# ssteinberg/wave_tracer

Measured on AMD Instinct MI355X. Metric: Msamples/sec (whole node), cornell-box 1440^2 wave-mode, higher is better.
Workload: dtype f32

## Files before the change

wave_tracer_amd/api.py:

```python
import ctypes as C
import json
import math
import os

_HERE = os.path.dirname(os.path.abspath(__file__))

os.environ.setdefault("HSA_KERNARG_POOL_SIZE", str(16 << 20))


def lib_path():
    return os.environ.get("WTGPU_LIB") or os.path.join(_HERE, "libwtgpu.so")


class WtgpuError(RuntimeError):
    pass


class SceneParams(C.Structure):
    _fields_ = [("res", C.c_uint32), ("max_depth", C.c_int32), ("fsd", C.c_int32), ("mis", C.c_int32), ("rr", C.c_int32),
                ("force_ray_tracing", C.c_int32), ("mesh_detail", C.c_int32), ("lut_n_theta", C.c_uint32), ("lut_m", C.c_uint32),
                ("polarimetric", C.c_int32)]


class TestHooks(C.Structure):
    _fields_ = [("only_s", C.c_uint32), ("only_t", C.c_uint32), ("crop_of", C.c_uint32)]


class SensorMaskSpec(C.Structure):
    _fields_ = [("present", C.c_int32), ("samples", C.c_uint32), ("regex", C.c_char_p), ("shape_flags", C.POINTER(C.c_uint8)),
                ("n_shapes", C.c_uint32)]


class TonemapSpec(C.Structure):
    _fields_ = [("present", C.c_int32), ("op", C.c_int32), ("mode", C.c_int32), ("gamma", C.c_float), ("db_min", C.c_float), ("db_max", C.c_float),
                ("colourmap", C.c_char_p), ("function", C.c_char_p)]


class Tonemap(C.Structure):
    _fields_ = [("op", C.c_int32), ("mode", C.c_int32), ("gamma", C.c_float), ("db_min", C.c_float), ("db_max", C.c_float),
                ("table", C.POINTER(C.c_float)), ("table_n", C.c_uint32)]


class FilmStatsSpec(C.Structure):
    _fields_ = [("stokes_component", C.c_uint32), ("scale", C.c_uint32), ("bins", C.c_uint32), ("flags", C.c_uint32), ("lo", C.c_float), ("hi", C.c_float)]


class FilmStats(C.Structure):
    _fields_ = [("n", C.c_uint64), ("n_nan", C.c_uint64), ("n_negative", C.c_uint64), ("n_zero", C.c_uint64), ("n_below", C.c_uint64), ("n_above", C.c_uint64),
                ("min", C.c_float), ("max", C.c_float), ("min_positive", C.c_float), ("pad", C.c_float), ("sum", C.c_double)]


class FilmCompareSpec(C.Structure):
    _fields_ = [("stokes_component", C.c_uint32), ("flags", C.c_uint32), ("eps", C.c_double)]


FILM_COMPARE_FIELDS = [("n", C.c_uint64), ("n_nonfinite", C.c_uint64), ("n_nonfinite_mismatch", C.c_uint64), ("n_differ", C.c_uint64), ("argmax", C.c_uint64),
                       ("max_abs", C.c_double), ("sum_abs", C.c_double), ("sum_sq", C.c_double), ("sum_a_sq", C.c_double), ("sum_b_sq", C.c_double),
                       ("sum_rel", C.c_double)]


class FilmCompare(C.Structure):
    _fields_ = FILM_COMPARE_FIELDS


class FilmPolarSpec(C.Structure):
    _fields_ = [("flags", C.c_uint32), ("maps", C.c_uint32), ("picture_plane", C.c_uint32), ("format", C.c_uint32), ("c2", C.c_double), ("s2", C.c_double),
                ("sat_gain", C.c_float), ("pad", C.c_float), ("tonemap", Tonemap)]


FILM_POLAR_FIELDS = [("n", C.c_uint64), ("n_nonfinite", C.c_uint64), ("n_dark", C.c_uint64), ("n_over", C.c_uint64), ("argmax", C.c_uint64),
                     ("max_dop", C.c_double), ("sum_i", C.c_double), ("sum_q", C.c_double), ("sum_u", C.c_double), ("sum_v", C.c_double),
                     ("sum_lin", C.c_double), ("sum_pol", C.c_double)]


class FilmPolar(C.Structure):
    _fields_ = FILM_POLAR_FIELDS


class FilmDenoiseSpec(C.Structure):
    _fields_ = [("window_radius", C.c_uint32), ("patch_radius", C.c_uint32), ("flags", C.c_uint32), ("pad", C.c_uint32), ("k", C.c_float), ("alpha", C.c_float),
                ("eps", C.c_float), ("pad2", C.c_float)]


FILM_POLAR_MAPS = ["dolp", "dop", "docp", "aolp", "chi", "analyser"]
FILM_STATS_SCALES = ["linear", "dB"]
FILM_STATS_ABS, FILM_STATS_LUMINANCE = 1, 2
FILM_STATS_MAX_BINS = 4096
TONEMAP_OPS = ["linear", "gamma", "sRGB", "dB", "function"]
TONEMAP_MODES = ["select", "normal", "colourmap"]
TONEMAP_FORMATS = {"f32": 0, "u8": 1, "u16": 2}


class SceneInfo(C.Structure):
    _fields_ = [("width", C.c_uint32), ("height", C.c_uint32), ("channels", C.c_uint32), ("n_tris", C.c_uint32), ("n_edges", C.c_uint32),
                ("n_nodes", C.c_uint32), ("n_leaves", C.c_uint32), ("n_shapes", C.c_uint32), ("n_emitters", C.c_uint32),
                ("n_materials", C.c_uint32), ("max_depth", C.c_int32), ("sensor_type", C.c_uint32), ("fsd_lut_power", C.c_double * 2),
                ("bytes_per_sample_state", C.c_uint64), ("stokes", C.c_uint32), ("integrator", C.c_uint32)]


COUNTER_FIELDS = ["samples", "segments", "ray_queries", "cone_queries", "vertices", "connections", "shadow_rays", "cone_tri_overflow",
                  "edge_overflow", "fsd_edge_overflow", "fsd_pool_overflow", "fsd_interactions", "null_interactions",
                  "surface_interactions", "light_splats", "walk_iteration_cap_hits", "traversal_stack_dropped"]


class Counters(C.Structure):
    _fields_ = [(n, C.c_uint64) for n in COUNTER_FIELDS]

    def as_dict(self):
        return {n: int(getattr(self, n)) for n in COUNTER_FIELDS}


SYMBOLS = ["wtgpu_scene_create_named", "wtgpu_scene_create_from_desc", "wtgpu_scene_get_info", "wtgpu_scene_host_desc",
           "wtgpu_scene_upload", "wtgpu_render", "wtgpu_trace_rays", "wtgpu_traverse_cones", "wtgpu_get_counters",
           "wtgpu_reset_counters", "wtgpu_last_render_timings", "wtgpu_develop", "wtgpu_scene_destroy", "wtgpu_last_error",
           "wtgpu_scene_stats_json", "wtgpu_calibrate_copy", "wtgpu_render_async", "wtgpu_join", "wtgpu_query_regions", "wtgpu_render_progressive",
           "wtgpu_cancel", "wtgpu_pause", "wtgpu_resume", "wtgpu_capture_intermediate", "wtgpu_comm_unique_id", "wtgpu_comm_create", "wtgpu_film_reduce", "wtgpu_comm_destroy", "wtgpu_scene_create_from_xml",
           "wtgpu_scene_shape_id", "wtgpu_scene_sensor_mask_spec", "wtgpu_sensor_mask", "wtgpu_sensor_mask_host",
           "wtgpu_scene_tonemap_spec", "wtgpu_develop_device", "wtgpu_tonemap_device", "wtgpu_tonemap_host",
           "wtgpu_film_stats_edges", "wtgpu_film_stats_device", "wtgpu_film_stats_host",
           "wtgpu_film_compare_device", "wtgpu_film_compare_host", "wtgpu_film_polar_device", "wtgpu_film_polar_host",
           "wtgpu_film_denoise_device", "wtgpu_film_denoise_host"]
PROGRESS_CB = C.CFUNCTYPE(C.c_int, C.c_uint64, C.c_uint64, C.c_void_p)
CAPTURE_CB = C.CFUNCTYPE(None, C.c_uint64, C.c_void_p)

_lib = None


def connect_class_order():
    import numpy as np
    lib = load_library()
    lib.wtgpu_test_connect_class_order.argtypes = [C.c_void_p, C.c_uint32, C.c_void_p, C.c_void_p]
    n, dim = C.c_uint32(0), C.c_uint32(0)
    _check(lib.wtgpu_test_connect_class_order(None, 0, C.byref(n), C.byref(dim)))
    keys = np.zeros(n.value, np.uint32)
    _check(lib.wtgpu_test_connect_class_order(keys.ctypes.data, keys.size, C.byref(n), C.byref(dim)))
    return keys, int(dim.value)


def dn_exp2_neg(t):
    import numpy as np
    t = np.ascontiguousarray(t, dtype=np.float32)
    out = np.zeros(t.shape, dtype=np.float32)
    _check(load_library().wtgpu_test_dn_exp2_neg(t.ctypes.data, t.size, out.ctypes.data))
    return out


def load_library():
    global _lib
    if _lib is not None:
        return _lib
    p = lib_path()
    if not os.path.exists(p):
        raise WtgpuError(f"{p} is missing: build it with `python -c 'import __graft_entry__ as g; g.build()'` "
                         f"(hipcc --offload-arch=gfx950); wave_tracer_amd has no CPU fallback")
    os.environ.setdefault("HSA_KERNARG_POOL_SIZE", str(16 << 20))
    try:
        import torch
    except ImportError:
        pass
    lib = C.CDLL(p)
    vp, u64, u32, i32 = C.c_void_p, C.c_uint64, C.c_uint32, C.c_int
    lib.wtgpu_scene_create_named.argtypes = [C.c_char_p, C.POINTER(SceneParams), C.POINTER(vp)]
    lib.wtgpu_scene_create_named_hooks.argtypes = [C.c_char_p, C.POINTER(SceneParams), C.POINTER(TestHooks), C.POINTER(vp)]
    lib.wtgpu_scene_create_from_desc.argtypes = [vp, C.POINTER(vp)]
    lib.wtgpu_scene_create_from_xml.argtypes = [C.c_char_p, C.POINTER(C.c_char_p), u32, C.POINTER(SceneParams), C.POINTER(vp)]
    lib.wtgpu_scene_compare.argtypes = [vp, vp, C.c_char_p, C.c_size_t]
    lib.wtgpu_scene_compare_part.argtypes = [vp, vp, C.c_char_p, C.c_char_p, C.c_size_t]
    lib.wtgpu_trace_ab_stats.argtypes = [vp, C.POINTER(C.c_double), C.POINTER(C.c_double), C.POINTER(u64), C.POINTER(u64), C.POINTER(u64)]
    lib.wtgpu_render_progressive.argtypes = [vp, vp, vp, vp, vp, u64, u64, u64, u32, PROGRESS_CB, vp, C.POINTER(u64)]
    lib.wtgpu_cancel.argtypes = [vp]
    lib.wtgpu_pause.argtypes = [vp]
    lib.wtgpu_resume.argtypes = [vp]
    lib.wtgpu_capture_intermediate.argtypes = [vp, CAPTURE_CB, vp]
    lib.wtgpu_comm_unique_id.argtypes = [vp]
    lib.wtgpu_comm_create.argtypes = [i32, i32, i32, vp, C.POINTER(vp)]
    lib.wtgpu_film_reduce.argtypes = [vp, vp, vp, vp, vp, u64, u64, i32]
    lib.wtgpu_comm_destroy.argtypes = [vp]
    lib.wtgpu_comm_destroy.restype = None
    lib.wtgpu_scene_get_info.argtypes = [vp, C.POINTER(SceneInfo)]
    lib.wtgpu_scene_host_desc.argtypes = [vp]
    lib.wtgpu_scene_host_desc.restype = vp
    lib.wtgpu_scene_upload.argtypes = [vp, i32, u64]
    lib.wtgpu_render.argtypes = [vp, vp, vp, vp, vp, u64, u64, u64]
    lib.wtgpu_render_async.argtypes = [vp, vp, vp, vp, vp, u64, u64, u64]
    lib.wtgpu_join.argtypes = [vp, vp]
    lib.wtgpu_trace_rays.argtypes = [vp, vp, vp, u32, vp, vp, vp, vp]
    lib.wtgpu_traverse_cones.argtypes = [vp, vp, vp, u32, u32, vp, vp, vp, vp]
    lib.wtgpu_query_regions.argtypes = [vp, vp, vp, u32, u32, vp, vp, vp, vp, vp, vp, vp]
    lib.wtgpu_test_fsd_apertures.argtypes = [vp, vp, vp, vp, vp, vp, u32, u32, u32, u32, vp, vp]
    lib.wtgpu_test_utd_sums.argtypes = [vp, vp, vp, vp, vp, u32, u32, u32, vp, vp, vp]
    lib.wtgpu_test_profile_counters.argtypes = [vp, vp, u32]
    lib.wtgpu_test_bsdf_queries.argtypes = [vp, vp, vp, u32, i32, vp]
    lib.wtgpu_test_source_queries.argtypes = [vp, vp, vp, u32, vp]
    lib.wtgpu_test_flux_queries.argtypes = [vp, vp, vp, u32, vp]
    lib.wtgpu_scene_shape_id.argtypes = [vp, u32, C.POINTER(C.c_char_p)]
    lib.wtgpu_scene_sensor_mask_spec.argtypes = [vp, C.POINTER(SensorMaskSpec)]
    lib.wtgpu_sensor_mask.argtypes = [vp, vp, vp, u32, u64, vp]
    lib.wtgpu_sensor_mask_host.argtypes = [vp, vp, u32, u64, u32, vp]
    lib.wtgpu_scene_tonemap_spec.argtypes = [vp, C.POINTER(TonemapSpec)]
    lib.wtgpu_develop_device.argtypes = [vp, vp, vp, vp, vp, u64, vp]
    lib.wtgpu_tonemap_device.argtypes = [vp, vp, vp, vp, vp, u64, C.POINTER(Tonemap), u32, vp, u32, vp]
    lib.wtgpu_tonemap_host.argtypes = [vp, vp, vp, vp, u64, C.POINTER(Tonemap), u32, vp, u32, u32, vp]
    lib.wtgpu_film_stats_edges.argtypes = [C.POINTER(FilmStatsSpec), vp]
    lib.wtgpu_film_stats_device.argtypes = [vp, vp, vp, vp, vp, u64, C.POINTER(FilmStatsSpec), vp, vp, vp]
    lib.wtgpu_film_stats_host.argtypes = [vp, vp, vp, vp, u64, C.POINTER(FilmStatsSpec), vp, u32, vp, vp]
    lib.wtgpu_film_compare_device.argtypes = [vp, vp, vp, vp, vp, u64, vp, vp, vp, u64, C.POINTER(FilmCompareSpec), vp, vp, vp]
    lib.wtgpu_film_compare_host.argtypes = [vp, vp, vp, vp, u64, vp, vp, vp, u64, C.POINTER(FilmCompareSpec), vp, u32, vp, vp]
    lib.wtgpu_film_polar_device.argtypes = [vp, vp, vp, vp, vp, u64, C.POINTER(FilmPolarSpec), vp, vp, vp, vp]
    lib.wtgpu_film_polar_host.argtypes = [vp, vp, vp, vp, u64, C.POINTER(FilmPolarSpec), vp, u32, vp, vp, vp]
    lib.wtgpu_film_denoise_device.argtypes = [vp, vp, vp, vp, vp, u64, vp, vp, vp, u64, C.POINTER(FilmDenoiseSpec), vp, vp, vp]
    lib.wtgpu_film_denoise_host.argtypes = [vp, vp, vp, vp, u64, vp, vp, vp, u64, C.POINTER(FilmDenoiseSpec), vp, u32, vp, vp]
    lib.wtgpu_test_dn_exp2_neg.argtypes = [vp, u64, vp]
    lib.wtgpu_calibrate_copy.argtypes = [u64, i32]
    lib.wtgpu_get_counters.argtypes = [vp, C.POINTER(Counters)]
    lib.wtgpu_reset_counters.argtypes = [vp]
    lib.wtgpu_last_render_timings.argtypes = [vp, C.POINTER(C.c_float * 12)]
    lib.wtgpu_develop.argtypes = [vp, vp, vp, vp, u64, vp]
    lib.wtgpu_scene_destroy.argtypes = [vp]
    lib.wtgpu_scene_destroy.restype = None
    lib.wtgpu_last_error.restype = C.c_char_p
    lib.wtgpu_scene_stats_json.argtypes = [vp]
    lib.wtgpu_scene_stats_json.restype = C.c_char_p
    _lib = lib
    return lib


def _check(rc):
    if rc != 0:
        raise WtgpuError(f"wtgpu error {rc}: {load_library().wtgpu_last_error().decode(errors='replace')}")


class Scene:

    def __init__(self, name, res=256, max_depth=-1, fsd=-1, mis=-1, rr=-1, force_ray_tracing=0, mesh_detail=1, lut=(0, 0), only_s=None, only_t=None, crop_of=0,
                 polarimetric=0):
        lib = load_library()
        p = SceneParams(res, max_depth, fsd, mis, rr, force_ray_tracing, mesh_detail, lut[0], lut[1], polarimetric)
        h = C.c_void_p()
        if only_s is None and only_t is None and not crop_of:
            _check(lib.wtgpu_scene_create_named(name.encode(), C.byref(p), C.byref(h)))
        else:
            hooks = TestHooks(0 if only_s is None else only_s + 1, 0 if only_t is None else only_t + 1, crop_of)
            _check(lib.wtgpu_scene_create_named_hooks(name.encode(), C.byref(p), C.byref(hooks), C.byref(h)))
        self._h = h
        self.name = name
        info = SceneInfo()
        _check(lib.wtgpu_scene_get_info(h, C.byref(info)))
        self.info = info
        self.spectral_channels, self.stokes = info.channels, info.stokes
        self.width, self.height, self.channels = info.width, info.height, info.channels * info.stokes
        self.device = None

    @classmethod
    def from_desc(cls, desc_ptr, keepalive=None, name="<desc>"):
        lib = load_library()
        self = cls.__new__(cls)
        h = C.c_void_p()
        _check(lib.wtgpu_scene_create_from_desc(C.c_void_p(desc_ptr), C.byref(h)))
        self._h = h
        self._keepalive = keepalive
        self.name = name
        info = SceneInfo()
        _check(lib.wtgpu_scene_get_info(h, C.byref(info)))
        self.info = info
        self.spectral_channels, self.stokes = info.channels, info.stokes
        self.width, self.height, self.channels = info.width, info.height, info.channels * info.stokes
        self.device = None
        return self

    @classmethod
    def from_xml(cls, path, defines=None, res=0, max_depth=-1, fsd=-1, mis=-1, rr=-1, force_ray_tracing=0, lut=(0, 0), polarimetric=0, mesh_detail=1):
        lib = load_library()
        self = cls.__new__(cls)
        p = SceneParams(res, max_depth, fsd, mis, rr, force_ray_tracing, mesh_detail, lut[0], lut[1], polarimetric)
        d = [f"{k}={v}".encode() for k, v in (defines or {}).items()]
        arr = (C.c_char_p * max(1, len(d)))(*d)
        h = C.c_void_p()
        _check(lib.wtgpu_scene_create_from_xml(str(path).encode(), arr, len(d), C.byref(p), C.byref(h)))
        self._h = h
        self.name = os.path.basename(str(path))
        info = SceneInfo()
        _check(lib.wtgpu_scene_get_info(h, C.byref(info)))
        self.info = info
        self.spectral_channels, self.stokes = info.channels, info.stokes
        self.width, self.height, self.channels = info.width, info.height, info.channels * info.stokes
        self.device = None
        return self

    def first_difference(self, other, part=None):
        buf = C.create_string_buffer(256)
        if part:
            rc = load_library().wtgpu_scene_compare_part(self._h, other._h, part.encode(), buf, 256)
        else:
            rc = load_library().wtgpu_scene_compare(self._h, other._h, buf, 256)
        if rc not in (0, 1):
            _check(rc)
        return buf.value.decode()

    @property
    def handle(self):
        return self._h

    def host_desc(self):
        return load_library().wtgpu_scene_host_desc(self._h)

    def stats(self):
        return json.loads(load_library().wtgpu_scene_stats_json(self._h).decode())

    def emitter_summary(self):
        return self.stats()["emitter_list"]

    def upload(self, device=0, max_batch_samples=0):
        _check(load_library().wtgpu_scene_upload(self._h, int(device), int(max_batch_samples)))
        self.device = int(device)
        return self

    def render_into(self, value, weight, light, sample_begin, sample_end, seed, stream=None):
        sp = C.c_void_p(stream) if stream else None
        _check(load_library().wtgpu_render(self._h, sp, value.data_ptr(), weight.data_ptr(), light.data_ptr(), int(sample_begin),
                                           int(sample_end), int(seed)))

    def render_async_into(self, value, weight, light, sample_begin, sample_end, seed, stream=None):
        sp = C.c_void_p(stream) if stream else None
        _check(load_library().wtgpu_render_async(self._h, sp, value.data_ptr(), weight.data_ptr(), light.data_ptr(), int(sample_begin),
                                                 int(sample_end), int(seed)))

    def render_progressive(self, value, weight, light, sample_begin, sample_end, seed, chunk_spp=1, progress=None, stream=None):
        sp = C.c_void_p(stream) if stream else None
        cb = PROGRESS_CB((lambda d, t, u: 1 if progress(d, t) else 0) if progress else (lambda d, t, u: 0))
        done = C.c_uint64(0)
        lib = load_library()
        rc = lib.wtgpu_render_progressive(self._h, sp, value.data_ptr(), weight.data_ptr(), light.data_ptr(), int(sample_begin), int(sample_end),
                                          int(seed), int(chunk_spp), cb, None, C.byref(done))
        if rc == 6:
            return True, int(done.value)
        _check(rc)
        return False, int(done.value)

    def cancel(self):
        _check(load_library().wtgpu_cancel(self._h))

    def pause(self):
        _check(load_library().wtgpu_pause(self._h))

    def resume(self):
        _check(load_library().wtgpu_resume(self._h))

    def capture_intermediate(self, fn):
        keep = self.__dict__.setdefault("_capture_keepalive", [])
        slot = []

        def tramp(done, user):
            try:
                fn(int(done))
            finally:
                if slot and slot[0] in keep:
                    keep.remove(slot[0])
        cb = CAPTURE_CB(tramp)
        slot.append(cb)
        keep.append(cb)
        if len(keep) > 64:
            del keep[0]
        _check(load_library().wtgpu_capture_intermediate(self._h, cb, None))

    def join(self, stream=None):
        _check(load_library().wtgpu_join(self._h, C.c_void_p(stream) if stream else None))

    def trace_rays(self, rays):
        import numpy as np
        import torch
        dev = torch.device("cuda", self.device)
        n = len(rays)
        d_rays = torch.from_numpy(np.ascontiguousarray(rays, dtype=np.float32)).to(dev)
        dist = torch.zeros(n, dtype=torch.float32, device=dev)
        tuid = torch.zeros(n, dtype=torch.int32, device=dev)
        bary = torch.zeros((n, 2), dtype=torch.float32, device=dev)
        front = torch.zeros(n, dtype=torch.int32, device=dev)
        _check(load_library().wtgpu_trace_rays(self._h, None, d_rays.data_ptr(), n, dist.data_ptr(), tuid.data_ptr(), bary.data_ptr(), front.data_ptr()))
        torch.cuda.synchronize(dev)
        return dist.cpu().numpy(), tuid.cpu().numpy().view(np.uint32), bary.cpu().numpy(), front.cpu().numpy().view(np.uint32)

    def traverse_cones(self, cones, cap=64):
        import numpy as np
        import torch
        dev = torch.device("cuda", self.device)
        n = len(cones)
        d_cones = torch.from_numpy(np.ascontiguousarray(cones, dtype=np.float32)).to(dev)
        dist = torch.zeros(n, dtype=torch.float32, device=dev)
        flags = torch.zeros(n, dtype=torch.int32, device=dev)
        ntris = torch.zeros(n, dtype=torch.int32, device=dev)
        tris = torch.zeros((n, cap), dtype=torch.int32, device=dev)
        _check(load_library().wtgpu_traverse_cones(self._h, None, d_cones.data_ptr(), n, cap, dist.data_ptr(), flags.data_ptr(), ntris.data_ptr(),
                                                   tris.data_ptr()))
        torch.cuda.synchronize(dev)
        return (dist.cpu().numpy(), flags.cpu().numpy().view(np.uint32), ntris.cpu().numpy().view(np.uint32),
                tris.cpu().numpy().view(np.uint32))

    def query_regions(self, cones, edge_cap=96):
        import numpy as np
        import torch
        dev = torch.device("cuda", self.device)
        n = len(cones)
        d_cones = torch.from_numpy(np.ascontiguousarray(cones, dtype=np.float32)).to(dev)
        dist = torch.zeros(n, dtype=torch.float32, device=dev)
        flux = torch.zeros(n, dtype=torch.float32, device=dev)
        flags, primary, ntris, nedges = (torch.zeros(n, dtype=torch.int32, device=dev) for _ in range(4))
        edges = torch.full((n, edge_cap), -1, dtype=torch.int32, device=dev)
        _check(load_library().wtgpu_query_regions(self._h, None, d_cones.data_ptr(), n, edge_cap, dist.data_ptr(), flags.data_ptr(), primary.data_ptr(),
                                                  ntris.data_ptr(), nedges.data_ptr(), edges.data_ptr(), flux.data_ptr()))
        torch.cuda.synchronize(dev)
        u = lambda t: t.cpu().numpy().view(np.uint32)
        return {"dist": dist.cpu().numpy(), "flags": u(flags), "primary": u(primary), "ntris": u(ntris), "nedges": u(nedges), "edges": u(edges),
                "flux": flux.cpu().numpy()}

    def fsd_apertures(self, cones, sk, ids, n_ids, pool_cap=4096, mode=0):
        import numpy as np
        import torch
        dev = torch.device("cuda", self.device)
        ids = np.ascontiguousarray(ids, dtype=np.uint32)
        n, id_cap = ids.shape
        n_ids = np.ascontiguousarray(n_ids, dtype=np.uint32)
        assert len(cones) == n and len(sk) == n and len(n_ids) == n and (n_ids <= id_cap).all()
        n_edges = self.info.n_edges
        assert all((ids[i, :n_ids[i]] < n_edges).all() for i in range(n)), "edge id out of range"
        t = lambda a, dt: torch.from_numpy(np.ascontiguousarray(a, dtype=dt)).to(dev)
        d_cones, d_sk = t(cones, np.float32), t(sk, np.float32)
        d_ids, d_nids = t(ids.view(np.int32), np.int32), t(n_ids.view(np.int32), np.int32)
        hdr = torch.zeros((n, 8), dtype=torch.int32, device=dev)
        segs = torch.zeros((n, pool_cap, 7), dtype=torch.float32, device=dev)
        _check(load_library().wtgpu_test_fsd_apertures(self._h, None, d_cones.data_ptr(), d_sk.data_ptr(), d_ids.data_ptr(), d_nids.data_ptr(), n, id_cap,
                                                       pool_cap, mode, hdr.data_ptr(), segs.data_ptr()))
        torch.cuda.synchronize(dev)
        return hdr.cpu().numpy().view(np.uint32), segs.cpu().numpy()

    def utd_sums(self, queries, ids, n_ids, utd_cap=48):
        import numpy as np
        import torch
        dev = torch.device("cuda", self.device)
        ids = np.ascontiguousarray(ids, dtype=np.uint32)
        n, id_cap = ids.shape
        n_ids = np.ascontiguousarray(n_ids, dtype=np.uint32)
        assert len(queries) == n and len(n_ids) == n and (n_ids <= id_cap).all()
        n_edges = self.info.n_edges
        assert all((ids[i, :n_ids[i]] < n_edges).all() for i in range(n)), "edge id out of range"
        t = lambda a, dt: torch.from_numpy(np.ascontiguousarray(a, dtype=dt)).to(dev)
        d_q, d_ids, d_nids = t(queries, np.float32), t(ids.view(np.int32), np.int32), t(n_ids.view(np.int32), np.int32)
        hdr = torch.zeros((n, 8), dtype=torch.int32, device=dev)
        edges = torch.zeros((n, utd_cap, 8), dtype=torch.int32, device=dev)
        recs = torch.zeros((n, utd_cap, 3), dtype=torch.int32, device=dev)
        _check(load_library().wtgpu_test_utd_sums(self._h, None, d_q.data_ptr(), d_ids.data_ptr(), d_nids.data_ptr(), n, id_cap, utd_cap, recs.data_ptr(),
                                                  hdr.data_ptr(), edges.data_ptr()))
        torch.cuda.synchronize(dev)
        u = lambda x: x.cpu().numpy().view(np.uint32)
        return u(hdr), u(edges), u(recs)

    def bsdf_queries(self, queries, form=-1):
        import numpy as np
        import torch
        dev = torch.device("cuda", self.device)
        q = np.ascontiguousarray(queries, dtype=np.uint32)
        n = q.shape[0]
        assert q.shape == (n, 18) and (q[:, 0] < self.info.n_materials).all(), "material id out of range"
        d_q = torch.from_numpy(q.view(np.int32)).to(dev)
        out = torch.zeros((n, 48), dtype=torch.int32, device=dev)
        _check(load_library().wtgpu_test_bsdf_queries(self._h, None, d_q.data_ptr(), n, int(form), out.data_ptr()))
        torch.cuda.synchronize(dev)
        return out.cpu().numpy().view(np.uint32)

    def source_queries(self, queries):
        import numpy as np
        import torch
        dev = torch.device("cuda", self.device)
        q = np.ascontiguousarray(queries, dtype=np.uint32)
        n = q.shape[0]
        assert q.shape == (n, 24)
        d_q = torch.from_numpy(q.view(np.int32)).to(dev)
        out = torch.zeros((n, 80), dtype=torch.int32, device=dev)
        _check(load_library().wtgpu_test_source_queries(self._h, None, d_q.data_ptr(), n, out.data_ptr()))
        torch.cuda.synchronize(dev)
        return out.cpu().numpy().view(np.uint32)

    def flux_queries(self, queries):
        import numpy as np
        import torch
        dev = torch.device("cuda", self.device)
        q = np.ascontiguousarray(queries, dtype=np.uint32)
        n = q.shape[0]
        assert q.shape == (n, 20)
        d_q = torch.from_numpy(q.view(np.int32)).to(dev)
        out = torch.zeros((n, 36), dtype=torch.int32, device=dev)
        _check(load_library().wtgpu_test_flux_queries(self._h, None, d_q.data_ptr(), n, out.data_ptr()))
        torch.cuda.synchronize(dev)
        return out.cpu().numpy().view(np.uint32)

    @property
    def shape_ids(self):
        lib, out = load_library(), []
        for i in range(self.info.n_shapes):
            p = C.c_char_p()
            _check(lib.wtgpu_scene_shape_id(self._h, i, C.byref(p)))
            out.append(p.value.decode())
        return out

    @property
    def sensor_mask_spec(self):
        import numpy as np
        s = SensorMaskSpec()
        _check(load_library().wtgpu_scene_sensor_mask_spec(self._h, C.byref(s)))
        if not s.present:
            return None
        flags = np.ctypeslib.as_array(s.shape_flags, (s.n_shapes,)).copy() if s.n_shapes else np.zeros(0, np.uint8)
        return {"regex": s.regex.decode(), "samples": int(s.samples), "shapes": flags}

    def _mask_args(self, samples, shapes):
        import numpy as np
        if samples is None:
            spec = self.sensor_mask_spec
            samples = spec["samples"] if spec else 32
        if shapes is None:
            return int(samples), None
        flags = np.ascontiguousarray(np.asarray(shapes) != 0, dtype=np.uint8)
        if flags.shape != (self.info.n_shapes,):
            raise ValueError(f"shapes: one flag per shape expected ({self.info.n_shapes}), got shape {flags.shape}")
        return int(samples), flags

    def sensor_mask(self, samples=None, seed=1, shapes=None, stream=None):
        import torch
        if self.device is None:
            raise WtgpuError("sensor_mask: upload(device) first")
        dev = torch.device("cuda", self.device)
        n, flags = self._mask_args(samples, shapes)
        out = torch.empty((self.height, self.width), dtype=torch.float32, device=dev)
        _check(load_library().wtgpu_sensor_mask(self._h, self._stream_arg(stream, dev), None if flags is None else flags.ctypes.data, n, int(seed),
                                                out.data_ptr()))
        return out

    def sensor_mask_host(self, samples=None, seed=1, shapes=None, threads=0):
        import numpy as np
        n, flags = self._mask_args(samples, shapes)
        out = np.zeros((self.height, self.width), np.float32)
        _check(load_library().wtgpu_sensor_mask_host(self._h, None if flags is None else flags.ctypes.data, n, int(seed), int(threads), out.ctypes.data))
        return out

    @property
    def tonemap_spec(self):
        s = TonemapSpec()
        _check(load_library().wtgpu_scene_tonemap_spec(self._h, C.byref(s)))
        return {"present": bool(s.present), "op": TONEMAP_OPS[s.op], "mode": TONEMAP_MODES[s.mode], "gamma": float(s.gamma),
                "db_range": (float(s.db_min), float(s.db_max)), "colourmap": s.colourmap.decode(), "function": s.function.decode()}

    @staticmethod
    def _tonemap_struct(tm):
        import numpy as np
        if tm is None:
            return None, None
        table = tm.get("table")
        tab = None if table is None else np.ascontiguousarray(table, dtype=np.float32)
        if tab is not None and (tab.ndim != 2 or tab.shape[1] != 3):
            raise ValueError(f"table: [n, 3] expected, got shape {tab.shape}")
        db = tm.get("db_range", (0.0, 0.0))
        st = Tonemap(TONEMAP_OPS.index(tm.get("op", "linear")), TONEMAP_MODES.index(tm.get("mode", "select")), float(tm.get("gamma", 2.2)),
                     float(db[0]), float(db[1]), None if tab is None else tab.ctypes.data_as(C.POINTER(C.c_float)), 0 if tab is None else len(tab))
        return st, tab

    @staticmethod
    def _stream_arg(stream, dev):
        import torch
        st = stream if stream is not None else torch.cuda.current_stream(dev).cuda_stream
        return C.c_void_p(st) if st else None

    def _host_films(self, what, value, weight, light, mask=None):
        import numpy as np
        v, w, l = (np.ascontiguousarray(t, dtype=np.float64) for t in (value, weight, light))
        m = None if mask is None else np.ascontiguousarray(mask, dtype=np.float32)
        n = self.width * self.height
        if v.size != n * self.channels or l.size != v.size or w.size != n or (m is not None and m.size != n):
            raise ValueError(f"{what}: films of the scene's size expected")
        return v, w, l, m

    def _device_films(self, what, value, weight, light, mask=None):
        import torch
        if self.device is None:
            raise WtgpuError(f"{what}: upload(device) first")
        n = self.width * self.height
        for t, name, numel, dtype in ((value, "value", n * self.channels, torch.float64), (weight, "weight", n, torch.float64),
                                      (light, "light", n * self.channels, torch.float64), (mask, "mask", n, torch.float32)):
            if t is None and name == "mask":
                continue
            if not (t.is_cuda and t.device.index == self.device and t.dtype == dtype and t.numel() == numel and t.is_contiguous()):
                raise ValueError(f"{what}: {name}: a contiguous {dtype} tensor of {numel} elements on cuda:{self.device} expected")
        return torch.device("cuda", self.device)

    def develop_device(self, value, weight, light, spe, stream=None):
        import torch
        dev = self._device_films("develop_device", value, weight, light)
        out = torch.empty(tuple(value.shape), dtype=torch.float32, device=dev)
        _check(load_library().wtgpu_develop_device(self._h, self._stream_arg(stream, dev), value.data_ptr(), weight.data_ptr(), light.data_ptr(), int(spe),
                                                   out.data_ptr()))
        return out

    def tonemap_device(self, value, weight, light, spe, tm=None, stokes_component=0, mask=None, fmt="f32", stream=None):
        import torch
        dev = self._device_films("tonemap_device", value, weight, light, mask)
        st_tm, keep = self._tonemap_struct(tm)
        dtype = {"f32": torch.float32, "u8": torch.uint8, "u16": torch.int16}[fmt]
        out = torch.empty((self.height, self.width, 4 if mask is not None else 3), dtype=dtype, device=dev)
        _check(load_library().wtgpu_tonemap_device(self._h, self._stream_arg(stream, dev), value.data_ptr(), weight.data_ptr(), light.data_ptr(), int(spe),
                                                   None if st_tm is None else C.byref(st_tm), int(stokes_component),
                                                   None if mask is None else mask.data_ptr(), TONEMAP_FORMATS[fmt], out.data_ptr()))
        del keep
        return out

    def tonemap_host(self, value, weight, light, spe, tm=None, stokes_component=0, mask=None, fmt="f32", threads=0):
        import numpy as np
        v, w, l, m = self._host_films("tonemap_host", value, weight, light, mask)
        st_tm, keep = self._tonemap_struct(tm)
        out = np.zeros((self.height, self.width, 4 if m is not None else 3), {"f32": np.float32, "u8": np.uint8, "u16": np.uint16}[fmt])
        _check(load_library().wtgpu_tonemap_host(self._h, v.ctypes.data, w.ctypes.data, l.ctypes.data, int(spe), None if st_tm is None else C.byref(st_tm),
                                                 int(stokes_component), None if m is None else m.ctypes.data, TONEMAP_FORMATS[fmt], int(threads), out.ctypes.data))
        del keep
        return out

    def _film_stats(self, what, call, stokes_component, scale, range, bins, abs, luminance):
        import numpy as np
        if scale not in FILM_STATS_SCALES:
            raise ValueError(f"{what}: scale 'dB' or 'linear' expected, got {scale!r}")
        planes = self.spectral_channels + (1 if luminance else 0)
        flags = (FILM_STATS_ABS if abs else 0) | (FILM_STATS_LUMINANCE if luminance else 0)

        def one_pass(lo, hi, nbins):
            spec = FilmStatsSpec(int(stokes_component), FILM_STATS_SCALES.index(scale), int(nbins), flags, float(lo), float(hi))
            rec = (FilmStats * max(planes, 1))()
            hist = np.zeros((planes, min(int(nbins), FILM_STATS_MAX_BINS)), dtype=np.uint64)
            call(spec, rec, hist.ctypes.data if hist.size else None)
            return spec, rec, hist

        if range is None:
            _, rec, _ = one_pass(0.0, 0.0, 0)
            lows = np.array([r.min_positive if scale == "dB" else r.min for r in rec], dtype=np.float64)
            highs = np.array([r.max for r in rec], dtype=np.float64)
            if np.isnan(lows).all() or not np.isfinite(np.nanmax(highs)):
                raise ValueError(f"{what}: range=None needs a finite {'positive ' if scale == 'dB' else ''}element to take the range from; pass a range")
            lo, hi = float(np.nanmin(lows)), float(np.nanmax(highs))
            if scale == "dB":
                lo, hi = 10.0 * math.log10(lo) - 1e-3, 10.0 * math.log10(hi) + 1e-3
            else:
                pad = max(math.fabs(lo), math.fabs(hi), 1e-30) * 1e-6
                lo, hi = lo - pad, hi + pad
            range = (lo, hi)
        spec, rec, hist = one_pass(range[0], range[1], bins)
        edges = np.zeros(spec.bins + 1, dtype=np.float32)
        _check(load_library().wtgpu_film_stats_edges(C.byref(spec), edges.ctypes.data))
        out = {name: np.array([getattr(r, name) for r in rec], dtype=dt) for name, dt in
               (("n", np.uint64), ("n_nan", np.uint64), ("n_negative", np.uint64), ("n_zero", np.uint64), ("n_below", np.uint64), ("n_above", np.uint64),
                ("min", np.float32), ("max", np.float32), ("min_positive", np.float32), ("sum", np.float64))}
        out.update(hist=hist, edges=edges, scale=scale, range=(float(spec.lo), float(spec.hi)), bins=int(spec.bins))
        return out

    def film_stats_device(self, value, weight, light, spe, *, stokes_component=0, scale="dB", range=None, bins=256, abs=False, luminance=False, mask=None,
                          stream=None):
        dev = self._device_films("film_stats_device", value, weight, light, mask)
        st = self._stream_arg(stream, dev)
        lib = load_library()

        def call(spec, rec, hist):
            _check(lib.wtgpu_film_stats_device(self._h, st, value.data_ptr(), weight.data_ptr(), light.data_ptr(), int(spe),
                                               C.byref(spec), None if mask is None else mask.data_ptr(), C.cast(rec, C.c_void_p), hist))
        return self._film_stats("film_stats_device", call, stokes_component, scale, range, bins, abs, luminance)

    def film_stats_host(self, value, weight, light, spe, *, stokes_component=0, scale="dB", range=None, bins=256, abs=False, luminance=False, mask=None,
                        threads=0):
        v, w, l, m = self._host_films("film_stats_host", value, weight, light, mask)
        lib = load_library()

        def call(spec, rec, hist):
            _check(lib.wtgpu_film_stats_host(self._h, v.ctypes.data, w.ctypes.data, l.ctypes.data, int(spe), C.byref(spec), None if m is None else m.ctypes.data,
                                             int(threads), C.cast(rec, C.c_void_p), hist))
        return self._film_stats("film_stats_host", call, stokes_component, scale, range, bins, abs, luminance)

    def _film_compare(self, call, stokes_component, abs, luminance, eps):
        import numpy as np
        planes = self.spectral_channels + (1 if luminance else 0)
        spec = FilmCompareSpec(int(stokes_component), (FILM_STATS_ABS if abs else 0) | (FILM_STATS_LUMINANCE if luminance else 0), float(eps))
        rec = (FilmCompare * max(planes, 1))()
        call(spec, rec, planes)
        out = {name: np.array([getattr(r, name) for r in rec], dtype=np.uint64 if t is C.c_uint64 else np.float64) for name, t in FILM_COMPARE_FIELDS}
        finite = (out["n"] - out["n_nonfinite"]).astype(np.float64)
        with np.errstate(divide="ignore", invalid="ignore"):
            out["rmse"] = np.sqrt(out["sum_sq"] / finite)
            out["mean_abs"] = out["sum_abs"] / finite
            out["rel_l2"] = np.sqrt(out["sum_sq"] / out["sum_b_sq"])
            out["rel_mse"] = out["sum_rel"] / finite
        return out

    def film_compare_device(self, films_a, spe_a, films_b, spe_b, *, stokes_component=0, abs=False, luminance=False, mask=None, eps=1e-4, diff=False, stream=None):
        import torch
        dev = self._device_films("film_compare_device", *films_a, mask)
        self._device_films("film_compare_device", *films_b)
        st = self._stream_arg(stream, dev)
        d = {}

        def call(spec, rec, planes):
            if diff:
                d["diff"] = torch.empty((self.height, self.width, planes), dtype=torch.float32, device=dev)
            _check(load_library().wtgpu_film_compare_device(self._h, st, *(t.data_ptr() for t in films_a), int(spe_a),
                                                            *(t.data_ptr() for t in films_b), int(spe_b), C.byref(spec), None if mask is None else mask.data_ptr(),
                                                            C.cast(rec, C.c_void_p), d["diff"].data_ptr() if diff else None))
        out = self._film_compare(call, stokes_component, abs, luminance, eps)
        out.update(d)
        return out

    def film_compare_host(self, films_a, spe_a, films_b, spe_b, *, stokes_component=0, abs=False, luminance=False, mask=None, eps=1e-4, diff=False, threads=0):
        import numpy as np
        sets = [self._host_films("film_compare_host", *films)[:3] for films in (films_a, films_b)]
        m = None if mask is None else np.ascontiguousarray(mask, dtype=np.float32)
        if m is not None and m.size != self.width * self.height:
            raise ValueError("film_compare_host: a mask of the scene's size expected")
        d = {}

        def call(spec, rec, planes):
            if diff:
                d["diff"] = np.zeros((self.height, self.width, planes), dtype=np.float32)
            _check(load_library().wtgpu_film_compare_host(self._h, *(t.ctypes.data for t in sets[0]), int(spe_a), *(t.ctypes.data for t in sets[1]), int(spe_b),
                                                          C.byref(spec), None if m is None else m.ctypes.data, int(threads), C.cast(rec, C.c_void_p),
                                                          d["diff"].ctypes.data if diff else None))
        out = self._film_compare(call, stokes_component, abs, luminance, eps)
        out.update(d)
        return out

    def _film_polar(self, what, call, luminance, maps, analyser, c2s2, picture, picture_plane, tm, fmt, sat_gain, masked):
        import numpy as np
        names = [maps] if isinstance(maps, str) else list(maps)
        for m in names:
            if m not in FILM_POLAR_MAPS:
                raise ValueError(f"{what}: maps of {FILM_POLAR_MAPS} expected, got {m!r}")
        if fmt not in TONEMAP_FORMATS:
            raise ValueError(f"{what}: fmt f32, u8 or u16 expected, got {fmt!r}")
        names = [m for m in FILM_POLAR_MAPS if m in names]
        planes = self.spectral_channels + (1 if luminance else 0)
        c2, s2 = (math.cos(2.0 * analyser), math.sin(2.0 * analyser)) if c2s2 is None else c2s2
        st_tm, _ = self._tonemap_struct(dict(tm or {"op": "linear"}, table=None))
        spec = FilmPolarSpec(FILM_STATS_LUMINANCE if luminance else 0, sum(1 << FILM_POLAR_MAPS.index(m) for m in names), int(picture_plane), TONEMAP_FORMATS[fmt],
                             float(c2), float(s2), float(sat_gain), 0.0, st_tm)
        rec = (FilmPolar * max(planes, 1))()
        got_maps, got_picture = call(spec, rec, (self.height, self.width, planes, len(names)) if names else None,
                                     (self.height, self.width, 4 if masked else 3) if picture else None)
        out = {name: np.array([getattr(r, name) for r in rec][:planes], dtype=np.uint64 if t is C.c_uint64 else np.float64) for name, t in FILM_POLAR_FIELDS}
        with np.errstate(divide="ignore", invalid="ignore"):
            out["dop_total"] = np.sqrt(out["sum_q"] ** 2 + out["sum_u"] ** 2 + out["sum_v"] ** 2) / out["sum_i"]
            out["aolp_total"] = 0.5 * np.arctan2(out["sum_u"], out["sum_q"])
            out["mean_dolp"] = out["sum_lin"] / out["sum_i"]
            out["mean_dop"] = out["sum_pol"] / out["sum_i"]
        out["maps"] = {m: got_maps[..., k] for k, m in enumerate(names)}
        out["picture"] = got_picture
        return out

    def film_polar_device(self, value, weight, light, spe, *, luminance=False, maps=(), analyser=0.0, c2s2=None, mask=None, picture=False, picture_plane=0, tm=None,
                          fmt="f32", sat_gain=1.0, stream=None):
        import torch
        dev = self._device_films("film_polar_device", value, weight, light, mask)
        st = self._stream_arg(stream, dev)

        def call(spec, rec, maps_shape, picture_shape):
            m = None if maps_shape is None else torch.empty(maps_shape, dtype=torch.float32, device=dev)
            p = None if picture_shape is None else torch.empty(picture_shape, dtype={"f32": torch.float32, "u8": torch.uint8, "u16": torch.int16}[fmt], device=dev)
            _check(load_library().wtgpu_film_polar_device(self._h, st, value.data_ptr(), weight.data_ptr(), light.data_ptr(), int(spe), C.byref(spec),
                                                          None if mask is None else mask.data_ptr(), C.cast(rec, C.c_void_p),
                                                          None if m is None else m.data_ptr(), None if p is None else p.data_ptr()))
            return m, p
        return self._film_polar("film_polar_device", call, luminance, maps, analyser, c2s2, picture, picture_plane, tm, fmt, sat_gain, mask is not None)

    def film_polar_host(self, value, weight, light, spe, *, luminance=False, maps=(), analyser=0.0, c2s2=None, mask=None, picture=False, picture_plane=0, tm=None,
                        fmt="f32", sat_gain=1.0, threads=0):
        import numpy as np
        v, w, l, m = self._host_films("film_polar_host", value, weight, light, mask)

        def call(spec, rec, maps_shape, picture_shape):
            mp = None if maps_shape is None else np.zeros(maps_shape, dtype=np.float32)
            p = None if picture_shape is None else np.zeros(picture_shape, dtype={"f32": np.float32, "u8": np.uint8, "u16": np.uint16}[fmt])
            _check(load_library().wtgpu_film_polar_host(self._h, v.ctypes.data, w.ctypes.data, l.ctypes.data, int(spe), C.byref(spec),
                                                        None if m is None else m.ctypes.data, int(threads), C.cast(rec, C.c_void_p),
                                                        None if mp is None else mp.ctypes.data, None if p is None else p.ctypes.data))
            return mp, p
        return self._film_polar("film_polar_host", call, luminance, maps, analyser, c2s2, picture, picture_plane, tm, fmt, sat_gain, m is not None)

    @staticmethod
    def _film_denoise_spec(window, patch, k, alpha, eps):
        return FilmDenoiseSpec(int(window), int(patch), 0, 0, float(k), float(alpha), float(eps), 0.0)

    def film_denoise_device(self, films_a, spe_a, films_b, spe_b, *, window=7, patch=2, k=0.45, alpha=1.0, eps=1e-10, mask=None, residual=False, stream=None):
        import torch
        dev = self._device_films("film_denoise_device", *films_a, mask)
        self._device_films("film_denoise_device", *films_b)
        shape = (self.height, self.width, self.spectral_channels, self.stokes)
        out = torch.empty(shape, dtype=torch.float32, device=dev)
        res = torch.empty(shape, dtype=torch.float32, device=dev) if residual else None
        spec = self._film_denoise_spec(window, patch, k, alpha, eps)
        _check(load_library().wtgpu_film_denoise_device(self._h, self._stream_arg(stream, dev), *(t.data_ptr() for t in films_a), int(spe_a),
                                                        *(t.data_ptr() for t in films_b), int(spe_b), C.byref(spec), None if mask is None else mask.data_ptr(),
                                                        out.data_ptr(), None if res is None else res.data_ptr()))
        return {"film": out, "residual": res}

    def film_denoise_host(self, films_a, spe_a, films_b, spe_b, *, window=7, patch=2, k=0.45, alpha=1.0, eps=1e-10, mask=None, residual=False, threads=0):
        import numpy as np
        sets = [self._host_films("film_denoise_host", *films)[:3] for films in (films_a, films_b)]
        m = None if mask is None else np.ascontiguousarray(mask, dtype=np.float32)
        if m is not None and m.size != self.width * self.height:
            raise ValueError("film_denoise_host: a mask of the scene's size expected")
        shape = (self.height, self.width, self.spectral_channels, self.stokes)
        out = np.zeros(shape, dtype=np.float32)
        res = np.zeros(shape, dtype=np.float32) if residual else None
        spec = self._film_denoise_spec(window, patch, k, alpha, eps)
        _check(load_library().wtgpu_film_denoise_host(self._h, *(t.ctypes.data for t in sets[0]), int(spe_a), *(t.ctypes.data for t in sets[1]), int(spe_b),
                                                      C.byref(spec), None if m is None else m.ctypes.data, int(threads), out.ctypes.data,
                                                      None if res is None else res.ctypes.data))
        return {"film": out, "residual": res}

    def profile_counters(self, n=8):
        out = (C.c_uint64 * n)()
        _check(load_library().wtgpu_test_profile_counters(self._h, out, n))
        return [int(v) for v in out]

    def connect_class_items(self, slice=0, max_items=1 << 22):
        import numpy as np
        lib = load_library()
        lib.wtgpu_test_connect_class_items.argtypes = [C.c_void_p, C.c_uint32, C.c_void_p, C.c_void_p, C.c_uint32, C.c_void_p]
        n_keys = connect_class_order()[0].size
        table = np.zeros(3 * n_keys + 1, np.uint32)
        items = np.zeros(max_items, np.uint32)
        n = C.c_uint32(0)
        _check(lib.wtgpu_test_connect_class_items(self._h, slice, table.ctypes.data, items.ctypes.data, items.size, C.byref(n)))
        return table[:n_keys + 1].copy(), table[n_keys + 1:2 * n_keys + 1].copy(), table[2 * n_keys + 1:].copy(), items[:n.value].copy()

    def counters(self):
        c = Counters()
        _check(load_library().wtgpu_get_counters(self._h, C.byref(c)))
        return c.as_dict()

    def reset_counters(self):
        _check(load_library().wtgpu_reset_counters(self._h))

    def trace_ab_stats(self):
        a, b, d, w, r = C.c_double(0), C.c_double(0), C.c_uint64(0), C.c_uint64(0), C.c_uint64(0)
        _check(load_library().wtgpu_trace_ab_stats(self._h, C.byref(a), C.byref(b), C.byref(d), C.byref(w), C.byref(r)))
        return {"ms_refill": a.value, "ms_sm": b.value, "differing_words": int(d.value), "walks": int(w.value), "rounds": int(r.value)}

    def timings(self):
        t = (C.c_float * 12)()
        _check(load_library().wtgpu_last_render_timings(self._h, C.byref(t)))
        return {"generate_ms": t[0], "trace_ms": t[1], "interact_ms": t[2], "connect_ms": t[3], "rounds": int(t[4]),
                "trace_launches": int(t[5]), "batches": int(t[6]), "trace_heavy_ms": t[7], "interact_b_ms": t[8], "flux_ms": t[9],
                "interact_c_ms": t[10], "rounds_per_batch": float(t[11])}

    def close(self):
        if self._h:
            load_library().wtgpu_scene_destroy(self._h)
            self._h = None

    def __del__(self):
        try:
            self.close()
        except Exception:
            pass


class Comm:

    def __init__(self, world, rank, device, unique_id):
        h = C.c_void_p()
        self._id = C.create_string_buffer(bytes(unique_id), 128)
        _check(load_library().wtgpu_comm_create(int(world), int(rank), int(device), self._id, C.byref(h)))
        self._h = h

    @staticmethod
    def unique_id():
        buf = C.create_string_buffer(128)
        _check(load_library().wtgpu_comm_unique_id(buf))
        return buf.raw

    def film_reduce(self, value, weight, light, root=0, stream=None):
        sp = C.c_void_p(stream) if stream else None
        _check(load_library().wtgpu_film_reduce(self._h, sp, value.data_ptr(), weight.data_ptr(), light.data_ptr(), value.numel(), weight.numel(), int(root)))

    def close(self):
        if self._h:
            load_library().wtgpu_comm_destroy(self._h)
            self._h = None

    def __del__(self):
        try:
            self.close()
        except Exception:
            pass
```

wave_tracer_amd/csrc/kernels_fsd.hip:

```cpp
#include "wtgpu_kernels.h"

namespace wtk {

__global__ void __launch_bounds__(64, 3) k_flux_split(launch_args_t a) {
    __shared__ coop_gather_shared_t sh;
    coop_set_dropped_counter(sh, a.st.counters + kDroppedSlot);
    uint32_t* ctl = a.st.ctl;
    const uint32_t n = ctl[CTL_INTC_COUNT];
    const int lane = threadIdx.x & 63;
    for (;;) {
        const uint32_t base = wave_grab(ctl + CTL_FSPLIT_HEAD);
        if (base >= n) break;
        uint32_t w_mine = 0;
        bool need = false;
        if (base + (uint32_t)lane < n) {
            w_mine = a.st.intc_queue[base + lane];
            need = is_region_marker(WT_TRAV_U(a, w_mine, tuid));
        }
        unsigned long long m = __ballot(need);
        while (m) {
            const int src = __ffsll((long long)m) - 1;
            m &= m - 1;
            const uint32_t w = (uint32_t)__shfl((int)w_mine, src, 64);
            const walk_trace_in_t wk = walk_load_trace_in(a.st.walks, a.st.walk_words, w);
            const cone_t tcone = walk_trace_envelope(a.sc, wk);
            const float beam_dist = WT_TRAV_F(a, w, dist), region_depth = WT_TRAV_F(a, w, region_depth);
            if (threadIdx.x == 0) a.st.facc[w] = 0.0;
            coop_split(a.sc, tcone, range_t{beam_dist, beam_dist + region_depth}, sh, a.flux_task_tris, [&](int32_t ptr) {
                const uint32_t idx = atomicAdd(ctl + CTL_FTASK_COUNT, 1u);
                if (idx < a.st.ftask_cap)
                    a.st.ftasks[idx] = make_uint2(w, (uint32_t)ptr);
                else
                    atomicAdd(a.st.counters + WT_COUNTER_SLOT(fsd_pool_overflow), 1ull);
            });
            __syncthreads();
        }
    }
}
__global__ void __launch_bounds__(64, WTGPU_LB_FLUX) k_flux_tasks(launch_args_t a) {
    __shared__ coop_gather_shared_t sh;
    coop_set_dropped_counter(sh, a.st.counters + kDroppedSlot);
    uint32_t* ctl = a.st.ctl;
    const uint32_t n = min(ctl[CTL_FTASK_COUNT], a.st.ftask_cap);
    for (;;) {
        const uint32_t item = wave_grab_item(ctl + CTL_FTASK_HEAD);
        if (item >= n) break;
        const uint2 task = a.st.ftasks[item];
        const uint32_t w = task.x;
        walk_t wk;
        soa_load(a.st.walks, a.st.walk_words, w, wk);
        const float beam_dist = WT_TRAV_F(a, w, dist), region_depth = WT_TRAV_F(a, w, region_depth);
        const bool want_front = WT_TRAV_U(a, w, front_face) != 0;
        const range_t izr{beam_dist, beam_dist + region_depth};
        const vec3 sd3 = beam_footprint(wk.beam, beam_dist) / kBeamEnvelope;
        const cone_t tcone = walk_trace_envelope(a.sc, wk);
        unsigned long long gst[2] = {0, 0};
        const double flux = coop_gather(a.sc, tcone, izr, wk.beam.env, cone_frame(wk.beam.env), izr, vec2{sd3.x, sd3.y}, want_front, sh, true, false,
                                        a.profile ? gst : nullptr, (int32_t)task.y).flux;
        if (threadIdx.x == 0) {
            if (flux != 0.0) unsafeAtomicAdd(&a.st.facc[w], flux);
            if (a.profile) {
                atomicAdd(a.st.counters + kNumCounters + 0, 1ull);
                atomicAdd(a.st.counters + kNumCounters + 1, gst[0]);
                atomicAdd(a.st.counters + kNumCounters + 2, gst[1]);
                atomicMax(a.st.counters + kNumCounters + 4, gst[0]);
            }
        }
        __syncthreads();
    }
}

constexpr uint32_t kEasyTries = 512;
constexpr uint32_t kStageSegs = 256;
template <int BLOCK>
WT_D void interact_c_body(const launch_args_t& a, int in) {
    constexpr bool HARD = BLOCK > 64;
    __shared__ uint32_t s_item;
    __shared__ uint32_t s_tmin;
    __shared__ float s_res[3];
    __shared__ stack_entry_t lds[8];
    __shared__ fsd_edge_t s_seg[kStageSegs];
    uint32_t* ctl = a.st.ctl;
    const uint32_t n = ctl[HARD ? CTL_INTD_COUNT : CTL_INTC_COUNT];
    const uint32_t* queue_in = HARD ? a.st.intd_queue : a.st.intc_queue;
    const int tid = threadIdx.x, lane = threadIdx.x & 63;
    bdpt_counters_t ctr;
    memset(&ctr, 0, sizeof(ctr));
    const fsd_pool_t pool = fsd_pool_of(a);
    for (;;) {
        const long long pl0 = a.profile == 3 ? clock64() : 0;
        uint32_t item = 0;
        if (HARD) {
            __syncthreads();
            if (tid == 0) s_item = atomicAdd(ctl + CTL_INTD_HEAD, 1u);
            __syncthreads();
            item = s_item;
        } else
            item = wave_grab_item(ctl + CTL_INTC_HEAD);
        if (item >= n) break;
        const uint32_t w = queue_in[item];
        uint32_t i, stream;
        walk_ident(a, w, i, stream);
        const uint64_t sample_id = sample_id_of(a, i);
        const uint32_t rng_draws = a.st.walks[(size_t)w * a.st.walk_words + WT_WALK_WORD(rng_draws)];
        const uint32_t slot = WT_TRAV_U(a, w, by);
        fsd_aperture_t ap = pool.hdr[slot];
        const fsd_edges_ref_t ed = fsd_pool_edges(pool, slot);
        const long long pc0 = a.profile == 3 ? clock64() : 0;
        if (!HARD) {
            const walk_trace_in_t wk = walk_load_trace_in(a.st.walks, a.st.walk_words, w);
            cone_t benv = wk.env;
            const float tr_dist = WT_TRAV_F(a, w, dist), tr_depth = WT_TRAV_F(a, w, region_depth);
            const uint32_t tr_tuid = WT_TRAV_U(a, w, tuid), tr_ntris = WT_TRAV_U(a, w, ntris);
            const bool tr_front = WT_TRAV_U(a, w, front_face) != 0;
            const range_t izr{tr_dist, tr_dist + tr_depth};
            const vec2 axes = cone_axes(benv, tr_dist);
            const vec2 sigma{axes.x / kBeamEnvelope, axes.y / kBeamEnvelope};
            double flux;
            if (is_region_marker(tr_tuid)) {
                flux = a.st.facc[w];
            } else {
                const uint32_t* tl = a.st.tris + (size_t)w * kTriListWords;
                flux = (uint32_t)lane < tr_ntris ? (double)region_triangle_flux(a.sc, cone_frame(benv), benv, izr, sigma, tl[lane], tr_front) : 0.0;
#pragma unroll
                for (int off = 32; off > 0; off >>= 1) flux += __shfl_xor(flux, off, 64);
            }
            const float I = (float)(1.0 - flux);
            ap.recp_I = I > 0.f ? 1.f / I : 0.f;
            if (lane == 0) pool.hdr[slot] = ap;
        }
        const sampler_t ss = make_sampler(a.seed, sample_id, stream, 0);
        const uint32_t base = fsd_tries_base(make_sampler(a.seed, sample_id, stream, rng_draws));
        const uint32_t max_tries = fsd_max_tries(ap);
        const uint32_t t_begin = HARD ? kEasyTries : 0u, t_end = HARD ? max_tries : (max_tries < kEasyTries ? max_tries : kEasyTries);
        bool acc = false;
        uint32_t t_acc = 0;
        float rx = 0.f, ry = 0.f, rf = 0.f;
        auto run_tries = [&](const fsd_edges_ref_t& edr) {
            for (uint32_t t0 = t_begin; t0 < t_end && !acc; t0 += BLOCK) {
                const uint32_t t = t0 + (uint32_t)tid;
                fsd_try_t r{{0.f, 0.f}, 0.f, 0u};
                if (t < t_end) r = fsd_try(a.sc, ap, edr, sampler_at(ss, base + t * kFsdDrawsPerTry));
                if (!HARD) {
                    const unsigned long long am = __ballot(r.accept != 0);
                    if (am) {
                        const int wl = __ffsll((long long)am) - 1;
                        rx = __shfl(r.x.x, wl, 64);
                        ry = __shfl(r.x.y, wl, 64);
                        rf = __shfl(r.f, wl, 64);
                        t_acc = t0 + (uint32_t)wl;
                        acc = true;
                    }
                } else {
                    if (tid == 0) s_tmin = 0xFFFFFFFFu;
                    __syncthreads();
                    if (r.accept) atomicMin(&s_tmin, t);
                    __syncthreads();
                    const uint32_t tm = s_tmin;
                    if (tm != 0xFFFFFFFFu) {
                        if (t == tm) {
                            s_res[0] = r.x.x;
                            s_res[1] = r.x.y;
                            s_res[2] = r.f;
                        }
                        __syncthreads();
                        rx = s_res[0];
                        ry = s_res[1];
                        rf = s_res[2];
                        t_acc = tm;
                        acc = true;
                    }
                    __syncthreads();
                }
            }
        };
        if (ap.n_edges <= kStageSegs) {
            __syncthreads();
            for (uint32_t k = (uint32_t)tid; k < ap.n_edges; k += BLOCK) s_seg[k] = ed.p[k];
            __syncthreads();
            run_tries(fsd_edges_ref_t{s_seg, 1});
        } else
            run_tries(ed);
        if (a.profile == 3 && tid == 0) {
            const int bin = 31 - __clz((int)max(ap.n_edges, 1u));
            atomicAdd(a.st.counters + kNumCounters + 8 + bin, 1ull);
            atomicAdd(a.st.counters + kNumCounters + 24 + bin, (unsigned long long)(acc ? t_acc + 1u - t_begin : t_end - t_begin));
            atomicAdd(a.st.counters + kNumCounters + 40 + bin, (unsigned long long)(clock64() - pc0));
            atomicAdd(a.st.counters + kNumCounters + 112 + bin, (unsigned long long)(pc0 - pl0));
        }
        const long long pm0 = a.profile == 3 ? clock64() : 0;
        if (!HARD && !acc && t_end < max_tries) {
            if (lane == 0) a.st.intd_queue[atomicAdd(ctl + CTL_INTD_COUNT, 1u)] = w;
            continue;
        }
        bool cont = false;
        if (tid == 0) {
            walk_t wk;
            soa_load(a.st.walks, a.st.walk_words, w, wk);
            trav_result_t tr;
            soa_load(a.st.trav, kTravWords, w, tr);
            fsd_defer_t defer;
            defer.defer_sampling = defer.to_sampling_pass = 0;
            defer.have_aperture = 1;
            defer.split_no_primary = 0;
            defer.known_no_primary = 1;
            defer.no_primary = 0;
            defer.has_gather = defer.gather_n_edges = defer.gather_edge_overflow = 0;
            defer.gather_flux = 0.f;
            defer.gather_edges = nullptr;
            defer.pending = 0;
            defer.resolved = 1;
            defer.slot = slot;
            defer.base = base;
            defer.next_try = 0;
            defer.fs = fsd_finalize(ap, acc, vec2{rx, ry}, rf);
            defer.end_draws = fsd_draws_after(base, acc ? t_acc : max_tries - 1u);
            const uint_list_t tris{a.st.tris + (size_t)w * kTriListWords, 1u, kMaxConeTris};
            const vertex_store_t vs = walk_vertices(a, w);
            stack_ref_t stack = make_stack_ref(lds, 1, 8, 8, nullptr);
            cont = bdpt_walk_step<2>(a.sc, wk, tr, tris, vs, pool, a.seed, sample_id, stream, &ctr, &stack, &defer);
            wk.active = cont ? 1u : 0u;
            soa_store(a.st.walks, a.st.walk_words, w, wk);
            if (a.profile == 3) atomicAdd(a.st.counters + kNumCounters + 96 + (31 - __clz((int)max(ap.n_edges, 1u))), (unsigned long long)(clock64() - pm0));
        }
        if (tid < 64) queue_append(a, ctl, 1 - in, cont, w);
    }
    if (a.count_stats && tid < 64) flush_counters(a.st.counters, ctr);
}
__global__ void __launch_bounds__(64, WTGPU_LB_INTERACT_C) k_interact_c(launch_args_t a, int in) { interact_c_body<64>(a, in); }
__global__ void __launch_bounds__(WTGPU_HARD_BLOCK) k_interact_c_hard(launch_args_t a, int in) { interact_c_body<WTGPU_HARD_BLOCK>(a, in); }

}
```

wave_tracer_amd/csrc/kernels_trace_refill.h:

```cpp
#pragma once
#include "wtgpu_kernels.h"

namespace wtk {

#ifndef WTGPU_LEAF_NUM
#define WTGPU_LEAF_NUM 1
#define WTGPU_LEAF_DEN 2
#endif
#ifndef WTGPU_REFILL_MIN
#define WTGPU_REFILL_MIN 16
#endif
WT_D bool policy_next_query(const scene_t& sc, const cone_t& env, bool rt, const stack_ref_t& stack, axis_walk_t& aw, cone_query_t& q, trav_result_t& r) {
    for (;;) {
        const int need = aw_next(sc, env, rt, stack, aw, q, r);
        if (need != AW_TEST) return need == AW_QUERY;
        aw_test_done(aw, cone_attempt_too_short_by(sc, env, aw.cand, aw.sr, aw.min_df_prog));
    }
}
WT_D void trace_round_begin(uint32_t* ctl, int in, uint32_t round, uint32_t n) {
    ctl[CTL_COUNT0 + (1 - in)] = 0;
    ctl[CTL_BACK0 + (1 - in)] = 0;
    ctl[CTL_HEAD_INTERACT] = 0;
    ctl[CTL_INTB_COUNT] = 0;
    ctl[CTL_INTB_HEAD] = 0;
    ctl[CTL_GATHER_COUNT] = 0;
    ctl[CTL_GATHER_HEAD] = 0;
    ctl[CTL_INTC_COUNT] = 0;
    ctl[CTL_INTC_HEAD] = 0;
    ctl[CTL_FTASK_COUNT] = 0;
    ctl[CTL_FTASK_HEAD] = 0;
    ctl[CTL_FSPLIT_HEAD] = 0;
    ctl[CTL_EPOOL_COUNT] = 0;
    ctl[CTL_INTD_COUNT] = 0;
    ctl[CTL_INTD_HEAD] = 0;
#pragma unroll
    for (uint32_t c = 0; c < kNumWalkClasses; ++c) ctl[CTL_CLS_COUNT0 + c] = ctl[CTL_CLS_HEAD0 + c] = 0;
    ctl[CTL_UTD_COUNT0 + (round & 1u)] = 0;
    ctl[CTL_FSDQ_COUNT0 + ((round + 1u) & 1u)] = 0;
    ctl[CTL_FSDQ_HEAD] = 0;
    ctl[CTL_NEEQ_COUNT] = 0;
    ctl[CTL_NEEQ_HEAD] = 0;
    if (n > 0) ctl[CTL_ROUNDS] = round + 1;
}
WT_D void trace_refill_body(const launch_args_t& a, int in, int first_round, uint32_t round) {
    __shared__ stack_entry_t lds[kLdsStack * kBlock];
    uint32_t* ctl = a.st.ctl;
    const uint32_t n = queue_count(ctl, in);
    if (blockIdx.x == 0 && threadIdx.x == 0) trace_round_begin(ctl, in, round, n);
    bdpt_counters_t ctr;
    memset(&ctr, 0, sizeof(ctr));
    stack_entry_t spill[kSpillStack];
    stack_ref_t stack;
    lds_stack(lds, spill, stack);
    const size_t W2 = 2 * (size_t)a.st.cap;
    const bool rt = a.sc.sensor.ray_trace_only || a.sc.opts.force_ray_tracing;
    const int lane = threadIdx.x & 63;
    const unsigned long long below = (1ull << lane) - 1ull;
    int st = 0;
    uint32_t w = 0;
    cone_t env;
    axis_walk_t aw;
    cone_query_t q;
    uint_list_t tris{nullptr, 1u, 0u, nullptr};
    memset(&env, 0, sizeof(env));
    memset(&aw, 0, sizeof(aw));
    memset(&q, 0, sizeof(q));
    bool exhausted = false;
#ifdef WTGPU_REFILL_PROF
    unsigned long long pc[6] = {0, 0, 0, 0, 0, 0}, pl[6] = {0, 0, 0, 0, 0, 0};
    long long pt;
#define RP_BEGIN() pt = clock64()
#define RP_END(i, mask) do { const long long d_ = clock64() - pt; pc[i] += (unsigned long long)d_; pl[i] += (unsigned long long)d_ * (unsigned long long)__popcll(mask); } while (0)
#else
#define RP_BEGIN()
#define RP_END(i, mask)
#endif
    for (;;) {
        bool fin = false;
        trav_result_t r;
        RP_BEGIN();
        const unsigned long long m_srv = __ballot(st == 2);
        if (st == 2) {
            cq_end(env, tris, q);
            fin = aw_query_done(a.sc, env, aw, q.rec, r);
            if (!fin) fin = !policy_next_query(a.sc, env, rt, stack, aw, q, r);
            st = fin ? 0 : 1;
        }
        RP_END(0, m_srv);
        uint32_t w_fin = w;
        const int n_idle = __popcll(__ballot(st == 0 && !fin)), n_run = __popcll(__ballot(st == 1));
        bool fetched = false;
        const bool any_fin = __ballot(fin) != 0;
        if (!exhausted && !any_fin && (n_idle >= WTGPU_REFILL_MIN || n_run == 0)) {
            const unsigned long long im = __ballot(st == 0);
            const bool take = st == 0;
            uint32_t base = 0;
            if (lane == 0) base = atomicAdd(ctl + CTL_HEAD_TRACE, (uint32_t)__popcll(im));
            base = (uint32_t)__shfl((int)base, 0, 64);
            if (base + (uint32_t)__popcll(im) >= n) exhausted = true;
            const uint32_t qi = base + (uint32_t)__popcll(im & below);
            RP_BEGIN();
            const unsigned long long m_f = __ballot(take && qi < n);
            if (take && qi < n) {
                w = queue_walk(a, ctl, in, qi, first_round);
                w_fin = w;
                const walk_trace_in_t wk = walk_load_trace_in(a.st.walks, a.st.walk_words, w);
                uint32_t* slot = a.st.tris + (size_t)w * kTriListWords;
                tris = uint_list_t{slot, 1u, (a.collect_list & 1u) ? kMaxConeTris : 0u, reinterpret_cast<float*>(slot + kMaxConeTris)};
                env = walk_trace_envelope(a.sc, wk);
                ray_hit_t ah;
                const bool axis_hit = ads_intersect_ray(a.sc, env.o, env.d, range_t{0.f, WT_INF}, stack, ah);
                aw_begin(aw, wavenum_to_wavelen_m(wk.k), WT_INF, axis_hit, ah, a.cone_budget, true, !(a.collect_list & 1u) || (a.collect_list & 2u), a.lane_cache ? wk.prev_offset_tuid : kInvalid);
                aw.use_cache = a.lane_cache;
                fin = !policy_next_query(a.sc, env, rt, stack, aw, q, r);
                st = fin ? 0 : 1;
            }
            RP_END(1, m_f);
            fetched = true;
        }
        RP_BEGIN();
        const unsigned long long m_st = __ballot(fin);
        {
            const bool heavy = fin && r.aborted == 1;
            if (fin) {
                if (heavy) {
                    a.st.trav[(size_t)w_fin * kTravWords + WT_TRAV_WORD(dist)] = __float_as_uint(r.dist);
                    a.st.trav[(size_t)w_fin * kTravWords + WT_TRAV_WORD(ntris)] = r.ntris;
                    a.st.trav[(size_t)w_fin * kTravWords + WT_TRAV_WORD(n_ray_queries)] = r.n_ray_queries;
                    a.st.trav[(size_t)w_fin * kTravWords + WT_TRAV_WORD(n_cone_queries)] = r.n_cone_queries;
                    a.st.trav[(size_t)w_fin * kTravWords + WT_TRAV_WORD(tuid)] = r.tuid;
                    a.st.trav[(size_t)w_fin * kTravWords + WT_TRAV_WORD(bx)] = __float_as_uint(r.bx);
                    a.st.trav[(size_t)w_fin * kTravWords + WT_TRAV_WORD(by)] = __float_as_uint(r.by);
                    a.st.trav[(size_t)w_fin * kTravWords + WT_TRAV_WORD(pdist)] = __float_as_uint(r.pdist);
                    a.st.trav[(size_t)w_fin * kTravWords + WT_TRAV_WORD(front_face)] = r.front_face;
                    a.st.trav[(size_t)w_fin * kTravWords + WT_TRAV_WORD(overflow)] = r.overflow;
                } else {
                    soa_store(a.st.trav, kTravWords, w_fin, r);
                    ctr.segments += 1;
                    ctr.ray_queries += r.n_ray_queries;
                    ctr.cone_queries += r.n_cone_queries;
                    if (a.collect_list & 1u) ctr.cone_tri_overflow += r.overflow;
                }
            }
            wave_append(a.st.heavy_queue, ctl + CTL_HEAVY_COUNT, heavy, w_fin);
        }
        RP_END(2, m_st);
        if (fetched || any_fin) continue;
        const int running = __popcll(__ballot(st == 1));
        if (running == 0) {
            if (exhausted) break;
            continue;
        }
        const int leave_at = running < 4 * WTGPU_REFILL_MIN ? (running + 3) / 4 : WTGPU_REFILL_MIN;
        for (;;) {
            for (;;) {
                const bool at_node = st == 1 && q.leaf == 0 && q.s > 0;
                const unsigned long long nm = __ballot(at_node);
                if (!nm) break;
                RP_BEGIN();
                if (at_node) cq_node_step(a.sc, env, stack, q);
                RP_END(3, nm);
                if (WTGPU_LEAF_DEN * __popcll(__ballot(st == 1 && q.leaf != 0)) >= WTGPU_LEAF_NUM * running) break;
            }
            RP_BEGIN();
            const unsigned long long m_leaf = __ballot(st == 1 && q.leaf != 0);
            if (st == 1 && q.leaf != 0) cq_leaf_step(a.sc, env, stack, tris, q);
            RP_END(4, m_leaf);
            if (st == 1 && !cq_running(q)) st = 2;
            const int waiting = __popcll(__ballot(st == 2)) + (exhausted ? 0 : __popcll(__ballot(st == 0)));
            if (waiting >= leave_at || !__ballot(st == 1)) break;
        }
    }
    if (a.count_stats) flush_counters(a.st.counters, ctr);
#ifdef WTGPU_REFILL_PROF
    if (lane == 0)
        for (int i = 0; i < 6; ++i) {
            atomicAdd(a.st.counters + kNumCounters + i, pc[i]);
            atomicAdd(a.st.counters + kNumCounters + 8 + i, pl[i]);
        }
    if (lane != 0 && pc[5]) { atomicAdd(a.st.counters + kNumCounters + 5, pc[5]); atomicAdd(a.st.counters + kNumCounters + 8 + 5, pl[5]); }
#endif
}


}
```

wave_tracer_amd/csrc/wtgpu.hip:

```cpp
#include "wtgpu_host.h"

thread_local std::string g_err;

static void note_rounds(wtgpu_scene* s, uint32_t n) { s->rounds_hist[s->rounds_hist_n++ % 8u] = n; }
static int drain_rec(wtgpu_scene* s, chunk_rec_t& r) {
    if (!r.busy) return WTGPU_OK;
    HIP_CHECK(hipEventSynchronize(r.ev[r.ev_final]));
    const uint32_t rounds = r.h_ctl[CTL_ROUNDS];
    s->cap_hits += r.h_ctl[CTL_COUNT0 + (r.rounds_launched & 1u)] + r.h_ctl[CTL_BACK0 + (r.rounds_launched & 1u)];
    s->acc[4] += rounds;
    s->acc[5] += rounds;
    s->acc[6] += 1;
    s->rounds_launched_total += r.rounds_launched;
    if (s->knobs.timing) {
        auto elapsed = [](hipEvent_t a, hipEvent_t b) {
            float ms = 0.f;
            return hipEventElapsedTime(&ms, a, b) == hipSuccess ? ms : 0.f;
        };
        s->acc[0] += elapsed(r.ev[0], r.ev[1]);
        size_t e = 1;
        for (uint32_t k = 0; k < r.rounds_timed; ++k, e += 6) {
            static const int slot[6] = {1, 7, 2, 8, 9, 10};
            for (int q = 0; q < 6; ++q) s->acc[slot[q]] += elapsed(r.ev[e + q], r.ev[e + q + 1]);
        }
        s->acc[3] += elapsed(r.ev[e], r.ev[r.ev_final]);
    }
    r.busy = false;
    return WTGPU_OK;
}

struct batch_launcher_t {
    wtgpu_scene* s;
    const wtgpu_scene::knobs_t& K;
    uint32_t grid_round = 0, grid_heavy = 0;
    bool path_mode = false;
    bool ev_fail = false;
    static constexpr int kHpSlots = 64;
    bool hp_on = false, trace_on = false;
    double hp_t[kHpSlots] = {0};
    unsigned long hp_n[kHpSlots] = {0};
    static const char** hp_labels() {
        static const char* labels[kHpSlots] = {nullptr};
        return labels;
    }
    static int hp_slot(const char* label) {
        static std::mutex m;
        std::lock_guard<std::mutex> l(m);
        const char** labels = hp_labels();
        int i = 0;
        while (i < kHpSlots - 1 && labels[i] && std::strcmp(labels[i], label) != 0) ++i;
        if (!labels[i]) labels[i] = label;
        return i;
    }
    explicit batch_launcher_t(wtgpu_scene* s_) : s(s_), K(s_->knobs) {
        grid_round = s->n_cus * K.round_blocks_per_cu;
        grid_heavy = s->n_cus * K.heavy_waves_per_cu;
        path_mode = s->host.opts.integrator != INTEGRATOR_BDPT;
        hp_on = K.host_prof != 0;
        trace_on = K.trace_launch != 0;
    }
#define HP_LAUNCH(kernel, ...)                                                                                            \
    do {                                                                                                                  \
        if (trace_on) {    \
            fprintf(stderr, "[wtgpu launch] %s ...", #kernel);                                                            \
            hipLaunchKernelGGL(kernel, __VA_ARGS__);                                                                      \
            const hipError_t e_ = hipDeviceSynchronize();                                                                 \
            fprintf(stderr, " done (%s)\n", hipGetErrorString(e_));                                                       \
        } else if (hp_on) {                                                                                                      \
            static const int slot_ = hp_slot(#kernel);                                                                    \
            const auto t0_ = std::chrono::steady_clock::now();                                                            \
            hipLaunchKernelGGL(kernel, __VA_ARGS__);                                                                      \
            hp_t[slot_] += std::chrono::duration<double, std::micro>(std::chrono::steady_clock::now() - t0_).count();     \
            hp_n[slot_]++;                                                                                                \
        } else                                                                                                            \
            hipLaunchKernelGGL(kernel, __VA_ARGS__);                                                                      \
    } while (0)
    void rec(chunk_rec_t& r, hipStream_t st_) {
        const auto hp0_ = std::chrono::steady_clock::now();
        if (s->knobs.timing && r.ev_used + 1 >= r.ev.size()) return;
        if (s->knobs.timing && hipEventRecord(r.ev[r.ev_used++], st_) != hipSuccess) ev_fail = true;
        if (hp_on) { static const int slot_ = hp_slot("hipEventRecord"); hp_t[slot_] += std::chrono::duration<double, std::micro>(std::chrono::steady_clock::now() - hp0_).count(); hp_n[slot_]++; }
    }
    uint32_t g_full(uint32_t nb) const { return std::min<uint32_t>(grid_round, ((path_mode ? 1u : 2u) * nb + kBlock - 1) / kBlock); }
    void generate(const launch_args_t& a, chunk_rec_t& r, hipStream_t st_) {
        r.ev_used = 0;
        r.rounds_launched = 0;
        r.rounds_timed = 0;
        rec(r, st_);
        if (path_mode)
            HP_LAUNCH(k_path_generate, dim3((a.nb + kBlock - 1) / kBlock), dim3(kBlock), 0, st_, a);
        else
            HP_LAUNCH(k_generate, dim3((a.nb + kBlock - 1) / kBlock), dim3(kBlock), 0, st_, a);
        rec(r, st_);
    }
    int rounds(const launch_args_t& a, const path_state_t* ps, chunk_rec_t& r, hipStream_t st_, uint32_t r_begin, uint32_t r_end, int stage_from = 0) {
        const uint32_t nb = a.nb, walks_per_sample = path_mode ? 1u : 2u, gf = g_full(nb);
        const uint32_t grid_div_b = K.grid_div_b, grid_div_c = K.grid_div_c, grid_mul_flux = K.grid_mul_flux;
        const int dbg_stage = (int)K.dbg_stage;
        for (uint32_t round = r_begin; round < r_end; ++round) {
            const int in = (int)(round & 1u), first = round == 0 ? 1 : 0;
            if (s->knobs.timing && r.ev_used + 7 < r.ev.size()) r.rounds_timed++;
            if (round == K.stagger_round && K.stagger_round > 0) {
                HIP_CHECK(hipEventRecord(r.ev_stagger, st_));
                s->ev_stagger_last = r.ev_stagger;
            }
            uint32_t g0, gh;
            if (K.decay_q > 0) {
                const double f = std::min(1.0, (double)K.decay_c * std::pow(K.decay_q * .01, (double)round));
                g0 = std::max<uint32_t>(2u, (uint32_t)(gf * f));
                gh = std::max<uint32_t>(2u, (uint32_t)(std::min<uint32_t>(grid_heavy, walks_per_sample * nb) * f));
            } else {
                const uint32_t shrink = round < K.shrink_r1 ? 1u : (round < K.shrink_r2 ? K.shrink_f1 : K.shrink_f2);
                g0 = std::max<uint32_t>(1u, gf / shrink);
                gh = std::max<uint32_t>(1u, std::min<uint32_t>(grid_heavy, walks_per_sample * nb) / (round < K.shrink_r1 ? 1u : (round < K.shrink_r2 ? K.shrink_h1 : 32u)));
            }
            const int sf = round == r_begin ? stage_from : 0;
            if (sf <= 0 && dbg_stage >= 2 + 3 * (int)round) {
                if (round < K.trace_ab) {
                    const int rc = trace_ab_round(s, a, st_, in, first, round, g0);
                    if (rc) return rc;
                } else if (K.trace_sm || (K.trace_staged && round < K.trace_staged_rounds))
                    launch_trace_alt(s, a, st_, in, first, round, g0);
                else
                    HP_LAUNCH(k_trace_refill, dim3(g0), dim3(kBlock), 0, st_, a, in, first, round);
            }
            rec(r, st_);
            if (sf <= 1 && dbg_stage >= 3 + 3 * (int)round) {
                if (a.profile == 2)
                    HP_LAUNCH(k_trace_heavy_prof, dim3(gh), dim3(64), 0, st_, a);
                else
                    HP_LAUNCH(k_trace_heavy, dim3(gh), dim3(64), 0, st_, a);
            }
            rec(r, st_);
            if (path_mode) {
                if (round > 0) HP_LAUNCH(k_path_fsd, dim3(gh), dim3(64), 0, st_, a, ps, round);
                if (dbg_stage >= 4 + 3 * (int)round) HP_LAUNCH(k_path_interact, dim3(g0), dim3(kBlock), 0, st_, a, ps, in, first, round);
                HP_LAUNCH(k_path_edges, dim3(gh), dim3(64), 0, st_, a, ps);
                HP_LAUNCH(k_path_interact_b, dim3(std::max<uint32_t>(1u, g0 / 2u)), dim3(kBlock), 0, st_, a, ps, in, round);
                HP_LAUNCH(k_path_nee, dim3(gh), dim3(64), 0, st_, a, ps, round);
                rec(r, st_);
                rec(r, st_);
                rec(r, st_);
                rec(r, st_);
                continue;
            }
            if (sf > 2) {
            } else if (K.sorted_interact) {
                HP_LAUNCH(k_classify, dim3(g0), dim3(kBlock), 0, st_, a, in, first);
                if (K.sorted_interact >= 2)
                    HP_LAUNCH(k_interact_sorted, dim3(g0), dim3(kBlock), 0, st_, a, in);
                else {
                HP_LAUNCH(k_interact_diffuse, dim3(std::max<uint32_t>(1u, g0 / K.grid_div_cls[0])), dim3(kBlock), 0, st_, a, in);
                HP_LAUNCH(k_interact_dielectric, dim3(std::max<uint32_t>(1u, g0 / K.grid_div_cls[1])), dim3(kBlock), 0, st_, a, in);
                HP_LAUNCH(k_interact_spm, dim3(std::max<uint32_t>(1u, g0 / K.grid_div_cls[2])), dim3(kBlock), 0, st_, a, in);
                HP_LAUNCH(k_interact_any, dim3(std::max<uint32_t>(1u, g0 / K.grid_div_cls[3])), dim3(kBlock), 0, st_, a, in);
                }
            } else if (K.coop_io)
                HP_LAUNCH(k_interact_coop, dim3(g0), dim3(kBlock), 0, st_, a, in, first);
            else
                HP_LAUNCH(k_interact, dim3(g0), dim3(kBlock), 0, st_, a, in, first);
            rec(r, st_);
            if (sf <= 3) HP_LAUNCH(k_edges, dim3(gh), dim3(64), 0, st_, a);
            if (sf <= 4) HP_LAUNCH(k_interact_b, dim3(std::max<uint32_t>(1u, g0 / grid_div_b)), dim3(kBlock), 0, st_, a, in);
            rec(r, st_);
            HP_LAUNCH(k_flux_split, dim3(std::max<uint32_t>(1u, gh / 4u)), dim3(64), 0, st_, a);
            HP_LAUNCH(k_flux_tasks, dim3(std::max<uint32_t>(1u, gh * grid_mul_flux)), dim3(64), 0, st_, a);
            rec(r, st_);
            HP_LAUNCH(k_interact_c, dim3(std::max<uint32_t>(1u, gh / grid_div_c)), dim3(64), 0, st_, a, in);
            HP_LAUNCH(k_interact_c_hard, dim3(std::max<uint32_t>(1u, gh / K.grid_div_hard)), dim3(WTGPU_HARD_BLOCK), 0, st_, a, in);
            rec(r, st_);
        }
        r.rounds_launched = r_end;
        return WTGPU_OK;
    }
    void light(const launch_args_t& a, hipStream_t st_, uint32_t launched) {
        if (path_mode || !K.light_rounds || launched >= K.max_rounds) return;
        HP_LAUNCH(k_light_rounds, dim3(1), dim3(kBlock), 0, st_, a, (int)(launched & 1u), launched, K.max_rounds - launched);
    }
    int tail(const launch_args_t& a, chunk_rec_t& r, hipStream_t st_) {
        const uint32_t nb = a.nb, gf = g_full(nb);
        if (path_mode) {
            HP_LAUNCH(k_path_flush, dim3(kFlushGrid), dim3(kBlock), 0, st_, a, (int)(r.rounds_launched & 1u));
        } else {
            const bool open = (uint32_t)s->host.opts.max_depth + 2 >= kKeyDim - 1;
            const bool staged = K.staged_connect && !open;
            const uint32_t by_class = !staged && K.connect_class ? 1u : 0u;
            HP_LAUNCH(k_connect_enum, dim3((nb + kEnumBlock - 1) / kEnumBlock), dim3(kEnumBlock), 0, st_, a, by_class);
            HP_LAUNCH(k_connect_scan, dim3(1), dim3(64), 0, st_, a, by_class);
            if (staged) {
                for (uint32_t c = 0; c < s->n_chunks; ++c) {
                    const uint32_t g = c == 0 ? gf : std::max<uint32_t>(1u, gf / 8u);
                    HP_LAUNCH(k_connect_eval, dim3(g), dim3(kBlock), 0, st_, a, c);
                    HP_LAUNCH(k_connect_shadow, dim3(g), dim3(kBlock), 0, st_, a, c);
                    HP_LAUNCH(k_connect_mis, dim3(g), dim3(kBlock), 0, st_, a, c);
                }
            } else if (by_class) {
                HP_LAUNCH(k_connect_class, dim3(gf), dim3(kBlock), 0, st_, a);
                if (open) HP_LAUNCH(k_connect_class_open, dim3(std::max<uint32_t>(1u, gf / 8u)), dim3(kBlock), 0, st_, a);
            } else {
                HP_LAUNCH(k_connect_strat, dim3(gf), dim3(kBlock), 0, st_, a);
                if (open) HP_LAUNCH(k_connect_strat_open, dim3(std::max<uint32_t>(1u, gf / 8u)), dim3(kBlock), 0, st_, a);
            }
            const uint32_t fw = a.film.width, fh = a.film.height, planes = film_planes(s->host.sensor);
            if (K.tiled_splat && s->host.sensor.rf_radius <= 1 && planes <= 16 && (uint64_t)nb * 2u >= (uint64_t)a.npix) {
                for (uint32_t phase = 0; phase < kSplatPhases; ++phase) {
                    const uint32_t rows = splat_phase_rows(phase, fh), segs = splat_phase_segments(phase, splat_segments(fw));
                    if (rows * segs) HP_LAUNCH(k_connect_splat_tiled, dim3(rows * segs), dim3(kSplatBlock), 3 * kSplatCols * (planes + 1) * sizeof(double), st_, a, phase);
                }
            } else
                HP_LAUNCH(k_connect_splat, dim3((nb + kBlock - 1) / kBlock), dim3(kBlock), 0, st_, a);
        }
        HIP_CHECK(hipGetLastError());
        HIP_CHECK(hipMemcpyAsync(r.h_ctl, a.st.ctl, CTL_WORDS * sizeof(uint32_t), hipMemcpyDeviceToHost, st_));
        r.ev_final = s->knobs.timing ? r.ev_used : 0;
        HIP_CHECK(hipEventRecord(r.ev[r.ev_final], st_));
        if (ev_fail) return fail(WTGPU_ERR_HIP, "hipEventRecord failed");
        r.busy = true;
        return WTGPU_OK;
    }
#undef HP_LAUNCH
    void report() const {
        if (!hp_on) return;
        const char* const* labels = hp_labels();
        for (int i = 0; i < kHpSlots; ++i)
            if (hp_n[i]) fprintf(stderr, "[host prof] %-22s %6lu calls %9.1f us total %7.2f us each\n", labels[i], hp_n[i], hp_t[i], hp_t[i] / hp_n[i]);
    }
};
static_assert(sizeof(launch_args_t) <= sizeof(wtgpu_scene::pending_t::args), "pending_t::args holds a launch block");

static uint32_t expected_rounds(const wtgpu_scene* s) {
    if (s->knobs.first_rounds) return s->knobs.first_rounds;
    if (s->rounds_hist_n == 0) return std::min<uint32_t>(kMaxWalkIters, 32u);
    const uint32_t n = std::min<uint32_t>(s->rounds_hist_n, 8u);
    uint32_t sum = 0;
    for (uint32_t i = 0; i < n; ++i) sum += s->rounds_hist[i];
    const uint32_t mean = (sum + n - 1) / n;
    return std::min<uint32_t>(kMaxWalkIters, mean + s->knobs.rounds_margin);
}
static int finish_look(wtgpu_scene* s, size_t k, batch_launcher_t& L) {
    wtgpu_scene::pending_t& p = s->pending[k];
    chunk_rec_t& r = *p.rec;
    launch_args_t a;
    std::memcpy(&a, p.args, sizeof(a));
    hipStream_t st_ = s->streams[k];
    uint32_t& launched = p.launched;
    const bool light = !L.path_mode && s->knobs.light_rounds != 0;
    uint32_t stop = 0;
    if (light && launched < s->knobs.max_rounds) {
        launched += r.h_mid[CTL_LIGHT_DONE];
        stop = r.h_mid[CTL_LIGHT_STOP];
        s->light_rounds_run += r.h_mid[CTL_LIGHT_DONE];
    }
    bool done = false;
    if (s->knobs.tail_diag) {
        static unsigned long long looks = 0, by_stop[8] = {0}, light_done = 0, left_sum = 0;
        static bool reg = false;
        if (!reg) { reg = true; atexit([] { fprintf(stderr, "[tail diag] looks %llu (stop 0/1/2/3/4: %llu %llu %llu %llu %llu), light rounds %llu, walks left at looks (sum) %llu\n", looks, by_stop[0], by_stop[1], by_stop[2], by_stop[3], by_stop[4], light_done, left_sum); }); }
        looks++; by_stop[stop < 8 ? stop : 7]++; light_done += light ? r.h_mid[CTL_LIGHT_DONE] : 0;
        left_sum += r.h_mid[CTL_COUNT0 + (launched & 1u)] + r.h_mid[CTL_BACK0 + (launched & 1u)];
    }
    if (stop >= 1 && stop <= 3) {
        static const int from[4] = {0, 1, 3, 5};
        const int rc = L.rounds(a, s->d_path_slices[k], r, st_, launched, launched + 1, from[stop]);
        if (rc) return rc;
        launched += 1;
    } else {
        const uint32_t q = launched & 1u;
        const uint32_t left = r.h_mid[CTL_COUNT0 + q] + r.h_mid[CTL_BACK0 + q];
        if (left == 0) {
            note_rounds(s, std::min<uint32_t>(r.h_mid[CTL_ROUNDS], kMaxWalkIters));
            done = true;
        } else if (launched >= s->knobs.max_rounds)
            done = true;
        else {
            s->round_fallbacks++;
            const uint32_t next = std::min<uint32_t>(s->knobs.max_rounds, launched + p.rounds_step);
            const int rc = L.rounds(a, s->d_path_slices[k], r, st_, launched, next);
            if (rc) return rc;
            launched = next;
            p.rounds_step = std::min<uint32_t>(64u, p.rounds_step * 2u);
        }
    }
    if (done) {
        p.active = false;
        r.rounds_launched = launched;
        return L.tail(a, r, st_);
    }
    L.light(a, st_, launched);
    HIP_CHECK(hipMemcpyAsync(r.h_mid, a.st.ctl, CTL_WORDS * sizeof(uint32_t), hipMemcpyDeviceToHost, st_));
    HIP_CHECK(hipEventRecord(r.ev_mid, st_));
    return WTGPU_OK;
}
static int serve_pending(wtgpu_scene* s, size_t k, batch_launcher_t& L) {
    const size_t n = s->pending.size();
    for (;;) {
        bool any = false, progressed = false;
        for (size_t j = 0; j < n; ++j) {
            wtgpu_scene::pending_t& p = s->pending[j];
            if (!p.active) continue;
            if (k != (size_t)-1 && !s->pending[k].active) break;
            any = true;
            const hipError_t q = hipEventQuery(p.rec->ev_mid);
            if (q == hipSuccess) {
                const int rc = finish_look(s, j, L);
                if (rc) return rc;
                progressed = true;
            } else if (q != hipErrorNotReady)
                HIP_CHECK(q);
            else
                (void)hipGetLastError();
        }
        if (k != (size_t)-1 ? !s->pending[k].active : !any) return WTGPU_OK;
        if (!progressed) {
            std::this_thread::sleep_for(std::chrono::microseconds(20));
        }
    }
}
static int finish_all_pending(wtgpu_scene* s) {
    bool any = false;
    for (const auto& p : s->pending) any = any || p.active;
    if (!any) return WTGPU_OK;
    batch_launcher_t L(s);
    return serve_pending(s, (size_t)-1, L);
}
int drain_all(wtgpu_scene* s) {
    {
        const int rc = finish_all_pending(s);
        if (rc) return rc;
    }
    for (auto& r : s->recs) {
        const int rc = drain_rec(s, r);
        if (rc) return rc;
    }
    return WTGPU_OK;
}

extern "C" {

const char* wtgpu_last_error(void) { return g_err.c_str(); }

int wtgpu_join(wtgpu_scene* s, void* stream_) {
    if (!s || !s->uploaded) return fail(WTGPU_ERR_INVALID, "scene not uploaded");
    hipStream_t caller = static_cast<hipStream_t>(stream_);
    device_guard_t guard(s->device);
    {
        const int rc = finish_all_pending(s);
        if (rc) return rc;
    }
    for (size_t k = 0; k < s->slices.size(); ++k) {
        HIP_CHECK(hipEventRecord(s->ev_done[k], s->streams[k]));
        HIP_CHECK(hipStreamWaitEvent(caller, s->ev_done[k], 0));
    }
    return WTGPU_OK;
}

int wtgpu_render(wtgpu_scene* s, void* stream_, double* d_value, double* d_weight, double* d_light, uint64_t sb, uint64_t se, uint64_t seed) {
    const int rc = wtgpu_render_async(s, stream_, d_value, d_weight, d_light, sb, se, seed);
    return rc ? rc : wtgpu_join(s, stream_);
}

int wtgpu_render_async(wtgpu_scene* s, void* stream_, double* d_value, double* d_weight, double* d_light, uint64_t sb, uint64_t se, uint64_t seed) {
    if (!s || !s->uploaded) return fail(WTGPU_ERR_INVALID, "scene not uploaded");
    if (!d_value || !d_weight || !d_light || se < sb) return fail(WTGPU_ERR_INVALID, "bad film pointers / sample range");
    hipStream_t caller = static_cast<hipStream_t>(stream_);
    device_guard_t guard(s->device);
    const scene_t& h = s->host;
    const uint64_t npix = (uint64_t)h.sensor.width * h.sensor.height;
    const uint64_t total = npix * (se - sb);
    if (total == 0) return WTGPU_OK;
    launch_args_t a;
    static_assert(sizeof(launch_args_t) <= 984, "by-value kernel arguments beyond 1 KB serialise the streams (see path_state_t)");
    a.sc = s->dev;
    a.film = film_t{d_value, d_weight, d_light, h.sensor.width, h.sensor.height, h.sensor.channels};
    a.seed = seed;
    a.npix = (uint32_t)npix;
    a.sample_begin = sb;
    const wtgpu_scene::knobs_t& K = s->knobs;
    a.count_stats = K.count_stats;
    a.cone_budget = K.cone_budget;
    a.profile = K.profile;
    a.coop_aperture_min = K.coop_aperture_min;
    a.heavy_probe = K.heavy_probe;
    a.split_queues = K.split_queues;
    a.lane_cache = K.lane_cache;
    a.heavy_cache = K.heavy_cache;
    a.flux_task_tris = K.flux_task_tris;
    a.collect_list = ((h.opts.integrator != INTEGRATOR_BDPT || !K.no_lists) ? 1u : 0u) | ((h.opts.integrator == INTEGRATOR_BDPT && K.primary_axis) ? 2u : 0u);
    batch_launcher_t L(s);

    HIP_CHECK(hipEventRecord(s->ev_begin, caller));
    const size_t n_slices = s->slices.size();
    std::vector<char> used(n_slices, 0);
    const uint64_t cap = s->slices[0].cap;
    for (uint64_t j0 = 0; j0 < total; j0 += cap) {
        const size_t k = s->slice_next++ % n_slices;
        hipStream_t st_ = s->streams[k];
        {
            const int rc = s->pending[k].active ? serve_pending(s, k, L) : WTGPU_OK;
            if (rc) return rc;
        }
        if (!used[k]) {
            HIP_CHECK(hipStreamWaitEvent(st_, s->ev_begin, 0));
            used[k] = 1;
        }
        chunk_rec_t& r = s->recs[s->rec_next];
        s->rec_next = (s->rec_next + 1) % s->recs.size();
        int rc = drain_rec(s, r);
        if (rc) return rc;
        const uint32_t nb = (uint32_t)std::min<uint64_t>(cap, total - j0);
        if (K.stagger_round > 0 && s->ev_stagger_last && n_slices > 1) HIP_CHECK(hipStreamWaitEvent(st_, s->ev_stagger_last, 0));
        a.st = s->slices[k];
        a.j0 = j0;
        a.nb = nb;
        const uint32_t r1 = expected_rounds(s);
        L.generate(a, r, st_);
        rc = L.rounds(a, s->d_path_slices[k], r, st_, 0, r1);
        if (rc) return rc;
        HIP_CHECK(hipGetLastError());
        L.light(a, st_, r1);
        HIP_CHECK(hipMemcpyAsync(r.h_mid, a.st.ctl, CTL_WORDS * sizeof(uint32_t), hipMemcpyDeviceToHost, st_));
        HIP_CHECK(hipEventRecord(r.ev_mid, st_));
        wtgpu_scene::pending_t& p = s->pending[k];
        std::memcpy(p.args, &a, sizeof(a));
        p.rec = &r;
        p.launched = r1;
        p.rounds_step = 8;
        p.active = true;

    }
    L.report();
    s->samples_rendered += total;
    return WTGPU_OK;
}

int wtgpu_last_render_timings(wtgpu_scene* s, float out[12]) {
    if (!s || !out || !s->uploaded) return fail(WTGPU_ERR_INVALID, "scene not uploaded");
    const int rc = drain_all(s);
    if (rc) return rc;
    for (int i = 0; i < 12; ++i) out[i] = (float)s->acc[i];
    out[11] = s->acc[6] > 0 ? (float)((double)s->rounds_launched_total / s->acc[6]) : (float)kMaxWalkIters;
    return WTGPU_OK;
}

}
```

wave_tracer_amd/csrc/wtgpu_counters.hip:

```cpp
#include "wtgpu_host.h"

extern "C" {

int wtgpu_get_counters(wtgpu_scene* s, wtgpu_counters* out) {
    if (!s || !out || !s->uploaded) return fail(WTGPU_ERR_INVALID, "scene not uploaded");
    bdpt_counters_t c;
    {
        const int rc = drain_all(s);
        if (rc) return rc;
    }
    HIP_CHECK(hipDeviceSynchronize());
    HIP_CHECK(hipMemcpy(&c, s->slices[0].counters, sizeof(c), hipMemcpyDeviceToHost));
    out->samples = s->samples_rendered;
    out->segments = c.segments;
    out->ray_queries = c.ray_queries;
    out->cone_queries = c.cone_queries;
    out->vertices = c.vertices;
    out->connections = c.connections;
    out->shadow_rays = c.shadow_rays;
    out->cone_tri_overflow = c.cone_tri_overflow;
    out->edge_overflow = c.edge_overflow;
    out->fsd_edge_overflow = c.fsd_edge_overflow;
    out->fsd_pool_overflow = c.fsd_pool_overflow;
    out->fsd_interactions = c.fsd_interactions;
    out->null_interactions = c.null_interactions;
    out->surface_interactions = c.surface_interactions;
    out->light_splats = c.light_splats;
    out->walk_iteration_cap_hits = s->cap_hits;
    {
        unsigned long long dropped = 0;
        HIP_CHECK(hipMemcpy(&dropped, s->slices[0].counters + kDroppedSlot, sizeof(dropped), hipMemcpyDeviceToHost));
        out->traversal_stack_dropped = dropped;
    }
#ifdef WTGPU_STEP_PROF
    {
        unsigned long long p[8];
        HIP_CHECK(hipMemcpy(p, s->slices[0].counters + kNumCounters, sizeof(p), hipMemcpyDeviceToHost));
        fprintf(stderr, "[wtgpu step prof] pass-B walks %llu (with aperture %llu); total Mticks: scan %.1f pre %.1f edges %.1f integrals+aperture %.1f sample+append %.1f continue %.1f\n", p[7], p[6],
                double(p[0]) * 1e-6, double(p[1]) * 1e-6, double(p[2]) * 1e-6, double(p[3]) * 1e-6, double(p[4]) * 1e-6, double(p[5]) * 1e-6);
    }
#endif
#ifdef WTGPU_COOP_PROF
    if (getenv("WTGPU_PROFILE")) {
        unsigned long long p[12];
        HIP_CHECK(hipMemcpy(p, s->slices[0].counters + kNumCounters, sizeof(p), hipMemcpyDeviceToHost));
        const double n = p[4] ? double(p[4]) : 1.;
        fprintf(stderr, "[coop prof] items %llu; per item ticks: A.pop %.0f A.node+test %.0f A.push %.0f B1.filter %.0f flush+phaseB %.0f; per item: phase-B entries %.1f, candidates %.0f, filter batches %.1f, exact batches %.1f\n", p[4], p[0] / n, p[1] / n,
                p[2] / n, p[7] / n, p[6] / n, p[10] / n, p[11] / n, p[8] / n, p[9] / n);
    }
#endif
    if (s->knobs.profile == 1) {
        unsigned long long p[8];
        HIP_CHECK(hipMemcpy(p, s->slices[0].counters + kNumCounters, sizeof(p), hipMemcpyDeviceToHost));
        fprintf(stderr, "[wtgpu profile] flux tasks: %llu, candidates %llu (max %llu per task), exact-tested %llu; k_edges: %llu walks, %llu edges, %llu apertures built\n", p[0], p[1], p[4], p[2], p[5], p[6], p[3]);
    }
    if (s->knobs.profile == 3) {
        unsigned long long p[kProfSlots];
        HIP_CHECK(hipMemcpy(p, s->slices[0].counters + kNumCounters, sizeof(p), hipMemcpyDeviceToHost));
        fprintf(stderr, "[wtgpu profile] pass C by aperture size (slice 0): bin=log2(segments) items tries/item kticks/item total-Mticks\n");
        for (int b = 0; b < 16; ++b)
            if (p[8 + b]) fprintf(stderr, "[wtgpu profile]   C %2d %8llu %10.1f %10.1f %10.1f   fetch+load %.1f commit %.1f kticks/item\n", b, p[8 + b], double(p[24 + b]) / p[8 + b], double(p[40 + b]) / p[8 + b] * 1e-3, double(p[40 + b]) * 1e-6, double(p[112 + b]) / p[8 + b] * 1e-3, double(p[96 + b]) / p[8 + b] * 1e-3);
        fprintf(stderr, "[wtgpu profile] pass B by gathered scene edges: bin items kticks/item total-Mticks\n");
        for (int b = 0; b < 16; ++b)
            if (p[56 + b]) fprintf(stderr, "[wtgpu profile]   B %2d %8llu %10.1f %10.1f\n", b, p[56 + b], double(p[72 + b]) / p[56 + b] * 1e-3, double(p[72 + b]) * 1e-6);
    }
#ifdef WTGPU_REFILL_PROF
    {
        unsigned long long p[16];
        HIP_CHECK(hipMemcpy(p, s->slices[0].counters + kNumCounters, sizeof(p), hipMemcpyDeviceToHost));
        const char* nm[6] = {"serve", "fetch", "store", "nodes", "leaf", "(ray in fetch)"};
        for (int i = 0; i < 6; ++i) fprintf(stderr, "[refill prof] %-16s %10.1f Mticks  lanes %.1f\n", nm[i], p[i] * 1e-6, p[i] ? double(p[8 + i]) / p[i] : 0.);
    }
#endif
#ifdef WTGPU_SM_PROF
    {
        unsigned long long p[64];
        HIP_CHECK(hipMemcpy(p, s->slices[0].counters + kNumCounters, sizeof(p), hipMemcpyDeviceToHost));
        const char* nm[7] = {"serve", "fetch", "aw_next", "store", "NODE", "TRI", "EXACT"};
        for (int i = 0; i < 7; ++i)
            fprintf(stderr, "[sm prof] %-8s %10.1f Mticks  %10.2f Msteps  %7.0f ticks/step  lanes %.1f\n", nm[i], p[32 + i] * 1e-6, p[48 + i] * 1e-6, p[48 + i] ? double(p[32 + i]) / p[48 + i] : 0.,
                    p[32 + i] ? double(p[40 + i]) / p[32 + i] : 0.);
    }
#endif
    if (s->knobs.profile == 2) {
        unsigned long long p[8];
        HIP_CHECK(hipMemcpy(p, s->slices[0].counters + kNumCounters, sizeof(p), hipMemcpyDeviceToHost));
        fprintf(stderr, "[wtgpu profile] heavy items %llu: clock ticks ray %llu probe %llu cone %llu total %llu (per item: ray %.0f probe %.0f cone %.0f total %.0f; cone+probe phase A %.0f phase B %.0f; phase-A steps %.1f entries %.1f)\n", p[4], p[0],
                p[1], p[2], p[3], p[4] ? double(p[0]) / p[4] : 0., p[4] ? double(p[1]) / p[4] : 0., p[4] ? double(p[2]) / p[4] : 0., p[4] ? double(p[3]) / p[4] : 0., p[4] ? double(p[5]) / p[4] : 0., p[4] ? double(p[6]) / p[4] : 0., p[4] ? double(p[7] & 0xffffffffull) / p[4] : 0., p[4] ? double(p[7] >> 32) / p[4] : 0.);
    }
    return WTGPU_OK;
}
int wtgpu_reset_counters(wtgpu_scene* s) {
    if (!s || !s->uploaded) return fail(WTGPU_ERR_INVALID, "scene not uploaded");
    {
        const int rc = drain_all(s);
        if (rc) return rc;
    }
    HIP_CHECK(hipDeviceSynchronize());
    HIP_CHECK(hipMemset(s->slices[0].counters, 0, (kNumCounters + kProfSlots + 1) * sizeof(unsigned long long)));
    s->samples_rendered = 0;
    s->cap_hits = 0;
    for (double& v : s->acc) v = 0;
    s->rounds_launched_total = 0;
    return WTGPU_OK;
}

int wtgpu_test_profile_counters(wtgpu_scene* s, unsigned long long* out, uint32_t n) {
    if (!s || !out || !s->uploaded || n > kProfSlots) return fail(WTGPU_ERR_INVALID, "wtgpu_test_profile_counters: uploaded scene, n <= kProfSlots");
    {
        const int rc = drain_all(s);
        if (rc) return rc;
    }
    HIP_CHECK(hipDeviceSynchronize());
    HIP_CHECK(hipMemcpy(out, s->slices[0].counters + kNumCounters, n * sizeof(unsigned long long), hipMemcpyDeviceToHost));
    return WTGPU_OK;
}

}
```

wave_tracer_amd/csrc/wtgpu_kernels.h:

```cpp
#pragma once
#include <hip/hip_runtime.h>

#include <cstddef>
#include <cstdint>
#include <cstring>

#include "../../include/wtgpu.h"
#include "wt/bdpt.h"
#include "wt/coop.h"
#include "wt/coop_fsd.h"
#include "wt/coop_utd.h"
#include "wt/path.h"

using namespace wt;
namespace wt {
struct tonemap_args_t;
struct film_polar_args_t;
struct film_denoise_args_t;
}

namespace wtk {


#ifndef WTGPU_LB_TRACE
#define WTGPU_LB_TRACE 3
#endif
#ifndef WTGPU_LB_HEAVY
#define WTGPU_LB_HEAVY 3
#endif
#ifndef WTGPU_LB_INTERACT
#define WTGPU_LB_INTERACT 3
#endif
#ifndef WTGPU_LB_INTERACT_B
#define WTGPU_LB_INTERACT_B 3
#endif
#ifndef WTGPU_LB_INTERACT_C
#define WTGPU_LB_INTERACT_C 3
#endif
#ifndef WTGPU_LB_FLUX
#define WTGPU_LB_FLUX 3
#endif
#ifndef WTGPU_LB_CONNECT
#define WTGPU_LB_CONNECT 2
#endif
constexpr uint32_t kFluxTaskTris = 2048;
constexpr int kBlock = 128;
#ifndef WTGPU_LDS_STACK
#define WTGPU_LDS_STACK 20
#endif
constexpr int kLdsStack = WTGPU_LDS_STACK;
constexpr uint32_t kConeBudget = 96;
constexpr int kSpillStack = 64 - kLdsStack;

enum : uint32_t { CTL_STRAT_HEAD_OPEN = 25, CTL_UTD_COUNT0 = 26, CTL_UTD_COUNT1 = 27, CTL_FSDQ_COUNT0 = 28, CTL_FSDQ_COUNT1 = 29, CTL_FSDQ_HEAD = 30, CTL_NEEQ_COUNT = 31, CTL_NEEQ_HEAD = 32, CTL_COUNT0 = 0, CTL_COUNT1 = 1, CTL_HEAD_TRACE = 2, CTL_HEAD_INTERACT = 3, CTL_HEAVY_COUNT = 4, CTL_HEAVY_HEAD = 5, CTL_FSD_COUNTER = 6,
                  CTL_ROUNDS = 7, CTL_STRAT_HEAD = 8, CTL_INTB_COUNT = 9, CTL_INTB_HEAD = 10, CTL_GATHER_COUNT = 11, CTL_GATHER_HEAD = 12, CTL_INTC_COUNT = 13, CTL_INTC_HEAD = 14, CTL_FTASK_COUNT = 15, CTL_FTASK_HEAD = 16, CTL_FSPLIT_HEAD = 17, CTL_EPOOL_COUNT = 18, CTL_FSD_ECOUNTER = 19, CTL_INTD_COUNT = 20, CTL_INTD_HEAD = 21, CTL_BACK0 = 22, CTL_BACK1 = 23,
                  CTL_TPOL_COUNT0 = 41, CTL_TPOL_COUNT1 = 42, CTL_TPOL_HEAD = 43, CTL_TCONE_COUNT0 = 44, CTL_TCONE_COUNT1 = 45, CTL_TCONE_HEAD = 46,
                  CTL_CLS_COUNT0 = 33, CTL_CLS_HEAD0 = 37,
                  CTL_LIGHT_DONE = 47, CTL_LIGHT_STOP = 48,
                  CTL_WORDS = 56 };
constexpr uint32_t kTriListWords = 128;
constexpr uint32_t kGatherMarker = 0xFFFFFFFEu;
constexpr uint32_t kApertureMarker = 0xFFFFFFFDu, kNullApertureMarker = 0xFFFFFFFCu;
__host__ __device__ inline bool is_region_marker(uint32_t t) { return t == kGatherMarker || t == kApertureMarker; }
constexpr uint32_t kKeyDim = kMaxVerts + 2, kNumKeys = kKeyDim * kKeyDim;
__host__ __device__ constexpr uint32_t class_key_work(uint32_t key) { return (key / kKeyDim) * (key % kKeyDim); }
__host__ __device__ constexpr uint32_t class_key_rank(uint32_t key) {
    uint32_t r = 0;
    for (uint32_t k = 0; k < kNumKeys; ++k)
        if (class_key_work(k) > class_key_work(key) || (class_key_work(k) == class_key_work(key) && k < key)) ++r;
    return r;
}
__host__ __device__ constexpr bool class_key_open(uint32_t key) { return key / kKeyDim == kKeyDim - 1 || key % kKeyDim == kKeyDim - 1; }
constexpr uint32_t kClassCount = kNumKeys + 1, kClassKey = kClassCount + kNumKeys, kClassTableWords = kClassKey + kNumKeys;

struct device_state_t {
    uint64_t cap = 0;
    uint32_t max_verts = 0;
    uint32_t walk_words = 0;
    size_t vert_words = 0;
    uint32_t* walks = nullptr;
    uint32_t* verts = nullptr;
    uint32_t* ctx = nullptr;
    uint32_t* trav = nullptr;
    uint32_t* tris = nullptr;
    uint32_t* queue[2] = {nullptr, nullptr};
    uint32_t* heavy_queue = nullptr;
    uint32_t* intb_queue = nullptr;
    uint32_t* gather_queue = nullptr;
    uint32_t* intc_queue = nullptr;
    uint32_t* intd_queue = nullptr;
    uint2* ftasks = nullptr;
    uint32_t ftask_cap = 0;
    double* facc = nullptr;
    uint32_t* epool = nullptr;
    uint32_t epool_cap = 0;
    uint32_t* ctl = nullptr;
    fsd_aperture_t* fsd_hdr = nullptr;
    fsd_edge_t* fsd_edges = nullptr;
    uint32_t fsd_cap = 0;
    uint32_t fsd_ecap = 0;
    uint32_t* strat_items = nullptr;
    uint32_t* strat_count = nullptr;
    uint32_t* strat_prefix = nullptr;
    double* lacc = nullptr;
    unsigned long long* counters = nullptr;
    const struct bdpt_ext_t* ext = nullptr;
};
struct bdpt_ext_t {
    const unsigned char* tri_class = nullptr;
    uint32_t* cls_queue = nullptr;
    struct conn_pending_t* pend = nullptr;
    uint32_t* surv = nullptr;
    uint32_t* chunk_ctl = nullptr;
    uint32_t pend_cap = 0, n_chunks = 0;
};
enum : uint32_t { CHUNK_EVAL_HEAD = 0, CHUNK_PEND_COUNT = 1, CHUNK_PEND_HEAD = 2, CHUNK_SURV_COUNT = 3, CHUNK_MIS_HEAD = 4, kChunkCtlWords = 8 };
struct conn_pending_t {
    uint32_t i;
    uint32_t st;
    float L[4];
    float o[3], d[3], dist;
};
struct path_state_t {
    utd_edge_rec_t* utd[2] = {nullptr, nullptr};
    uint32_t utd_cap = 0;
    uint32_t* fsdq[2] = {nullptr, nullptr};
    uint32_t* neeq = nullptr;
    float* fsd_f = nullptr;
    path_nee_rec_t* nee_recs = nullptr;
    uint2* gather_info = nullptr;
};
constexpr size_t kWalkWords = sizeof(walk_t) / 4;
constexpr size_t kCtxWords = sizeof(sample_ctx_t) / 4;
constexpr size_t kTravWords = sizeof(trav_result_t) / 4;
#define WT_TRAV_WORD(field) (offsetof(trav_result_t, field) / 4)
struct trace_stage_t {
    cone_t env;
    axis_walk_t aw;
};
constexpr size_t kStageWords = sizeof(trace_stage_t) / 4;
constexpr size_t kNumCounters = sizeof(bdpt_counters_t) / sizeof(unsigned long long);
constexpr size_t kProfSlots = 128;
constexpr size_t kDroppedSlot = kNumCounters + kProfSlots;


struct launch_args_t {
    scene_t sc;
    device_state_t st;
    film_t film;
    uint64_t seed;
    uint64_t j0;
    uint32_t nb;
    uint32_t npix;
    uint64_t sample_begin;
    uint32_t count_stats;
    uint32_t cone_budget;
    uint32_t flux_task_tris;
    uint32_t heavy_probe;
    uint32_t coop_aperture_min;
    uint32_t profile;
    uint32_t split_queues;
    uint32_t lane_cache, heavy_cache;
    uint32_t collect_list;
};

WT_D uint32_t* trace_stage_words(const launch_args_t& a) { return a.st.trav + kTravWords * 2 * (size_t)a.st.cap; }
WT_D uint32_t* trace_pol_queue(const launch_args_t& a) { return a.st.heavy_queue + 2 * (size_t)a.st.cap; }
WT_D uint32_t* trace_cone_queue(const launch_args_t& a) { return a.st.heavy_queue + 4 * (size_t)a.st.cap; }
WT_D void lds_stack(stack_entry_t* lds, stack_entry_t* spill, stack_ref_t& s, uint32_t block = kBlock) {
    s = make_stack_ref(lds + threadIdx.x, block, kLdsStack + kSpillStack, kLdsStack, spill);
}

WT_D void flush_counters(unsigned long long* g, const bdpt_counters_t& c) {
    const unsigned long long* p = reinterpret_cast<const unsigned long long*>(&c);
#pragma unroll
    for (size_t i = 0; i < kNumCounters; ++i) {
        unsigned long long v = p[i];
        for (int off = 32; off > 0; off >>= 1) v += __shfl_down(v, off, 64);
        if ((threadIdx.x & 63) == 0 && v) atomicAdd(&g[i], v);
    }
}

WT_D void walk_ident(const launch_args_t& a, uint32_t w, uint32_t& i, uint32_t& stream) {
    if (w < a.st.cap) {
        i = w;
        stream = STREAM_SENSOR_WALK;
    } else {
        i = w - (uint32_t)a.st.cap;
        stream = STREAM_EMITTER_WALK;
    }
}
WT_D uint32_t queue_count(const uint32_t* ctl, int in) { return ctl[CTL_COUNT0 + in] + ctl[CTL_BACK0 + in]; }
WT_D uint32_t queue_walk(const launch_args_t& a, const uint32_t* ctl, int in, uint32_t qi, int first_round) {
    if (first_round) return qi < a.nb ? qi : (uint32_t)a.st.cap + (qi - a.nb);
    const uint32_t front = ctl[CTL_COUNT0 + in];
    return qi < front ? a.st.queue[in][qi] : a.st.queue[in][2 * (size_t)a.st.cap - 1 - (qi - front)];
}
WT_D bool wave_first_lane() { return __builtin_amdgcn_mbcnt_hi(~0u, __builtin_amdgcn_mbcnt_lo(~0u, 0u)) == 0u; }
WT_D uint32_t wave_grab0(uint32_t* head, uint32_t inc) {
    __builtin_amdgcn_wave_barrier();
    uint32_t old = 0;
    if (wave_first_lane()) old = atomicAdd(head, inc);
    __builtin_amdgcn_wave_barrier();
    return (uint32_t)__builtin_amdgcn_readfirstlane((int)old);
}
WT_D uint32_t wave_grab(uint32_t* head) { return wave_grab0(head, 64u); }
WT_D uint32_t wave_grab_item(uint32_t* head) { return wave_grab0(head, 1u); }
WT_D uint32_t wave_bcast0(uint32_t v) {
    __builtin_amdgcn_wave_barrier();
    return (uint32_t)__builtin_amdgcn_readfirstlane((int)v);
}
WT_D void wave_append(uint32_t* queue, uint32_t* count, bool pred, uint32_t w) {
    const unsigned long long m = __ballot(pred);
    if (!m) return;
    const int lane = threadIdx.x & 63;
    const int leader = __ffsll((long long)m) - 1;
    uint32_t base = 0;
    if (lane == leader) base = atomicAdd(count, (uint32_t)__popcll(m));
    base = (uint32_t)__shfl((int)base, leader, 64);
    if (pred) queue[base + (uint32_t)__popcll(m & ((1ull << lane) - 1ull))] = w;
}

WT_D void queue_append(const launch_args_t& a, uint32_t* ctl, int out, bool pred, uint32_t w) {
    const bool back = pred && w >= a.st.cap && a.split_queues;
    wave_append(a.st.queue[out], ctl + CTL_COUNT0 + out, pred && !back, w);
    const unsigned long long m = __ballot(back);
    if (!m) return;
    const int lane = threadIdx.x & 63;
    const int leader = __ffsll((long long)m) - 1;
    uint32_t base = 0;
    if (lane == leader) base = atomicAdd(ctl + CTL_BACK0 + out, (uint32_t)__popcll(m));
    base = (uint32_t)__shfl((int)base, leader, 64);
    if (back) a.st.queue[out][2 * (size_t)a.st.cap - 1 - (base + (uint32_t)__popcll(m & ((1ull << lane) - 1ull)))] = w;
}

WT_D uint64_t sample_id_of(const launch_args_t& a, uint32_t i, uint32_t& pix) {
    const uint64_t j = a.j0 + i;
    pix = (uint32_t)(j % a.npix);
    const uint64_t smp = a.sample_begin + j / a.npix;
    return ((uint64_t)pix << 32) | (smp & 0xFFFFFFFFull);
}
WT_D uint64_t sample_id_of(const launch_args_t& a, uint32_t i) {
    uint32_t pix;
    return sample_id_of(a, i, pix);
}
WT_D fsd_pool_t fsd_pool_of(const launch_args_t& a) {
    return fsd_pool_t{a.st.fsd_hdr, a.st.fsd_edges, a.st.ctl + CTL_FSD_COUNTER, a.st.fsd_cap, a.st.ctl + CTL_FSD_ECOUNTER, a.st.fsd_ecap};
}
WT_D vertex_store_t walk_vertices(const launch_args_t& a, size_t w) { return vertex_store_t{a.st.verts, a.st.vert_words, w}; }
WT_D vertex_store_t sensor_vertices(const launch_args_t& a, uint32_t i) { return walk_vertices(a, i); }
WT_D vertex_store_t emitter_vertices(const launch_args_t& a, uint32_t i) { return walk_vertices(a, (size_t)a.st.cap + i); }
__host__ __device__ constexpr __attribute__((always_inline)) uint32_t bucket_of(const uint32_t* prefix, uint32_t idx, uint32_t n = kNumKeys) {
    uint32_t lo = 0, hi = n;
    while (hi - lo > 1) {
        const uint32_t mid = (lo + hi) >> 1;
        if (prefix[mid] <= idx)
            lo = mid;
        else
            hi = mid;
    }
    return lo;
}
namespace bucket_of_check {
constexpr uint32_t front[] = {0, 0, 0, 3, 5};
constexpr uint32_t middle[] = {0, 2, 2, 2, 5};
constexpr uint32_t back[] = {0, 3, 5, 5, 5};
constexpr uint32_t ranks[] = {0, 64, 64, 192, 256};
static_assert(bucket_of(front, 0, 4) == 2 && bucket_of(front, 2, 4) == 2 && bucket_of(front, 3, 4) == 3 && bucket_of(front, 4, 4) == 3, "empty buckets at the front");
static_assert(bucket_of(middle, 0, 4) == 0 && bucket_of(middle, 1, 4) == 0 && bucket_of(middle, 2, 4) == 3 && bucket_of(middle, 4, 4) == 3, "empty buckets in the middle");
static_assert(bucket_of(back, 0, 4) == 0 && bucket_of(back, 2, 4) == 0 && bucket_of(back, 3, 4) == 1 && bucket_of(back, 4, 4) == 1, "empty buckets at the end");
static_assert(bucket_of(ranks, 0, 4) == 0 && bucket_of(ranks, 64, 4) == 2 && bucket_of(ranks, 128, 4) == 2 && bucket_of(ranks, 192, 4) == 3, "classes start at multiples of 64");
static_assert(bucket_of(front, 0, 1) == 0, "one key");
}
#define WT_COUNTER_SLOT(field) (offsetof(bdpt_counters_t, field) / sizeof(unsigned long long))
WT_D void flush_counter(const launch_args_t& a, size_t slot, unsigned long long v) {
    for (int off = 32; off > 0; off >>= 1) v += __shfl_down(v, off, 64);
    if ((threadIdx.x & 63) == 0 && v) atomicAdd(a.st.counters + slot, v);
}
WT_D uint32_t& trav_word(const launch_args_t& a, uint32_t w, size_t word) { return a.st.trav[(size_t)w * kTravWords + word]; }
#define WT_TRAV_U(a, w, field) trav_word(a, w, WT_TRAV_WORD(field))
#define WT_TRAV_F(a, w, field) __uint_as_float(WT_TRAV_U(a, w, field))
WT_D vec3 trav_origin(const launch_args_t& a, uint32_t w) { return vec3{WT_TRAV_F(a, w, origin.x), WT_TRAV_F(a, w, origin.y), WT_TRAV_F(a, w, origin.z)}; }
WT_D uint32_t edges_to_pool(const launch_args_t& a, const gather_out_t& g, coop_edges_t& eg, uint32_t& n_edges, uint32_t& dropped) {
    const bool bitmap = a.sc.n_edges <= kCoopEdgeBits;
    n_edges = bitmap ? coop_edge_count(a.sc, eg) : g.n_edges;
    dropped = bitmap ? 0u : g.edge_overflow;
    const uint32_t off = wave_grab0(a.st.ctl + CTL_EPOOL_COUNT, n_edges);
    if (off + n_edges > a.st.epool_cap) {
        dropped += n_edges;
        n_edges = 0;
    } else if (bitmap)
        coop_edge_write(a.sc, eg, a.st.epool + off, n_edges);
    else
        for (uint32_t j = threadIdx.x; j < n_edges; j += 64) a.st.epool[off + j] = eg.edge_ids[j];
    return off;
}
WT_D void ctl_reset_batch(uint32_t* ctl) {
    ctl[CTL_COUNT1] = 0;
    ctl[CTL_BACK0] = ctl[CTL_BACK1] = 0;
    ctl[CTL_UTD_COUNT0] = ctl[CTL_UTD_COUNT1] = ctl[CTL_FSDQ_COUNT0] = ctl[CTL_FSDQ_COUNT1] = ctl[CTL_FSDQ_HEAD] = ctl[CTL_NEEQ_COUNT] = ctl[CTL_NEEQ_HEAD] = 0;
    ctl[CTL_HEAD_TRACE] = ctl[CTL_HEAD_INTERACT] = ctl[CTL_HEAVY_COUNT] = ctl[CTL_HEAVY_HEAD] = ctl[CTL_FSD_COUNTER] = ctl[CTL_ROUNDS] = 0;
    ctl[CTL_TPOL_COUNT0] = ctl[CTL_TPOL_COUNT1] = ctl[CTL_TPOL_HEAD] = ctl[CTL_TCONE_COUNT0] = ctl[CTL_TCONE_COUNT1] = ctl[CTL_TCONE_HEAD] = 0;
    ctl[CTL_INTB_COUNT] = ctl[CTL_INTB_HEAD] = ctl[CTL_GATHER_COUNT] = ctl[CTL_GATHER_HEAD] = ctl[CTL_INTC_COUNT] = ctl[CTL_INTC_HEAD] = 0;
    ctl[CTL_FTASK_COUNT] = ctl[CTL_FTASK_HEAD] = ctl[CTL_FSPLIT_HEAD] = ctl[CTL_EPOOL_COUNT] = ctl[CTL_FSD_ECOUNTER] = 0;
    ctl[CTL_INTD_COUNT] = ctl[CTL_INTD_HEAD] = 0;
}
WT_D void interact_round_begin(uint32_t* ctl) {
    ctl[CTL_HEAVY_COUNT] = 0;
    ctl[CTL_HEAVY_HEAD] = 0;
    ctl[CTL_HEAD_TRACE] = 0;
}

constexpr int kIoRows = 32;
template <int W>
constexpr int io_pitch() { return (W & 1) ? W : W + 1; }
template <int W, class T>
WT_D void wave_load_records(const uint32_t* base, size_t stride, uint32_t idx, bool valid, uint32_t* lds, T& out) {
    static_assert(sizeof(T) == 4 * W, "record size");
    constexpr int P = io_pitch<W>();
    const int lane = threadIdx.x & 63;
    uint32_t* o = reinterpret_cast<uint32_t*>(&out);
    const unsigned long long all = __ballot(valid);
#pragma unroll 1
    for (int h = 0; h < 2; ++h) {
        unsigned long long m = all & (h ? 0xFFFFFFFF00000000ull : 0x00000000FFFFFFFFull);
        while (m) {
            const int r = __ffsll((long long)m) - 1;
            m &= m - 1;
            const uint32_t* src = base + (size_t)__builtin_amdgcn_readlane(idx, r) * stride;
#pragma unroll
            for (int w0 = 0; w0 < W; w0 += 64)
                if (w0 + lane < W) lds[(r & 31) * P + w0 + lane] = src[w0 + lane];
        }
        __builtin_amdgcn_wave_barrier();
        if (valid && (lane >> 5) == h) {
#pragma unroll
            for (int i = 0; i < W; ++i) o[i] = lds[(lane & 31) * P + i];
        }
        __builtin_amdgcn_wave_barrier();
    }
}
template <int W, class T>
WT_D void wave_store_records(uint32_t* base, size_t stride, uint32_t idx, uint32_t off, bool valid, uint32_t* lds, const T& in) {
    static_assert(sizeof(T) == 4 * W, "record size");
    constexpr int P = io_pitch<W>();
    const int lane = threadIdx.x & 63;
    const uint32_t* o = reinterpret_cast<const uint32_t*>(&in);
    const unsigned long long all = __ballot(valid);
    if (!all) return;
#pragma unroll 1
    for (int h = 0; h < 2; ++h) {
        if (valid && (lane >> 5) == h) {
#pragma unroll
            for (int i = 0; i < W; ++i) lds[(lane & 31) * P + i] = o[i];
        }
        __builtin_amdgcn_wave_barrier();
        unsigned long long m = all & (h ? 0xFFFFFFFF00000000ull : 0x00000000FFFFFFFFull);
        while (m) {
            const int r = __ffsll((long long)m) - 1;
            m &= m - 1;
            uint32_t* dst = base + (size_t)__builtin_amdgcn_readlane(idx, r) * stride + __builtin_amdgcn_readlane(off, r);
#pragma unroll
            for (int w0 = 0; w0 < W; w0 += 64)
                if (w0 + lane < W) dst[w0 + lane] = lds[(r & 31) * P + w0 + lane];
        }
        __builtin_amdgcn_wave_barrier();
    }
}

constexpr uint32_t kFlushGrid = 64;
constexpr int kEnumBlock = 1024;
constexpr uint32_t kSplatBlock = 64, kSplatCols = kSplatBlock + 2;
constexpr uint32_t kSplatPhases = 6;
__host__ __device__ constexpr uint32_t splat_segments(uint32_t width) { return (width + kSplatBlock - 1) / kSplatBlock; }
__host__ __device__ constexpr uint32_t splat_phase_rows(uint32_t phase, uint32_t height) { return (height + 2u - phase / 2u) / 3u; }
__host__ __device__ constexpr uint32_t splat_phase_segments(uint32_t phase, uint32_t segs) { return (segs + 1u - (phase & 1u)) / 2u; }
__host__ __device__ constexpr uint32_t splat_block_row(uint32_t phase, uint32_t block, uint32_t phase_segs) { return phase / 2u + 3u * (block / phase_segs); }
__host__ __device__ constexpr uint32_t splat_block_segment(uint32_t phase, uint32_t block, uint32_t phase_segs) { return (phase & 1u) + 2u * (block % phase_segs); }
__host__ __device__ constexpr bool splat_phases_cover(uint32_t height, uint32_t segs) {
    uint32_t seen[8 * 8] = {};
    for (uint32_t phase = 0; phase < kSplatPhases; ++phase) {
        const uint32_t ps = splat_phase_segments(phase, segs), n = splat_phase_rows(phase, height) * ps;
        for (uint32_t b = 0; b < n; ++b) {
            const uint32_t r = splat_block_row(phase, b, ps), s = splat_block_segment(phase, b, ps);
            if (r >= height || s >= segs || r % 3u != phase / 2u || s % 2u != (phase & 1u)) return false;
            ++seen[r * 8 + s];
        }
    }
    for (uint32_t r = 0; r < height; ++r)
        for (uint32_t s = 0; s < segs; ++s)
            if (seen[r * 8 + s] != 1) return false;
    return true;
}
static_assert(splat_phases_cover(1, 1) && splat_phases_cover(2, 1) && splat_phases_cover(3, 2) && splat_phases_cover(4, 2) && splat_phases_cover(5, 3) && splat_phases_cover(6, 4) &&
              splat_phases_cover(7, 5) && splat_phases_cover(8, 8) && splat_phases_cover(7, 1) && splat_phases_cover(1, 6),
              "heights 0, 1, 2 mod 3; even and odd segment counts");
static_assert(splat_segments(1) == 1 && splat_segments(64) == 1 && splat_segments(65) == 2 && splat_segments(1440) == 23 && splat_segments(1920) == 30, "segments of a row");
#ifndef WTGPU_HARD_BLOCK
#define WTGPU_HARD_BLOCK 256
#endif
__global__ void k_generate(launch_args_t a);
__global__ void k_trace_refill(launch_args_t a, int in, int first_round, uint32_t round);
__global__ void k_trace_sm(launch_args_t a, int in, int first_round, uint32_t round);
__global__ void k_tr_axis(launch_args_t a, int in, int first_round, uint32_t round);
__global__ void k_tr_cone(launch_args_t a, uint32_t it);
__global__ void k_tr_policy(launch_args_t a, uint32_t it);
__global__ void k_tr_tail(launch_args_t a, uint32_t it);
__global__ void k_trace_heavy(launch_args_t a);
__global__ void k_trace_heavy_prof(launch_args_t a);
__global__ void k_interact(launch_args_t a, int in, int first_round);
__global__ void k_classify(launch_args_t a, int in, int first_round);
__global__ void k_interact_diffuse(launch_args_t a, int in);
__global__ void k_interact_dielectric(launch_args_t a, int in);
__global__ void k_interact_spm(launch_args_t a, int in);
__global__ void k_interact_any(launch_args_t a, int in);
__global__ void k_interact_sorted(launch_args_t a, int in);
__global__ void k_interact_coop(launch_args_t a, int in, int first_round);
__global__ void k_edges(launch_args_t a);
__global__ void k_interact_b(launch_args_t a, int in);
__global__ void k_light_rounds(launch_args_t a, int in, uint32_t round, uint32_t max_rounds);
__global__ void k_flux_split(launch_args_t a);
__global__ void k_flux_tasks(launch_args_t a);
__global__ void k_interact_c(launch_args_t a, int in);
__global__ void k_interact_c_hard(launch_args_t a, int in);
__global__ void k_path_generate(launch_args_t a);
__global__ void k_path_fsd(launch_args_t a, const path_state_t* __restrict__ ps, uint32_t round);
__global__ void k_path_edges(launch_args_t a, const path_state_t* __restrict__ ps);
__global__ void k_path_interact(launch_args_t a, const path_state_t* __restrict__ ps, int in, int first_round, uint32_t round);
__global__ void k_path_interact_b(launch_args_t a, const path_state_t* __restrict__ ps, int in, uint32_t round);
__global__ void k_path_nee(launch_args_t a, const path_state_t* __restrict__ ps, uint32_t round);
__global__ void k_path_flush(launch_args_t a, int in);
__global__ void k_connect_enum(launch_args_t a, uint32_t by_class);
__global__ void k_connect_scan(launch_args_t a, uint32_t by_class);
__global__ void k_connect_strat(launch_args_t a);
__global__ void k_connect_strat_open(launch_args_t a);
__global__ void k_connect_class(launch_args_t a);
__global__ void k_connect_class_open(launch_args_t a);
__global__ void k_connect_eval(launch_args_t a, uint32_t chunk);
__global__ void k_connect_shadow(launch_args_t a, uint32_t chunk);
__global__ void k_connect_mis(launch_args_t a, uint32_t chunk);
__global__ void k_connect_splat(launch_args_t a);
__global__ void k_connect_splat_tiled(launch_args_t a, uint32_t phase);
__global__ void k_calib_copy(const uint32_t* in, uint32_t* out, size_t n);
__global__ void k_trace_rays(scene_t sc, const float* rays, uint32_t n, float* dist, uint32_t* tuid, float* bary, uint32_t* front);
__global__ void k_traverse_cones(scene_t sc, const float* cones, uint32_t n, uint32_t cap, float* dist, uint32_t* flags, uint32_t* ntris, uint32_t* out_tris,
                                 uint32_t* scratch_tris);
__global__ void k_query_regions(scene_t sc, const float* cones, uint32_t n, uint32_t edge_cap, float* dist, uint32_t* flags, uint32_t* primary, uint32_t* ntris,
                                uint32_t* nedges, uint32_t* edges, float* flux, unsigned long long* dropped);
int test_fsd_apertures(const scene_t& sc, hipStream_t stream, const float* d_cones, const float* d_sk, const uint32_t* d_ids, const uint32_t* d_n_ids,
                       uint32_t n, uint32_t id_cap, uint32_t pool_cap, uint32_t mode, uint32_t* d_hdr, float* d_segs);
int test_utd_sums(const scene_t& sc, hipStream_t stream, const float* d_queries, const uint32_t* d_ids, const uint32_t* d_n_ids, uint32_t n, uint32_t id_cap,
                  uint32_t utd_cap, uint32_t* d_recs, uint32_t* d_hdr, uint32_t* d_edges);
int test_bsdf_queries(const scene_t& sc, hipStream_t stream, const uint32_t* d_queries, uint32_t n, int form, uint32_t* d_out);
int test_source_queries(const scene_t& sc, hipStream_t stream, const uint32_t* d_queries, uint32_t n, uint32_t* d_out);
int test_flux_queries(const scene_t& sc, hipStream_t stream, const uint32_t* d_queries, uint32_t n, uint32_t* d_out);
int sensor_mask_launch(const scene_t& sc, hipStream_t stream, const uint8_t* d_shape_matches, uint32_t samples, uint64_t seed, float* d_out);
void sensor_mask_host(const scene_t& sc, const uint8_t* shape_matches, uint32_t samples, uint64_t seed, uint32_t n_threads, float* out);
constexpr uint32_t kMaxTonemapTable = 1024;
int develop_launch(const sensor_t& sn, hipStream_t stream, const double* d_value, const double* d_weight, const double* d_light, uint64_t spe,
                   uint32_t per_pixel, float* d_out);
int develop_tonemap_launch(const sensor_t& sn, hipStream_t stream, const double* d_value, const double* d_weight, const double* d_light, uint64_t spe,
                           const tonemap_args_t& t, uint32_t s, const float* d_mask, uint32_t format, uint32_t lds_table, void* d_out);
void develop_tonemap_host(const sensor_t& sn, const double* value, const double* weight, const double* light, uint64_t spe, const tonemap_args_t& t, uint32_t s,
                          const float* mask, uint32_t format, uint32_t n_threads, void* out);
int film_stats_launch(const sensor_t& sn, hipStream_t stream, uint32_t n_cus, const double* d_value, const double* d_weight, const double* d_light, uint64_t spe, uint32_t s,
                      uint32_t flags, const float* d_mask, const float* d_edges, uint32_t bins, void* d_rec, unsigned long long* d_hist, double* d_sums);
void film_stats_host(const sensor_t& sn, const double* value, const double* weight, const double* light, uint64_t spe, uint32_t s, uint32_t flags, const float* mask,
                     const float* edges, uint32_t bins, uint32_t n_threads, void* out_rec, unsigned long long* out_hist);
size_t film_compare_wave_bytes(uint64_t npix, uint32_t n_cus);
int film_compare_launch(const sensor_t& sn, hipStream_t stream, uint32_t n_cus, const double* a_value, const double* a_weight, const double* a_light, uint64_t spe_a,
                        const double* b_value, const double* b_weight, const double* b_light, uint64_t spe_b, uint32_t s, uint32_t flags, double eps, const float* d_mask,
                        void* d_rec, double* d_sums, void* d_wave, float* d_diff);
void film_compare_host(const sensor_t& sn, const double* a_value, const double* a_weight, const double* a_light, uint64_t spe_a, const double* b_value,
                       const double* b_weight, const double* b_light, uint64_t spe_b, uint32_t s, uint32_t flags, double eps, const float* mask, uint32_t n_threads,
                       void* out_rec, float* diff);
size_t film_polar_wave_bytes(uint64_t npix, uint32_t n_cus);
int film_polar_launch(const sensor_t& sn, hipStream_t stream, uint32_t n_cus, const double* d_value, const double* d_weight, const double* d_light, uint64_t spe,
                      uint32_t flags, const film_polar_args_t& a, uint32_t staged, const float* d_mask, void* d_rec, double* d_sums, void* d_wave, float* d_maps,
                      void* d_picture);
void film_polar_host(const sensor_t& sn, const double* value, const double* weight, const double* light, uint64_t spe, uint32_t flags, const film_polar_args_t& a,
                     const float* mask, uint32_t n_threads, void* out_rec, float* maps, void* picture);
size_t film_denoise_scratch_floats(const sensor_t& sn);
int film_denoise_launch(const sensor_t& sn, hipStream_t stream, const double* a_value, const double* a_weight, const double* a_light, uint64_t spe_a,
                        const double* b_value, const double* b_weight, const double* b_light, uint64_t spe_b, const film_denoise_args_t& a, uint32_t fused,
                        const float* d_mask, float* d_scratch, float* d_out, float* d_residual);
void film_denoise_host(const sensor_t& sn, const double* a_value, const double* a_weight, const double* a_light, uint64_t spe_a, const double* b_value,
                       const double* b_weight, const double* b_light, uint64_t spe_b, const film_denoise_args_t& a, const float* mask, uint32_t n_threads,
                       float* out, float* residual);
void film_denoise_exp2_neg(const float* t, uint64_t n, float* out);

}
using namespace wtk;
```

wave_tracer_amd/csrc/wtgpu_knobs.h:

```cpp
#pragma once
#include <cstddef>
#include <cstdint>

struct knobs_t {
    uint32_t cone_budget, count_stats, split_queues, lane_cache, heavy_cache, heavy_probe, coop_aperture_min, flux_task_tris, profile, no_lists, primary_axis;
    uint32_t streams, state_gb, timing, conn_pool;
    uint32_t first_rounds, rounds_margin, light_rounds, max_rounds, stagger_round;
    uint32_t shrink_r1, shrink_f1, shrink_r2, shrink_f2, shrink_h1, decay_q, decay_c;
    uint32_t heavy_waves_per_cu, round_blocks_per_cu, grid_div_b, grid_div_c, grid_div_hard, grid_mul_flux;
    uint32_t sorted_interact, coop_io, staged_connect, connect_class, tiled_splat;
    uint32_t trace_staged, trace_stages, trace_staged_rounds, trace_sm, trace_ab;
    uint32_t develop_per_pixel, tonemap_lds_table, film_polar_staged, film_denoise_fused;
    uint32_t dbg_stage;
    uint32_t host_prof, trace_launch, tail_diag, trace_ab_verbose;
    uint32_t grid_div_cls[4];
};

enum knob_kind_t {
    KNOB_U32,
    KNOB_INT,
    KNOB_NONZERO,
    KNOB_PRESENT
};
struct knob_t {
    const char* name;
    uint32_t knobs_t::*field;
    knob_kind_t kind;
    long long dflt, lo, hi;
    const char* help;
};
#pragma GCC visibility push(hidden)
extern const knob_t kKnobs[];
extern const size_t kNumKnobs;
constexpr uint32_t kKnobConeBudget = 96, kKnobFluxTaskTris = 2048;

void read_knobs(knobs_t& k);
#pragma GCC visibility pop
```

wave_tracer_amd/csrc/wtgpu_knobs.hip:

```cpp
#include "wtgpu_knobs.h"

#include <algorithm>
#include <climits>
#include <cstdio>
#include <cstdlib>

#include "wt/bdpt.h"

using wt::kMaxWalkIters;
using wt::kWalkIterLimit;

#define K(field) &knobs_t::field
static constexpr long long kU32 = 0xFFFFFFFFll;
const knob_t kKnobs[] = {
    {"WTGPU_CONE_BUDGET", K(cone_budget), KNOB_U32, kKnobConeBudget, 0, kU32, "work units one lane may spend on a cone query before it is handed to a wavefront (wtgpu_kernels.h: kConeBudget)"},
    {"WTGPU_COUNT_STATS", K(count_stats), KNOB_U32, 1, 0, kU32, "0: the kernels keep no statistics (wtgpu_kernels.h: launch_args_t::count_stats)"},
    {"WTGPU_SPLIT_QUEUES", K(split_queues), KNOB_U32, 1, 0, kU32, "round queues keep sensor and emitter walks apart; 0: one mixed queue (A/B)"},
    {"WTGPU_LANE_CACHE", K(lane_cache), KNOB_U32, 1, 0, kU32, "0 (diagnostic): the per-lane traversal without its remembered rejecting triangles"},
    {"WTGPU_HEAVY_CACHE", K(heavy_cache), KNOB_U32, 1, 0, kU32, "0 (diagnostic): the wave-cooperative traversal without its remembered rejecting triangles"},
    {"WTGPU_HEAVY_PROBE", K(heavy_probe), KNOB_U32, 1, 0, kU32, "k_trace_heavy: any-hit probe of the near slab before the handed-over cone query too; 0: off"},
    {"WTGPU_COOP_APERTURE_MIN", K(coop_aperture_min), KNOB_U32, 8, 0, kU32, "segments from which an aperture is built by a wavefront; 0xFFFFFFFF: every aperture by a single lane of pass B"},
    {"WTGPU_FLUX_TASK_TRIS", K(flux_task_tris), KNOB_U32, kKnobFluxTaskTris, 64, kU32, "triangles per region-sum task (k_flux_split / k_flux_tasks; wtgpu_kernels.h: kFluxTaskTris)"},
    {"WTGPU_PROFILE", K(profile), KNOB_U32, 0, 0, kU32, "1 / 2 / 3: in-kernel clock breakdowns, printed by wtgpu_get_counters (wtgpu_counters.hip)"},
    {"WTGPU_NO_LISTS", K(no_lists), KNOB_PRESENT, 0, 0, 1, "set (any value; plt_bdpt, diagnostic): no bounded triangle lists, every interaction region is gathered"},
    {"WTGPU_PRIMARY_AXIS", K(primary_axis), KNOB_U32, 0, 0, kU32, "1 (plt_bdpt): the triangle under the beam axis of every diffusive hit comes from the trace kernels' axis query"},
    {"WTGPU_STREAMS", K(streams), KNOB_INT, 3, 1, INT_MAX, "state slices = internal streams; ms per pass at 1 / 2 / 3 / 4 / 6 / 8: 158 / 142 / 130 / 142 / 157 / 206 (headline)"},
    {"WTGPU_STATE_GB", K(state_gb), KNOB_INT, 224, 1, INT_MAX, "budget of the per-batch state of all slices, GB (of the MI355X's 288; never more than 85 % of what is free): deep scenes get smaller batches"},
    {"WTGPU_TIMING", K(timing), KNOB_NONZERO, 1, 0, 1, "0: no per-kernel HIP events (wtgpu_last_render_timings reads zeros)"},
    {"WTGPU_CONN_POOL", K(conn_pool), KNOB_U32, 16, 1, kU32, "staged connections: pending connections per sample of a chunk"},
    {"WTGPU_FIRST_ROUNDS", K(first_rounds), KNOB_U32, 0, 0, kMaxWalkIters, "rounds launched up front; 0: adaptive (the recent batches' mean + WTGPU_ROUNDS_MARGIN); tests use 2, 96 = as before round 4"},
    {"WTGPU_ROUNDS_MARGIN", K(rounds_margin), KNOB_U32, 2, 0, kU32, "rounds added to the recent batches' mean"},
    {"WTGPU_LIGHT_ROUNDS", K(light_rounds), KNOB_U32, 1, 0, kU32, "0: the rounds beyond the expected ones as ordinary rounds only (k_light_rounds off)"},
    {"WTGPU_MAX_ROUNDS", K(max_rounds), KNOB_U32, kWalkIterLimit, 8, kWalkIterLimit, "rounds a batch may get before its surviving walks are dropped and counted (CHANGES RESULTS below the default, wt/bdpt.h kWalkIterLimit: nothing is dropped in any workload seen; 96 = rounds 1-5)"},
    {"WTGPU_STAGGER_ROUND", K(stagger_round), KNOB_U32, 0, 0, kMaxWalkIters - 1, "r > 0 (diagnostic): a batch starts when the previous one has finished its round r; 0: all streams start at once.  4 streams, r = 0 / 3 / 6 / 10 / 16: 151 / 150 / 161 / 200 / 263 ms per pass"},
    {"WTGPU_SHRINK_R1", K(shrink_r1), KNOB_U32, 8, 0, kU32, "from this round on the round kernels' grids are divided by WTGPU_SHRINK_F1 (heavy: WTGPU_SHRINK_H1)"},
    {"WTGPU_SHRINK_F1", K(shrink_f1), KNOB_U32, 4, 1, kU32, "see WTGPU_SHRINK_R1"},
    {"WTGPU_SHRINK_R2", K(shrink_r2), KNOB_U32, 16, 0, kU32, "from this round on the grids are divided by WTGPU_SHRINK_F2 (heavy: 32)"},
    {"WTGPU_SHRINK_F2", K(shrink_f2), KNOB_U32, 32, 1, kU32, "see WTGPU_SHRINK_R2"},
    {"WTGPU_SHRINK_H1", K(shrink_h1), KNOB_U32, 4, 1, kU32, "see WTGPU_SHRINK_R1"},
    {"WTGPU_DECAY_Q", K(decay_q), KNOB_U32, 0, 0, kU32, "per cent; > 0: grids follow WTGPU_DECAY_C x q^round instead of the step schedule above"},
    {"WTGPU_DECAY_C", K(decay_c), KNOB_U32, 4, 1, kU32, "safety factor of the geometric schedule"},
    {"WTGPU_HEAVY_WAVES", K(heavy_waves_per_cu), KNOB_U32, 8, 1, kU32, "wavefronts per CU of the wave-per-item kernels; swept 6 / 8 / 10 / 12 / 16 / 24 / 32: 169.6 / 168.0 / 171.6 / 174.3 / 176 / 181 / 183 ms per pass"},
    {"WTGPU_ROUND_BLOCKS", K(round_blocks_per_cu), KNOB_U32, 8, 1, kU32, "blocks per CU of the round kernels' persistent grids"},
    {"WTGPU_GRID_B", K(grid_div_b), KNOB_U32, 4, 1, kU32, "pass B's grid relative to the round's (divisor)"},
    {"WTGPU_GRID_C", K(grid_div_c), KNOB_U32, 1, 1, kU32, "pass C's grid (divisor); 2 until round 4; 1: bidir_room 33.6 -> 33.9, cornell 25.15 -> 25.35 Msamples/s, pass C's bracket 69 -> 56 / 93 -> 65 ms"},
    {"WTGPU_GRID_HARD", K(grid_div_hard), KNOB_U32, 4, 1, kU32, "k_interact_c_hard's grid (divisor)"},
    {"WTGPU_GRID_FLUX", K(grid_mul_flux), KNOB_U32, 2, 1, kU32, "k_flux_tasks' grid (multiplier)"},
    {"WTGPU_SORTED_INTERACT", K(sorted_interact), KNOB_U32, 0, 0, kU32, "pass A: 0 k_interact (one kernel, every walk); 1 k_classify + one kernel per material class; 2 k_classify + k_interact_sorted"},
    {"WTGPU_COOP_IO", K(coop_io), KNOB_U32, 0, 0, kU32, "1: pass A with wave-cooperative record transfers (k_interact_coop)"},
    {"WTGPU_STAGED_CONNECT", K(staged_connect), KNOB_U32, 0, 0, kU32, "connections: 0 k_connect_strat (one kernel per strategy item); 1 k_connect_eval -> k_connect_shadow -> k_connect_mis, in chunks"},
    {"WTGPU_CONNECT_CLASS", K(connect_class), KNOB_U32, 1, 0, kU32, "connections (the one-kernel form): 0 k_connect_strat (an item is one strategy of a sample); 1 k_connect_class (an item is a sample, bucketed by the lengths of its subpaths, all of its strategies in a row; DESIGN.md §4)"},
    {"WTGPU_TILED_SPLAT", K(tiled_splat), KNOB_U32, 1, 0, kU32, "0: the plain per-sample splat kernel"},
    {"WTGPU_TRACE_STAGED", K(trace_staged), KNOB_U32, 1, 0, kU32, "1: the traversal in stages (k_tr_axis / k_tr_cone / k_tr_policy / k_tr_tail) ..."},
    {"WTGPU_TRACE_STAGES", K(trace_stages), KNOB_U32, 3, 1, 16, "... with this many cone stages before the tail ..."},
    {"WTGPU_TRACE_STAGED_ROUNDS", K(trace_staged_rounds), KNOB_U32, 4, 0, kU32, "... for the first so many rounds of a batch (the long ones: a stage is a launch, and a short round is bound by its launches)"},
    {"WTGPU_TRACE_SM", K(trace_sm), KNOB_U32, 0, 0, kU32, "1: the phase-machine trace kernel (k_trace_sm)"},
    {"WTGPU_TRACE_AB", K(trace_ab), KNOB_U32, 0, 0, kU32, "n: the first n rounds replay their trace queue through both trace kernels, timed, outputs compared (wtgpu_trace_ab.hip)"},
    {"WTGPU_DEVELOP_PER_PIXEL", K(develop_per_pixel), KNOB_U32, 0, 0, 1, "k_develop: 0 one lane per plane element; 1 one lane per pixel (A/B: tools/bench_develop.py)"},
    {"WTGPU_TONEMAP_LDS_TABLE", K(tonemap_lds_table), KNOB_U32, 0, 0, 1, "k_develop_tonemap: 1 every block stages the colour table in LDS; 0 the lanes read it through the caches (A/B: tools/bench_develop.py)"},
    {"WTGPU_FILM_POLAR_STAGED", K(film_polar_staged), KNOB_U32, 1, 0, 1, "k_film_polar: 1 a wavefront loads its chunk's planes contiguously, develops them and hands them to the pixels' lanes through LDS; 0 every lane loads its own pixels' planes (A/B: tools/bench_film_polar.py)"},
    {"WTGPU_FILM_DENOISE_FUSED", K(film_denoise_fused), KNOB_U32, 2, 0, 2, "k_denoise_filter: 1 a block filters both directions (A by B's weights, B by A's) in one launch and keeps the first in registers; 0 one launch per direction, the first leaving its result in scratch memory; 2 whichever was measured faster for the film's planes: 1 up to 4 planes, 0 for 12 (A/B: tools/bench_film_denoise.py)"},
    {"WTGPU_DEBUG_STAGE", K(dbg_stage), KNOB_INT, 1 << 30, INT_MIN, INT_MAX, "bring-up aid: stops launching the round kernels after stage n (INVALID RESULTS)"},
    {"WTGPU_HOST_PROF", K(host_prof), KNOB_PRESENT, 0, 0, 1, "set: host time spent inside each kind of launch call, printed per render call"},
    {"WTGPU_TRACE_LAUNCH", K(trace_launch), KNOB_PRESENT, 0, 0, 1, "set (bring-up aid): every launch is named and waited for — the last line names a kernel that hangs"},
    {"WTGPU_TAIL_DIAG", K(tail_diag), KNOB_PRESENT, 0, 0, 1, "set: why the host was called back for a pending batch, printed at exit (DESIGN.md §9)"},
    {"WTGPU_TRACE_AB_VERBOSE", K(trace_ab_verbose), KNOB_PRESENT, 0, 0, 1, "set: one line per round replayed by WTGPU_TRACE_AB"},
};
#undef K
const size_t kNumKnobs = sizeof(kKnobs) / sizeof(kKnobs[0]);

void read_knobs(knobs_t& k) {
    for (size_t i = 0; i < kNumKnobs; ++i) {
        const knob_t& d = kKnobs[i];
        const char* e = getenv(d.name);
        long long v = d.dflt;
        if (d.kind == KNOB_PRESENT) v = e ? 1 : 0;
        else if (e && d.kind == KNOB_U32) v = std::min<long long>(std::max<long long>(0, strtoll(e, nullptr, 10)), kU32);
        else if (e && d.kind == KNOB_INT) v = atoi(e);
        else if (e) v = atoi(e) != 0;
        k.*d.field = (uint32_t)std::min(d.hi, std::max(d.lo, v));
    }
    unsigned v[4] = {1, 4, 2, 4};
    if (const char* e = getenv("WTGPU_GRID_CLS")) sscanf(e, "%u,%u,%u,%u", &v[0], &v[1], &v[2], &v[3]);
    for (int c = 0; c < 4; ++c) k.grid_div_cls[c] = std::max(1u, v[c]);
}
```

wave_tracer_amd/csrc/wtgpu_upload.hip:

```cpp
#include "wtgpu_host.h"

static int g_env_by_host = 0;
__attribute__((constructor)) static void wtgpu_runtime_settings() {
    if (getenv("HSA_KERNARG_POOL_SIZE")) g_env_by_host |= 1;
    setenv("HSA_KERNARG_POOL_SIZE", "16777216", 0);
}
static int runtime_settings_ok(std::string& why) {
    const char* k = getenv("HSA_KERNARG_POOL_SIZE");
    const long ring = k ? atol(k) : (1l << 20);
    if (getenv("WTGPU_ALLOW_SLOW_RUNTIME")) return 1;
    if (ring < (4l << 20)) {
        why = "HSA_KERNARG_POOL_SIZE=" + std::string(k ? k : "(unset)") + ": a batch enqueues ~900 launches of ~1 KB of kernel arguments; with a ring below 4 MiB the enqueueing "
              "thread blocks and the streams serialise; export HSA_KERNARG_POOL_SIZE=16777216 before the HIP runtime initialises, or WTGPU_ALLOW_SLOW_RUNTIME=1";
        return 0;
    }
    if (!(g_env_by_host & 1) && !getenv("WTGPU_QUIET")) {
        static bool told = false;
        if (!told) fprintf(stderr, "[wtgpu] note: HSA_KERNARG_POOL_SIZE=16777216 defaulted by libwtgpu.so; effective only if the HIP runtime had not initialised before the library was loaded "
                           "(a host that uses HIP earlier exports it itself, INTEGRATION.md)\n");
        told = true;
    }
    return 1;
}

static int upload_scene_arrays(wtgpu_scene* s) {
    const scene_t& h = s->host;
    scene_t d = h;
    int rc;
#define UP(field, n) \
    if ((rc = upload(s, h.field, (size_t)(n), &d.field)) != WTGPU_OK) return rc;
    {
        d.tri_geo = nullptr;
        if (h.n_tris > 0 && h.tri_geo) {
            const size_t nt = h.n_tris;
            std::vector<float> sph(4 * nt);
            for (size_t i = 0; i < nt; ++i) tri_bounding_sphere(h.tri_geo[i].a, h.tri_geo[i].b, h.tri_geo[i].c, &sph[4 * i]);
            void* p = nullptr;
            HIP_CHECK(hipMalloc(&p, nt * (sizeof(tri_geo_t) + 16)));
            s->dev_allocs.push_back(p);
            HIP_CHECK(hipMemcpy(p, h.tri_geo, nt * sizeof(tri_geo_t), hipMemcpyHostToDevice));
            HIP_CHECK(hipMemcpy(static_cast<char*>(p) + nt * sizeof(tri_geo_t), sph.data(), nt * 16, hipMemcpyHostToDevice));
            d.tri_geo = static_cast<const tri_geo_t*>(p);
        }
    }
    UP(tri_meta, h.n_tris)
    UP(tri_shade, h.n_tris)
    UP(edges, h.n_edges)
    {
        d.nodes = nullptr;
        if (h.n_nodes > 0 && h.nodes) {
            const size_t nn = h.n_nodes;
            vec3 mn{WT_INF, WT_INF, WT_INF}, mx{-WT_INF, -WT_INF, -WT_INF};
            for (size_t i = 0; i < nn; ++i)
                for (int c = 0; c < 8; ++c)
                    if (h.nodes[i].child[c] != 0) {
                        mn = vmin(mn, vec3{h.nodes[i].minx[c], h.nodes[i].miny[c], h.nodes[i].minz[c]});
                        mx = vmax(mx, vec3{h.nodes[i].maxx[c], h.nodes[i].maxy[c], h.nodes[i].maxz[c]});
                    }
            const qgrid_t g = qgrid_make(mn, mx);
            std::vector<bvh8_qnode_t> qn(nn);
            bool ok = finitef(mn.x) && finitef(mn.y) && finitef(mn.z) && finitef(mx.x) && finitef(mx.y) && finitef(mx.z);
            for (size_t i = 0; i < nn && ok; ++i) ok = qnode_make(h.nodes[i], g, qn[i]);
            if (!ok) return fail(WTGPU_ERR_INVALID, "the scene's BVH boxes cannot be enclosed by the 16-bit node grid (non-finite or out-of-range box)");
            const float gw[8] = {g.origin.x, g.origin.y, g.origin.z, g.cell.x, g.cell.y, g.cell.z, 0.f, 0.f};
            void* p = nullptr;
            HIP_CHECK(hipMalloc(&p, nn * (sizeof(bvh8_node_t) + sizeof(bvh8_qnode_t)) + sizeof(gw)));
            s->dev_allocs.push_back(p);
            HIP_CHECK(hipMemcpy(p, h.nodes, nn * sizeof(bvh8_node_t), hipMemcpyHostToDevice));
            HIP_CHECK(hipMemcpy(static_cast<char*>(p) + nn * sizeof(bvh8_node_t), qn.data(), nn * sizeof(bvh8_qnode_t), hipMemcpyHostToDevice));
            HIP_CHECK(hipMemcpy(static_cast<char*>(p) + nn * (sizeof(bvh8_node_t) + sizeof(bvh8_qnode_t)), gw, sizeof(gw), hipMemcpyHostToDevice));
            d.nodes = static_cast<const bvh8_node_t*>(p);
        }
    }
    UP(leaves, h.n_leaves)
    UP(shapes, h.n_shapes)
    const scene_extents_t ex = scene_extents(h);
    UP(shape_tri_tuid, ex.shape_tris)
    UP(shape_tri_cdf, ex.shape_tris + h.n_shapes)
    UP(materials, h.n_materials)
    UP(spectra, h.n_spectra)
    UP(spectra_data, ex.spec_words)
    UP(textures, h.n_textures)
    for (uint32_t i = 0; i < h.n_emitters; ++i)
        if (h.emitters[i].type == EMIT_AREA && h.emitters[i].radiance_tex > 0) {
            const emitter_t& e = h.emitters[i];
            if ((uint32_t)e.radiance_tex > h.n_textures || h.textures[e.radiance_tex - 1].type != TEX_BITMAP || e.shape < 0 || (uint32_t)e.shape >= h.n_shapes ||
                e.tab_words < h.shapes[e.shape].tri_count * 5ull + 1)
                return fail(WTGPU_ERR_INVALID, "area emitter " + std::to_string(i) + ": radiance_tex must name a bitmap texture and tab / tab_words the emitter's sampling tables (wt/sources.h area_table_*)");
        }
    UP(texture_data, ex.tex_words)
    UP(emitters, h.n_emitters)
    UP(emitter_cdf, h.n_emitters + 1)
    UP(kdists, h.n_emitters)
    UP(kdist_data, ex.kd_words)
    if ((rc = upload(s, h.lut.icdf_theta1, h.lut.m ? h.lut.n_theta : 0, &d.lut.icdf_theta1)) != WTGPU_OK) return rc;
    if ((rc = upload(s, h.lut.icdf_theta2, h.lut.m ? h.lut.n_theta : 0, &d.lut.icdf_theta2)) != WTGPU_OK) return rc;
    if ((rc = upload(s, h.lut.icdf1, (size_t)h.lut.m * h.lut.m, &d.lut.icdf1)) != WTGPU_OK) return rc;
    if ((rc = upload(s, h.lut.icdf2, (size_t)h.lut.m * h.lut.m, &d.lut.icdf2)) != WTGPU_OK) return rc;
#undef UP
    s->dev = d;
    s->d_tri_class = nullptr;
    if (h.n_tris > 0 && h.opts.integrator == INTEGRATOR_BDPT) {
        std::vector<unsigned char> cls(h.n_tris);
        for (uint32_t t = 0; t < h.n_tris; ++t) cls[t] = (unsigned char)walk_class_of_triangle(h, t);
        if ((rc = upload(s, cls.data(), cls.size(), &s->d_tri_class)) != WTGPU_OK) return rc;
    }
    return WTGPU_OK;
}

static int alloc_slice(wtgpu_scene* s, uint32_t k, uint64_t batch_cap, unsigned long long* counters) {
    const scene_t& h = s->host;
    int rc;
    device_state_t& st = s->slices[k];
    st.cap = batch_cap;
    st.max_verts = (uint32_t)h.opts.max_depth + 2;
    st.walk_words = (uint32_t)(h.opts.integrator != INTEGRATOR_BDPT ? kPathWalkWords : kWalkWords);
    st.vert_words = (size_t)st.max_verts * kVertexWords;
    st.counters = counters;
    const size_t W2 = 2 * (size_t)st.cap;
    const bool path_mode = h.opts.integrator != INTEGRATOR_BDPT;
    if ((rc = dmalloc(s, &st.walks, (path_mode ? kPathWalkWords : kWalkWords) * W2))) return rc;
    {
        path_state_t P;
        P.utd_cap = path_mode ? (uint32_t)std::min<uint64_t>(48ull * st.cap + 65536, 1ull << 28) : 1u;
        for (int q = 0; q < 2; ++q) {
            if ((rc = dmalloc(s, &P.utd[q], (size_t)P.utd_cap))) return rc;
            if ((rc = dmalloc(s, &P.fsdq[q], path_mode ? (size_t)st.cap : 1))) return rc;
        }
        if ((rc = dmalloc(s, &P.neeq, path_mode ? (size_t)st.cap : 1))) return rc;
        if ((rc = dmalloc(s, &P.fsd_f, path_mode ? (size_t)st.cap : 1))) return rc;
        if ((rc = dmalloc(s, &P.nee_recs, path_mode ? (size_t)st.cap : 1))) return rc;
        if ((rc = dmalloc(s, &P.gather_info, path_mode ? (size_t)st.cap : 1))) return rc;
        path_state_t* dP = nullptr;
        if ((rc = dmalloc(s, &dP, 1))) return rc;
        HIP_CHECK(hipMemcpy(dP, &P, sizeof(P), hipMemcpyHostToDevice));
        s->d_path_slices.push_back(dP);
    }
    if (!path_mode) {
        bdpt_ext_t X;
        X.tri_class = s->d_tri_class;
        if (s->knobs.sorted_interact && (rc = dmalloc(s, &X.cls_queue, (size_t)kNumWalkClasses * W2))) return rc;
        X.pend_cap = (uint32_t)std::min<uint64_t>((uint64_t)s->knobs.conn_pool * st.cap + 4096, 0xFFFFFF00ull);
        if (s->knobs.staged_connect) {
            uint64_t pairs = 0;
            const int md = h.opts.max_depth;
            for (int t = 0; t <= md + 2; ++t)
                for (int q = 0; q <= md + 2; ++q)
                    if (t + q - 2 >= 0 && t + q - 2 <= md && !(t == 1 && q == 1)) ++pairs;
            X.n_chunks = (uint32_t)((pairs * st.cap + X.pend_cap - 1) / X.pend_cap);
            if ((rc = dmalloc(s, &X.pend, (size_t)X.pend_cap))) return rc;
            if ((rc = dmalloc(s, &X.surv, (size_t)X.pend_cap))) return rc;
            if ((rc = dmalloc(s, &X.chunk_ctl, (size_t)X.n_chunks * kChunkCtlWords))) return rc;
        } else
            X.pend_cap = 0;
        s->pend_cap = X.pend_cap;
        s->n_chunks = X.n_chunks;
        bdpt_ext_t* dX = nullptr;
        if ((rc = dmalloc(s, &dX, 1))) return rc;
        HIP_CHECK(hipMemcpy(dX, &X, sizeof(X), hipMemcpyHostToDevice));
        st.ext = dX;
    }
    if ((rc = dmalloc(s, &st.verts, path_mode ? 1 : (size_t)st.max_verts * kVertexWords * W2))) return rc;
    if ((rc = dmalloc(s, &st.ctx, kCtxWords * (size_t)st.cap))) return rc;
    if ((rc = dmalloc(s, &st.trav, (kTravWords + kStageWords) * W2))) return rc;
    if ((rc = dmalloc(s, &st.tris, (size_t)kTriListWords * W2))) return rc;
    if ((rc = dmalloc(s, &st.queue[0], W2))) return rc;
    if ((rc = dmalloc(s, &st.queue[1], W2))) return rc;
    if ((rc = dmalloc(s, &st.heavy_queue, 3 * W2))) return rc;
    if ((rc = dmalloc(s, &st.intb_queue, W2))) return rc;
    if ((rc = dmalloc(s, &st.gather_queue, W2))) return rc;
    if ((rc = dmalloc(s, &st.intc_queue, W2))) return rc;
    if ((rc = dmalloc(s, &st.intd_queue, W2))) return rc;
    st.ftask_cap = path_mode ? 1u : (1u << 22);
    if ((rc = dmalloc(s, &st.ftasks, (size_t)st.ftask_cap))) return rc;
    if ((rc = dmalloc(s, &st.facc, path_mode ? 1 : W2))) return rc;
    st.epool_cap = 1u << 23;
    if ((rc = dmalloc(s, &st.epool, (size_t)st.epool_cap))) return rc;
    if ((rc = dmalloc(s, &st.ctl, (size_t)CTL_WORDS))) return rc;
    HIP_CHECK(hipMemset(st.ctl, 0, CTL_WORDS * sizeof(uint32_t)));
    st.fsd_cap = (h.opts.FSD && !h.opts.force_ray_tracing && !path_mode) ? (uint32_t)std::min<uint64_t>(W2, 1u << 22) : 1u;
    if ((rc = dmalloc(s, &st.fsd_hdr, st.fsd_cap))) return rc;
    st.fsd_ecap = st.fsd_cap > 1 ? (uint32_t)std::min<uint64_t>(64ull * st.cap + kFsdMaxEdges, 1ull << 28) : 1u;
    if ((rc = dmalloc(s, &st.fsd_edges, (size_t)st.fsd_ecap))) return rc;
    if ((rc = dmalloc(s, &st.strat_items, path_mode ? 1 : (size_t)kNumKeys * st.cap))) return rc;
    if ((rc = dmalloc(s, &st.strat_count, (size_t)kNumKeys))) return rc;
    if ((rc = dmalloc(s, &st.strat_prefix, (size_t)kClassTableWords))) return rc;
    if ((rc = dmalloc(s, &st.lacc, 4 * (size_t)st.cap))) return rc;
    HIP_CHECK(hipMemset(st.strat_count, 0, kNumKeys * sizeof(uint32_t)));
    HIP_CHECK(hipStreamCreateWithFlags(&s->streams[k], hipStreamNonBlocking));
    HIP_CHECK(hipEventCreateWithFlags(&s->ev_done[k], hipEventDisableTiming));
    return WTGPU_OK;
}

static uint64_t size_batches(const wtgpu_scene* s, uint64_t max_batch, uint32_t& n_slices) {
    const scene_t& h = s->host;
    const uint64_t npix = (uint64_t)h.sensor.width * h.sensor.height;
    n_slices = s->knobs.streams;
    uint64_t batch_cap = max_batch ? std::min<uint64_t>(max_batch, 1u << 24) : std::min<uint64_t>(npix, 1u << 22);
    n_slices = (uint32_t)std::min<uint64_t>(n_slices, std::max<uint64_t>(1, batch_cap / 64));
    {
        const bool pm = h.opts.integrator != INTEGRATOR_BDPT;
        const uint64_t mv = (uint64_t)h.opts.max_depth + 2;
        uint64_t per_sample = 4ull * (2 * ((pm ? kPathWalkWords : kWalkWords) + (pm ? 0 : mv * kVertexWords) + kTravWords + kStageWords + 2 + kTriListWords) + kCtxWords) + 64ull * 28ull + 2048ull;
        if (pm) per_sample += 2ull * 48ull * sizeof(utd_edge_rec_t) + sizeof(path_nee_rec_t) + 3ull * 4ull + 4ull + sizeof(uint2);
        else per_sample += (s->knobs.staged_connect ? (uint64_t)s->knobs.conn_pool * (sizeof(conn_pending_t) + 4ull) : 0ull) + (s->knobs.sorted_interact ? 4ull * 2ull * kNumWalkClasses : 0ull);
        uint64_t budget = (uint64_t)s->knobs.state_gb << 30;
        size_t free_b = 0, total_b = 0;
        if (hipMemGetInfo(&free_b, &total_b) == hipSuccess && free_b > 0) budget = std::min<uint64_t>(budget, (uint64_t)((double)free_b * 0.85));
        const uint64_t fixed = (uint64_t)n_slices * ((1ull << 23) * 4ull + (1ull << 22) * 8ull + (64ull << 20));
        budget = budget > 2 * fixed ? budget - fixed : budget / 2;
        const uint64_t fit = std::max<uint64_t>(4096, budget / per_sample / n_slices);
        if (batch_cap > fit) batch_cap = fit;
    }
    return batch_cap;
}

static int upload_impl(wtgpu_scene* s, uint64_t max_batch) {
    read_knobs(s->knobs);
    int n_cu = 256;
    (void)hipDeviceGetAttribute(&n_cu, hipDeviceAttributeMultiprocessorCount, s->device);
    s->n_cus = (uint32_t)std::max(1, n_cu);
    int rc;
    if ((rc = upload_scene_arrays(s)) != WTGPU_OK) return rc;
    uint32_t n_slices = 0;
    const uint64_t batch_cap = size_batches(s, max_batch, n_slices);
    unsigned long long* counters = nullptr;
    if ((rc = dmalloc(s, &counters, kNumCounters + kProfSlots + 1))) return rc;
    HIP_CHECK(hipMemset(counters, 0, (kNumCounters + kProfSlots + 1) * sizeof(unsigned long long)));
    s->slices.resize(n_slices);
    s->streams.resize(n_slices);
    s->ev_done.resize(n_slices);
    for (uint32_t k = 0; k < n_slices; ++k)
        if ((rc = alloc_slice(s, k, batch_cap, counters)) != WTGPU_OK) return rc;
    HIP_CHECK(hipEventCreateWithFlags(&s->ev_begin, hipEventDisableTiming));
    s->recs.resize(4 * (size_t)n_slices);
    s->pending.assign(n_slices, wtgpu_scene::pending_t{});
    for (auto& r : s->recs) {
        r.ev.resize(s->knobs.timing ? 3 + 6 * (size_t)kMaxWalkIters : 1);
        for (auto& e : r.ev) HIP_CHECK(hipEventCreate(&e));
        HIP_CHECK(hipHostMalloc((void**)&r.h_ctl, CTL_WORDS * sizeof(uint32_t), hipHostMallocDefault));
        HIP_CHECK(hipHostMalloc((void**)&r.h_mid, CTL_WORDS * sizeof(uint32_t), hipHostMallocDefault));
        HIP_CHECK(hipEventCreateWithFlags(&r.ev_mid, hipEventDisableTiming));
        HIP_CHECK(hipEventCreateWithFlags(&r.ev_stagger, hipEventDisableTiming));
    }
    s->uploaded = true;
    return WTGPU_OK;
}

void release_device(wtgpu_scene* s) {
    if (s->device < 0) return;
    device_guard_t guard(s->device);
    (void)hipDeviceSynchronize();
    for (void* p : s->dev_allocs) (void)hipFree(p);
    s->dev_allocs.clear();
    for (auto& r : s->recs) {
        for (auto& e : r.ev)
            if (e) (void)hipEventDestroy(e);
        if (r.h_ctl) (void)hipHostFree(r.h_ctl);
        if (r.h_mid) (void)hipHostFree(r.h_mid);
        if (r.ev_mid) (void)hipEventDestroy(r.ev_mid);
        if (r.ev_stagger) (void)hipEventDestroy(r.ev_stagger);
    }
    s->recs.clear();
    s->pending.clear();
    for (auto& e : s->ev_done)
        if (e) (void)hipEventDestroy(e);
    s->ev_done.clear();
    s->ev_stagger_last = nullptr;
    if (s->ev_begin) (void)hipEventDestroy(s->ev_begin);
    s->ev_begin = nullptr;
    for (auto& st_ : s->streams)
        if (st_) (void)hipStreamDestroy(st_);
    s->streams.clear();
    s->slices.clear();
    s->d_path_slices.clear();
    s->d_tri_class = nullptr;
    s->pend_cap = s->n_chunks = 0;
    s->d_mask_flags = nullptr;
    if (s->h_mask_flags) (void)hipHostFree(s->h_mask_flags);
    s->h_mask_flags = nullptr;
    if (s->ev_mask) (void)hipEventDestroy(s->ev_mask);
    s->ev_mask = nullptr;
    s->d_tm_table = nullptr;
    if (s->h_tm_table) (void)hipHostFree(s->h_tm_table);
    s->h_tm_table = nullptr;
    if (s->ev_tm) (void)hipEventDestroy(s->ev_tm);
    s->ev_tm = nullptr;
    film_scratch_free(s->fs);
    film_scratch_free(s->fc);
    film_scratch_free(s->fp);
    s->d_denoise = nullptr;
    s->uploaded = false;
}

extern "C" {

int wtgpu_scene_upload(wtgpu_scene* s, int device, uint64_t max_batch) {
    if (!s) return fail(WTGPU_ERR_INVALID, "null scene");
    if (s->uploaded) return fail(WTGPU_ERR_INVALID, "scene already uploaded");
    {
        std::string why;
        if (!runtime_settings_ok(why)) return fail(WTGPU_ERR_INVALID, why);
    }
    int ndev = 0;
    const hipError_t dc = hipGetDeviceCount(&ndev);
    if (dc != hipSuccess || ndev == 0)
        return fail(WTGPU_ERR_NO_DEVICE, std::string("no HIP device present (there is no CPU fallback): hipGetDeviceCount -> ") + hipGetErrorString(dc) +
                                             ", count " + std::to_string(ndev));
    if (device < 0 || device >= ndev) return fail(WTGPU_ERR_NO_DEVICE, "invalid device index");
    device_guard_t guard(device);
    s->device = device;
    const int rc_up = upload_impl(s, max_batch);
    if (rc_up != WTGPU_OK) release_device(s);
    return rc_up;
}

}
```

Before: 32.44.

## Split pass C into prep, wide, hard-tries and commit tiers with per-lane walks

Replaces the single wavefront-per-walk pass C with a tiered pipeline. A prep kernel puts eight lanes on each walk to sum the triangle flux and run tries 0-7, settling most walks early. The rest go to wide and hard kernels that only run tries, and a commit kernel finishes the walk step with one lane per walk. The aim is to stop wasting 64 lanes on walks that accept within a few tries. In exchange it adds kernel launches, extra queues and outcome records written into the tris buffer, a larger intd_queue allocation, and profiling counters.

Result: faster. 33.03 (median of 6 runs) (+1.8%).

```diff
diff --git a/wave_tracer_amd/api.py b/wave_tracer_amd/api.py
--- a/wave_tracer_amd/api.py
+++ b/wave_tracer_amd/api.py
@@ -821,6 +821,12 @@
         _check(load_library().wtgpu_test_profile_counters(self._h, out, n))
         return [int(v) for v in out]
 
+    def pass_c_tiers(self):
+        p = self.profile_counters(224)
+        rounds = p[164]
+        return {"prep": p[160], "wide": p[161], "hard": p[162], "walks": p[163], "rounds": rounds, "rounds_not_multiple_of_8": p[165],
+                "rounds_shorter_than_8": p[166], "queue_lengths": p[168:168 + min(rounds, 56)]}
+
     def connect_class_items(self, slice=0, max_items=1 << 22):
         import numpy as np
         lib = load_library()
diff --git a/wave_tracer_amd/csrc/kernels_fsd.hip b/wave_tracer_amd/csrc/kernels_fsd.hip
--- a/wave_tracer_amd/csrc/kernels_fsd.hip
+++ b/wave_tracer_amd/csrc/kernels_fsd.hip
@@ -230,4 +230,330 @@
 __global__ void __launch_bounds__(64, WTGPU_LB_INTERACT_C) k_interact_c(launch_args_t a, int in) { interact_c_body<64>(a, in); }
 __global__ void __launch_bounds__(WTGPU_HARD_BLOCK) k_interact_c_hard(launch_args_t a, int in) { interact_c_body<WTGPU_HARD_BLOCK>(a, in); }
 
-}
+template <int BLOCK, bool THIN>
+WT_D void interact_c_tries_body(const launch_args_t& a, uint32_t easy_tries);
+__global__ void __launch_bounds__(64, WTGPU_LB_INTERACT_C) k_interact_c_prep(launch_args_t a, uint32_t thin_below, uint32_t easy_tries) {
+    uint32_t* ctl = a.st.ctl;
+    const uint32_t n = ctl[CTL_INTC_COUNT];
+    const int lane = threadIdx.x & 63;
+    const uint32_t s = (uint32_t)lane & (kPrepTries - 1u), group = (uint32_t)lane / kPrepTries;
+    const fsd_pool_t pool = fsd_pool_of(a);
+    uint32_t* wide_queue = pass_c_wide_queue(a);
+    uint32_t* commit_queue = pass_c_commit_queue(a);
+    unsigned long long* prof = a.st.counters + kNumCounters;
+    unsigned long long settled = 0;
+    if (a.count_stats && blockIdx.x == 0 && threadIdx.x == 0 && n > 0) {
+        atomicAdd(prof + kPassCWalksSlot, (unsigned long long)n);
+        const unsigned long long r = atomicAdd(prof + kPassCRoundsSlot, 1ull);
+        if (n % kPrepTries) atomicAdd(prof + kPassCRoundsSlot + 1, 1ull);
+        if (n < kPrepTries) atomicAdd(prof + kPassCRoundsSlot + 2, 1ull);
+        if (r < kPassCQueueSlots) prof[kPassCQueueSlot + r] = n;
+    }
+    if (n <= thin_below) {
+        interact_c_tries_body<64, true>(a, easy_tries);
+        return;
+    }
+    for (;;) {
+        const long long pl0 = a.profile == 3 ? clock64() : 0;
+        const uint32_t base0 = wave_grab0(ctl + CTL_INTC_HEAD, 64u / kPrepTries);
+        if (base0 >= n) break;
+        const uint32_t item = base0 + group;
+        const bool have = item < n;
+        uint32_t w = 0, slot = 0, base = 0, max_tries = 0;
+        fsd_aperture_t ap;
+        memset(&ap, 0, sizeof(ap));
+        sampler_t ss = make_sampler(a.seed, 0, 0, 0);
+        bool marker = false;
+        double flux = 0.0;
+        if (have) {
+            w = a.st.intc_queue[item];
+            uint32_t i, stream;
+            walk_ident(a, w, i, stream);
+            const uint64_t sample_id = sample_id_of(a, i);
+            const uint32_t rng_draws = a.st.walks[(size_t)w * a.st.walk_words + WT_WALK_WORD(rng_draws)];
+            slot = WT_TRAV_U(a, w, by);
+            ap = pool.hdr[slot];
+            ss = make_sampler(a.seed, sample_id, stream, 0);
+            base = fsd_tries_base(make_sampler(a.seed, sample_id, stream, rng_draws));
+            const uint32_t tr_tuid = WT_TRAV_U(a, w, tuid);
+            marker = is_region_marker(tr_tuid);
+            if (marker) {
+                flux = a.st.facc[w];
+            } else {
+                const walk_trace_in_t wk = walk_load_trace_in(a.st.walks, a.st.walk_words, w);
+                const cone_t benv = wk.env;
+                const float tr_dist = WT_TRAV_F(a, w, dist), tr_depth = WT_TRAV_F(a, w, region_depth);
+                const uint32_t tr_ntris = WT_TRAV_U(a, w, ntris);
+                const bool tr_front = WT_TRAV_U(a, w, front_face) != 0;
+                const range_t izr{tr_dist, tr_dist + tr_depth};
+                const vec2 axes = cone_axes(benv, tr_dist);
+                const vec2 sigma{axes.x / kBeamEnvelope, axes.y / kBeamEnvelope};
+                const frame_t bframe = cone_frame(benv);
+                const uint32_t* tl = a.st.tris + (size_t)w * kTriListWords;
+                double t0 = 0.0, t1 = 0.0, t2 = 0.0, t3 = 0.0, t4 = 0.0, t5 = 0.0, t6 = 0.0, t7 = 0.0;
+#pragma unroll 1
+                for (uint32_t k = 0; s + kPrepTries * k < tr_ntris && k < 8u; ++k) {
+                    const double f = (double)region_triangle_flux(a.sc, bframe, benv, izr, sigma, tl[s + kPrepTries * k], tr_front);
+                    t0 = k == 0u ? f : t0;
+                    t1 = k == 1u ? f : t1;
+                    t2 = k == 2u ? f : t2;
+                    t3 = k == 3u ? f : t3;
+                    t4 = k == 4u ? f : t4;
+                    t5 = k == 5u ? f : t5;
+                    t6 = k == 6u ? f : t6;
+                    t7 = k == 7u ? f : t7;
+                }
+                flux = ((t0 + t4) + (t2 + t6)) + ((t1 + t5) + (t3 + t7));
+            }
+        }
+        double fsum = flux;
+#pragma unroll
+        for (int off = (int)kPrepTries / 2; off > 0; off >>= 1) fsum += __shfl_xor(fsum, off, 64);
+        if (!marker) flux = fsum;
+        if (have) {
+            const float I = (float)(1.0 - flux);
+            ap.recp_I = I > 0.f ? 1.f / I : 0.f;
+            if (s == 0u) pool.hdr[slot] = ap;
+            max_tries = fsd_max_tries(ap);
+        }
+        const long long pc0 = a.profile == 3 ? clock64() : 0;
+        fsd_try_t r{{0.f, 0.f}, 0.f, 0u};
+        if (have && s < max_tries) r = fsd_try(a.sc, ap, fsd_edges_ref_t{pool.edges + (size_t)ap.edge_offset, 1}, sampler_at(ss, base + s * kFsdDrawsPerTry));
+        const uint32_t am = (uint32_t)(__ballot(r.accept != 0) >> (group * kPrepTries)) & ((1u << kPrepTries) - 1u);
+        const bool acc = am != 0u;
+        const uint32_t t_acc = acc ? (uint32_t)__ffs((int)am) - 1u : 0u;
+        const int wl = (int)(group * kPrepTries + t_acc);
+        const float rx = __shfl(r.x.x, wl, 64), ry = __shfl(r.x.y, wl, 64), rf = __shfl(r.f, wl, 64);
+        const bool lead = have && s == 0u;
+        const bool settle = lead && (acc || max_tries <= kPrepTries);
+        if (settle) {
+            uint32_t* o = pass_c_outcome(a, w);
+            o[0] = acc ? (kOutcomeAccepted | t_acc) : 0u;
+            o[1] = __float_as_uint(rx);
+            o[2] = __float_as_uint(ry);
+            o[3] = __float_as_uint(rf);
+            ++settled;
+        }
+        wave_append(commit_queue, ctl + CTL_PCC_COUNT, settle, w);
+        wave_append(wide_queue, ctl + CTL_PCW_COUNT, lead && !settle, w);
+        if (a.profile == 3) {
+            const long long pt = clock64();
+            const long long ng = (long long)__popcll(__ballot(lead));
+            if (lead) {
+                const int bin = 31 - __clz((int)max(ap.n_edges, 1u));
+                atomicAdd(prof + 8 + bin, 1ull);
+                atomicAdd(prof + 24 + bin, (unsigned long long)(acc ? t_acc + 1u : min(max_tries, kPrepTries)));
+                atomicAdd(prof + 112 + bin, (unsigned long long)((pc0 - pl0) / ng));
+                atomicAdd(prof + 40 + bin, (unsigned long long)((pt - pc0) / ng));
+            }
+        }
+    }
+    if (a.count_stats) flush_counter(a, kNumCounters + kPassCTierSlot, settled);
+}
+
+template <int BLOCK, bool THIN>
+WT_D void interact_c_tries_body(const launch_args_t& a, uint32_t easy_tries) {
+    constexpr bool HARD = BLOCK > 64;
+    static_assert(!(HARD && THIN), "thin rounds: one wavefront per walk");
+    __shared__ uint32_t s_item;
+    __shared__ uint32_t s_tmin;
+    __shared__ float s_res[3];
+    __shared__ fsd_edge_t s_seg[kStageSegs];
+    uint32_t* ctl = a.st.ctl;
+    const uint32_t n = ctl[HARD ? CTL_INTD_COUNT : (THIN ? CTL_INTC_COUNT : CTL_PCW_COUNT)];
+    const uint32_t* queue_in = HARD ? a.st.intd_queue : (THIN ? a.st.intc_queue : pass_c_wide_queue(a));
+    uint32_t* commit_queue = pass_c_commit_queue(a);
+    unsigned long long* prof = a.st.counters + kNumCounters;
+    const int tid = threadIdx.x;
+    const fsd_pool_t pool = fsd_pool_of(a);
+    unsigned long long settled = 0, settled_early = 0;
+    for (;;) {
+        uint32_t item = 0;
+        if (HARD) {
+            __syncthreads();
+            if (tid == 0) s_item = atomicAdd(ctl + CTL_INTD_HEAD, 1u);
+            __syncthreads();
+            item = s_item;
+        } else
+            item = wave_grab_item(ctl + (THIN ? CTL_INTC_HEAD : CTL_PCW_HEAD));
+        if (item >= n) break;
+        const uint32_t w = queue_in[item];
+        uint32_t i, stream;
+        walk_ident(a, w, i, stream);
+        const uint64_t sample_id = sample_id_of(a, i);
+        const uint32_t rng_draws = a.st.walks[(size_t)w * a.st.walk_words + WT_WALK_WORD(rng_draws)];
+        const uint32_t slot = WT_TRAV_U(a, w, by);
+        fsd_aperture_t ap = pool.hdr[slot];
+        const fsd_edges_ref_t ed = fsd_pool_edges(pool, slot);
+        const long long pc0 = a.profile == 3 ? clock64() : 0;
+        if (THIN) {
+            const walk_trace_in_t wk = walk_load_trace_in(a.st.walks, a.st.walk_words, w);
+            const cone_t benv = wk.env;
+            const float tr_dist = WT_TRAV_F(a, w, dist), tr_depth = WT_TRAV_F(a, w, region_depth);
+            const uint32_t tr_tuid = WT_TRAV_U(a, w, tuid), tr_ntris = WT_TRAV_U(a, w, ntris);
+            const bool tr_front = WT_TRAV_U(a, w, front_face) != 0;
+            const range_t izr{tr_dist, tr_dist + tr_depth};
+            const vec2 axes = cone_axes(benv, tr_dist);
+            const vec2 sigma{axes.x / kBeamEnvelope, axes.y / kBeamEnvelope};
+            double flux;
+            if (is_region_marker(tr_tuid)) {
+                flux = a.st.facc[w];
+            } else {
+                const uint32_t* tl = a.st.tris + (size_t)w * kTriListWords;
+                flux = (uint32_t)tid < tr_ntris ? (double)region_triangle_flux(a.sc, cone_frame(benv), benv, izr, sigma, tl[tid], tr_front) : 0.0;
+#pragma unroll
+                for (int off = 32; off > 0; off >>= 1) flux += __shfl_xor(flux, off, 64);
+            }
+            const float I = (float)(1.0 - flux);
+            ap.recp_I = I > 0.f ? 1.f / I : 0.f;
+            if (tid == 0) pool.hdr[slot] = ap;
+        }
+        const sampler_t ss = make_sampler(a.seed, sample_id, stream, 0);
+        const uint32_t base = fsd_tries_base(make_sampler(a.seed, sample_id, stream, rng_draws));
+        const uint32_t max_tries = fsd_max_tries(ap);
+        const uint32_t t_begin = HARD ? easy_tries : (THIN ? 0u : kPrepTries), t_end = HARD ? max_tries : (max_tries < easy_tries ? max_tries : easy_tries);
+        bool acc = false;
+        uint32_t t_acc = 0;
+        float rx = 0.f, ry = 0.f, rf = 0.f;
+        auto run_tries = [&](const fsd_edges_ref_t& edr) {
+            for (uint32_t t0 = t_begin; t0 < t_end && !acc; t0 += BLOCK) {
+                const uint32_t t = t0 + (uint32_t)tid;
+                fsd_try_t r{{0.f, 0.f}, 0.f, 0u};
+                if (t < t_end) r = fsd_try(a.sc, ap, edr, sampler_at(ss, base + t * kFsdDrawsPerTry));
+                if (!HARD) {
+                    const unsigned long long am = __ballot(r.accept != 0);
+                    if (am) {
+                        const int wl = __ffsll((long long)am) - 1;
+                        rx = __shfl(r.x.x, wl, 64);
+                        ry = __shfl(r.x.y, wl, 64);
+                        rf = __shfl(r.f, wl, 64);
+                        t_acc = t0 + (uint32_t)wl;
+                        acc = true;
+                    }
+                } else {
+                    if (tid == 0) s_tmin = 0xFFFFFFFFu;
+                    __syncthreads();
+                    if (r.accept) atomicMin(&s_tmin, t);
+                    __syncthreads();
+                    const uint32_t tm = s_tmin;
+                    if (tm != 0xFFFFFFFFu) {
+                        if (t == tm) {
+                            s_res[0] = r.x.x;
+                            s_res[1] = r.x.y;
+                            s_res[2] = r.f;
+                        }
+                        __syncthreads();
+                        rx = s_res[0];
+                        ry = s_res[1];
+                        rf = s_res[2];
+                        t_acc = tm;
+                        acc = true;
+                    }
+                    __syncthreads();
+                }
+            }
+        };
+        if (t_begin >= t_end) {
+        } else if (ap.n_edges <= kStageSegs) {
+            __syncthreads();
+            for (uint32_t k = (uint32_t)tid; k < ap.n_edges; k += BLOCK) s_seg[k] = ed.p[k];
+            __syncthreads();
+            run_tries(fsd_edges_ref_t{s_seg, 1});
+        } else
+            run_tries(ed);
+        if (a.profile == 3 && tid == 0) {
+            const int bin = 31 - __clz((int)max(ap.n_edges, 1u));
+            atomicAdd(prof + (THIN ? 8 : 144) + bin, 1ull);
+            atomicAdd(prof + 24 + bin, (unsigned long long)(acc ? t_acc + 1u - t_begin : t_end - t_begin));
+            atomicAdd(prof + (THIN ? 40 : 128) + bin, (unsigned long long)(clock64() - pc0));
+        }
+        if (tid == 0) {
+            if (!HARD && !acc && t_end < max_tries) {
+                a.st.intd_queue[atomicAdd(ctl + CTL_INTD_COUNT, 1u)] = w;
+            } else {
+                uint32_t* o = pass_c_outcome(a, w);
+                o[0] = acc ? (kOutcomeAccepted | t_acc) : 0u;
+                o[1] = __float_as_uint(rx);
+                o[2] = __float_as_uint(ry);
+                o[3] = __float_as_uint(rf);
+                commit_queue[atomicAdd(ctl + CTL_PCC_COUNT, 1u)] = w;
+                if (THIN && (acc ? t_acc < kPrepTries : max_tries <= kPrepTries))
+                    ++settled_early;
+                else
+                    ++settled;
+            }
+        }
+    }
+    if (a.count_stats && tid == 0 && settled) atomicAdd(prof + kPassCTierSlot + (HARD ? 2 : 1), settled);
+    if (THIN && a.count_stats && tid == 0 && settled_early) atomicAdd(prof + kPassCTierSlot, settled_early);
+}
+__global__ void __launch_bounds__(64, WTGPU_LB_INTERACT_C) k_interact_c_wide(launch_args_t a, uint32_t easy_tries) { interact_c_tries_body<64, false>(a, easy_tries); }
+__global__ void __launch_bounds__(WTGPU_HARD_BLOCK) k_interact_c_hard_tries(launch_args_t a, uint32_t easy_tries) { interact_c_tries_body<WTGPU_HARD_BLOCK, false>(a, easy_tries); }
+
+__global__ void __launch_bounds__(kBlock, WTGPU_LB_INTERACT_B) k_interact_c_commit(launch_args_t a, int in) {
+    uint32_t* ctl = a.st.ctl;
+    const uint32_t n = ctl[CTL_PCC_COUNT];
+    const uint32_t* commit_queue = pass_c_commit_queue(a);
+    bdpt_counters_t ctr;
+    memset(&ctr, 0, sizeof(ctr));
+    const fsd_pool_t pool = fsd_pool_of(a);
+    for (;;) {
+        const uint32_t base0 = wave_grab(ctl + CTL_PCC_HEAD);
+        if (base0 >= n) break;
+        const uint32_t qi = base0 + (threadIdx.x & 63);
+        const bool valid = qi < n;
+        bool cont = false;
+        uint32_t w = 0;
+        const long long pm0 = a.profile == 3 ? clock64() : 0;
+        int bin = 0;
+        if (valid) {
+            w = commit_queue[qi];
+            uint32_t i, stream;
+            walk_ident(a, w, i, stream);
+            const uint64_t sample_id = sample_id_of(a, i);
+            walk_t wk;
+            soa_load(a.st.walks, a.st.walk_words, w, wk);
+            trav_result_t tr;
+            soa_load(a.st.trav, kTravWords, w, tr);
+            const uint32_t slot = __float_as_uint(tr.by);
+            const fsd_aperture_t ap = pool.hdr[slot];
+            const uint32_t* o = pass_c_outcome(a, w);
+            const uint32_t o0 = o[0];
+            const bool acc = (o0 & kOutcomeAccepted) != 0u;
+            const uint32_t t_acc = o0 & ~kOutcomeAccepted;
+            const float rx = __uint_as_float(o[1]), ry = __uint_as_float(o[2]), rf = __uint_as_float(o[3]);
+            const uint32_t base = fsd_tries_base(make_sampler(a.seed, sample_id, stream, wk.rng_draws));
+            const uint32_t max_tries = fsd_max_tries(ap);
+            bin = 31 - __clz((int)max(ap.n_edges, 1u));
+            fsd_defer_t defer;
+            defer.defer_sampling = defer.to_sampling_pass = 0;
+            defer.have_aperture = 1;
+            defer.split_no_primary = 0;
+            defer.known_no_primary = 1;
+            defer.no_primary = 0;
+            defer.has_gather = defer.gather_n_edges = defer.gather_edge_overflow = 0;
+            defer.gather_flux = 0.f;
+            defer.gather_edges = nullptr;
+            defer.pending = 0;
+            defer.resolved = 1;
+            defer.slot = slot;
+            defer.base = base;
+            defer.next_try = 0;
+            defer.fs = fsd_finalize(ap, acc, vec2{rx, ry}, rf);
+            defer.end_draws = fsd_draws_after(base, acc ? t_acc : max_tries - 1u);
+            const uint_list_t tris{a.st.tris + (size_t)w * kTriListWords, 1u, kMaxConeTris};
+            const vertex_store_t vs = walk_vertices(a, w);
+            cont = bdpt_walk_step<2>(a.sc, wk, tr, tris, vs, pool, a.seed, sample_id, stream, &ctr, nullptr, &defer);
+            wk.active = cont ? 1u : 0u;
+            soa_store(a.st.walks, a.st.walk_words, w, wk);
+        }
+        if (a.profile == 3) {
+            const long long dt = clock64() - pm0, nv = (long long)__popcll(__ballot(valid));
+            if (valid) atomicAdd(a.st.counters + kNumCounters + 96 + bin, (unsigned long long)(dt / nv));
+        }
+        queue_append(a, ctl, 1 - in, cont, w);
+    }
+    if (a.count_stats) flush_counters(a.st.counters, ctr);
+}
+
+}
diff --git a/wave_tracer_amd/csrc/kernels_trace_refill.h b/wave_tracer_amd/csrc/kernels_trace_refill.h
--- a/wave_tracer_amd/csrc/kernels_trace_refill.h
+++ b/wave_tracer_amd/csrc/kernels_trace_refill.h
@@ -33,6 +33,7 @@
     ctl[CTL_EPOOL_COUNT] = 0;
     ctl[CTL_INTD_COUNT] = 0;
     ctl[CTL_INTD_HEAD] = 0;
+    ctl[CTL_PCW_COUNT] = ctl[CTL_PCW_HEAD] = ctl[CTL_PCC_COUNT] = ctl[CTL_PCC_HEAD] = 0;
 #pragma unroll
     for (uint32_t c = 0; c < kNumWalkClasses; ++c) ctl[CTL_CLS_COUNT0 + c] = ctl[CTL_CLS_HEAD0 + c] = 0;
     ctl[CTL_UTD_COUNT0 + (round & 1u)] = 0;
diff --git a/wave_tracer_amd/csrc/wtgpu.hip b/wave_tracer_amd/csrc/wtgpu.hip
--- a/wave_tracer_amd/csrc/wtgpu.hip
+++ b/wave_tracer_amd/csrc/wtgpu.hip
@@ -166,8 +166,17 @@
             HP_LAUNCH(k_flux_split, dim3(std::max<uint32_t>(1u, gh / 4u)), dim3(64), 0, st_, a);
             HP_LAUNCH(k_flux_tasks, dim3(std::max<uint32_t>(1u, gh * grid_mul_flux)), dim3(64), 0, st_, a);
             rec(r, st_);
-            HP_LAUNCH(k_interact_c, dim3(std::max<uint32_t>(1u, gh / grid_div_c)), dim3(64), 0, st_, a, in);
-            HP_LAUNCH(k_interact_c_hard, dim3(std::max<uint32_t>(1u, gh / K.grid_div_hard)), dim3(WTGPU_HARD_BLOCK), 0, st_, a, in);
+            if (K.pass_c_tiers) {
+                const uint32_t g_prep = std::max<uint32_t>(1u, gh / grid_div_c);
+                const uint32_t thin_below = (uint32_t)std::min<uint64_t>((uint64_t)K.pass_c_thin * g_prep, 0xFFFFFFFFull);
+                HP_LAUNCH(k_interact_c_prep, dim3(g_prep), dim3(64), 0, st_, a, thin_below, K.pass_c_easy_tries);
+                HP_LAUNCH(k_interact_c_wide, dim3(std::max<uint32_t>(1u, gh / grid_div_c)), dim3(64), 0, st_, a, K.pass_c_easy_tries);
+                HP_LAUNCH(k_interact_c_hard_tries, dim3(std::max<uint32_t>(1u, gh / K.grid_div_hard)), dim3(WTGPU_HARD_BLOCK), 0, st_, a, K.pass_c_easy_tries);
+                HP_LAUNCH(k_interact_c_commit, dim3(std::max<uint32_t>(1u, g0 / grid_div_b)), dim3(kBlock), 0, st_, a, in);
+            } else {
+                HP_LAUNCH(k_interact_c, dim3(std::max<uint32_t>(1u, gh / grid_div_c)), dim3(64), 0, st_, a, in);
+                HP_LAUNCH(k_interact_c_hard, dim3(std::max<uint32_t>(1u, gh / K.grid_div_hard)), dim3(WTGPU_HARD_BLOCK), 0, st_, a, in);
+            }
             rec(r, st_);
         }
         r.rounds_launched = r_end;
diff --git a/wave_tracer_amd/csrc/wtgpu_counters.hip b/wave_tracer_amd/csrc/wtgpu_counters.hip
--- a/wave_tracer_amd/csrc/wtgpu_counters.hip
+++ b/wave_tracer_amd/csrc/wtgpu_counters.hip
@@ -60,6 +60,12 @@
         fprintf(stderr, "[wtgpu profile] pass C by aperture size (slice 0): bin=log2(segments) items tries/item kticks/item total-Mticks\n");
         for (int b = 0; b < 16; ++b)
             if (p[8 + b]) fprintf(stderr, "[wtgpu profile]   C %2d %8llu %10.1f %10.1f %10.1f   fetch+load %.1f commit %.1f kticks/item\n", b, p[8 + b], double(p[24 + b]) / p[8 + b], double(p[40 + b]) / p[8 + b] * 1e-3, double(p[40 + b]) * 1e-6, double(p[112 + b]) / p[8 + b] * 1e-3, double(p[96 + b]) / p[8 + b] * 1e-3);
+        if (s->knobs.pass_c_tiers) {
+            fprintf(stderr, "[wtgpu profile] pass C in tiers (slice 0): walks settled by prep %llu, wide %llu, hard %llu; wide + hard tries by aperture size: bin items kticks/item total-Mticks\n",
+                    p[kPassCTierSlot], p[kPassCTierSlot + 1], p[kPassCTierSlot + 2]);
+            for (int b = 0; b < 16; ++b)
+                if (p[144 + b]) fprintf(stderr, "[wtgpu profile]   W %2d %8llu %10.1f %10.1f\n", b, p[144 + b], double(p[128 + b]) / p[144 + b] * 1e-3, double(p[128 + b]) * 1e-6);
+        }
         fprintf(stderr, "[wtgpu profile] pass B by gathered scene edges: bin items kticks/item total-Mticks\n");
         for (int b = 0; b < 16; ++b)
             if (p[56 + b]) fprintf(stderr, "[wtgpu profile]   B %2d %8llu %10.1f %10.1f\n", b, p[56 + b], double(p[72 + b]) / p[56 + b] * 1e-3, double(p[72 + b]) * 1e-6);
diff --git a/wave_tracer_amd/csrc/wtgpu_kernels.h b/wave_tracer_amd/csrc/wtgpu_kernels.h
--- a/wave_tracer_amd/csrc/wtgpu_kernels.h
+++ b/wave_tracer_amd/csrc/wtgpu_kernels.h
@@ -57,6 +57,7 @@
                   CTL_TPOL_COUNT0 = 41, CTL_TPOL_COUNT1 = 42, CTL_TPOL_HEAD = 43, CTL_TCONE_COUNT0 = 44, CTL_TCONE_COUNT1 = 45, CTL_TCONE_HEAD = 46,
                   CTL_CLS_COUNT0 = 33, CTL_CLS_HEAD0 = 37,
                   CTL_LIGHT_DONE = 47, CTL_LIGHT_STOP = 48,
+                  CTL_PCW_COUNT = 49, CTL_PCW_HEAD = 50, CTL_PCC_COUNT = 51, CTL_PCC_HEAD = 52,
                   CTL_WORDS = 56 };
 constexpr uint32_t kTriListWords = 128;
 constexpr uint32_t kGatherMarker = 0xFFFFFFFEu;
@@ -140,7 +141,7 @@
 };
 constexpr size_t kStageWords = sizeof(trace_stage_t) / 4;
 constexpr size_t kNumCounters = sizeof(bdpt_counters_t) / sizeof(unsigned long long);
-constexpr size_t kProfSlots = 128;
+constexpr size_t kProfSlots = 224;
 constexpr size_t kDroppedSlot = kNumCounters + kProfSlots;
 
 
@@ -167,6 +168,12 @@
 WT_D uint32_t* trace_stage_words(const launch_args_t& a) { return a.st.trav + kTravWords * 2 * (size_t)a.st.cap; }
 WT_D uint32_t* trace_pol_queue(const launch_args_t& a) { return a.st.heavy_queue + 2 * (size_t)a.st.cap; }
 WT_D uint32_t* trace_cone_queue(const launch_args_t& a) { return a.st.heavy_queue + 4 * (size_t)a.st.cap; }
+WT_D uint32_t* pass_c_wide_queue(const launch_args_t& a) { return a.st.intd_queue + 2 * (size_t)a.st.cap; }
+WT_D uint32_t* pass_c_commit_queue(const launch_args_t& a) { return a.st.intd_queue + 4 * (size_t)a.st.cap; }
+constexpr uint32_t kOutcomeAccepted = 0x80000000u;
+WT_D uint32_t* pass_c_outcome(const launch_args_t& a, uint32_t w) { return a.st.tris + (size_t)w * kTriListWords; }
+constexpr uint32_t kPrepTries = 8;
+constexpr size_t kPassCTierSlot = 160, kPassCWalksSlot = 163, kPassCRoundsSlot = 164, kPassCQueueSlot = 168, kPassCQueueSlots = kProfSlots - kPassCQueueSlot;
 WT_D void lds_stack(stack_entry_t* lds, stack_entry_t* spill, stack_ref_t& s, uint32_t block = kBlock) {
     s = make_stack_ref(lds + threadIdx.x, block, kLdsStack + kSpillStack, kLdsStack, spill);
 }
@@ -304,6 +311,7 @@
     ctl[CTL_INTB_COUNT] = ctl[CTL_INTB_HEAD] = ctl[CTL_GATHER_COUNT] = ctl[CTL_GATHER_HEAD] = ctl[CTL_INTC_COUNT] = ctl[CTL_INTC_HEAD] = 0;
     ctl[CTL_FTASK_COUNT] = ctl[CTL_FTASK_HEAD] = ctl[CTL_FSPLIT_HEAD] = ctl[CTL_EPOOL_COUNT] = ctl[CTL_FSD_ECOUNTER] = 0;
     ctl[CTL_INTD_COUNT] = ctl[CTL_INTD_HEAD] = 0;
+    ctl[CTL_PCW_COUNT] = ctl[CTL_PCW_HEAD] = ctl[CTL_PCC_COUNT] = ctl[CTL_PCC_HEAD] = 0;
 }
 WT_D void interact_round_begin(uint32_t* ctl) {
     ctl[CTL_HEAVY_COUNT] = 0;
@@ -423,6 +431,10 @@
 __global__ void k_flux_tasks(launch_args_t a);
 __global__ void k_interact_c(launch_args_t a, int in);
 __global__ void k_interact_c_hard(launch_args_t a, int in);
+__global__ void k_interact_c_prep(launch_args_t a, uint32_t thin_below, uint32_t easy_tries);
+__global__ void k_interact_c_wide(launch_args_t a, uint32_t easy_tries);
+__global__ void k_interact_c_hard_tries(launch_args_t a, uint32_t easy_tries);
+__global__ void k_interact_c_commit(launch_args_t a, int in);
 __global__ void k_path_generate(launch_args_t a);
 __global__ void k_path_fsd(launch_args_t a, const path_state_t* __restrict__ ps, uint32_t round);
 __global__ void k_path_edges(launch_args_t a, const path_state_t* __restrict__ ps);
diff --git a/wave_tracer_amd/csrc/wtgpu_knobs.h b/wave_tracer_amd/csrc/wtgpu_knobs.h
--- a/wave_tracer_amd/csrc/wtgpu_knobs.h
+++ b/wave_tracer_amd/csrc/wtgpu_knobs.h
@@ -8,7 +8,7 @@
     uint32_t first_rounds, rounds_margin, light_rounds, max_rounds, stagger_round;
     uint32_t shrink_r1, shrink_f1, shrink_r2, shrink_f2, shrink_h1, decay_q, decay_c;
     uint32_t heavy_waves_per_cu, round_blocks_per_cu, grid_div_b, grid_div_c, grid_div_hard, grid_mul_flux;
-    uint32_t sorted_interact, coop_io, staged_connect, connect_class, tiled_splat;
+    uint32_t sorted_interact, coop_io, staged_connect, connect_class, tiled_splat, pass_c_tiers, pass_c_easy_tries, pass_c_thin;
     uint32_t trace_staged, trace_stages, trace_staged_rounds, trace_sm, trace_ab;
     uint32_t develop_per_pixel, tonemap_lds_table, film_polar_staged, film_denoise_fused;
     uint32_t dbg_stage;
diff --git a/wave_tracer_amd/csrc/wtgpu_knobs.hip b/wave_tracer_amd/csrc/wtgpu_knobs.hip
--- a/wave_tracer_amd/csrc/wtgpu_knobs.hip
+++ b/wave_tracer_amd/csrc/wtgpu_knobs.hip
@@ -50,6 +50,9 @@
     {"WTGPU_COOP_IO", K(coop_io), KNOB_U32, 0, 0, kU32, "1: pass A with wave-cooperative record transfers (k_interact_coop)"},
     {"WTGPU_STAGED_CONNECT", K(staged_connect), KNOB_U32, 0, 0, kU32, "connections: 0 k_connect_strat (one kernel per strategy item); 1 k_connect_eval -> k_connect_shadow -> k_connect_mis, in chunks"},
     {"WTGPU_CONNECT_CLASS", K(connect_class), KNOB_U32, 1, 0, kU32, "connections (the one-kernel form): 0 k_connect_strat (an item is one strategy of a sample); 1 k_connect_class (an item is a sample, bucketed by the lengths of its subpaths, all of its strategies in a row; DESIGN.md §4)"},
+    {"WTGPU_PASS_C_TIERS", K(pass_c_tiers), KNOB_U32, 1, 0, 1, "pass C: 1 in three lane shapes (k_interact_c_prep: 8 lanes per walk, power sum and tries 0-7; k_interact_c_wide / _hard_tries: tries only; k_interact_c_commit: lane = walk); 0 k_interact_c / k_interact_c_hard, one wavefront per walk (A/B; the results do not depend on it; DESIGN.md §4)"},
+    {"WTGPU_PASS_C_EASY_TRIES", K(pass_c_easy_tries), KNOB_U32, 512, 8, kU32, "pass C in tiers: the try from which four wavefronts take a walk over (kernels_fsd.hip: kEasyTries); the tests move it to drive walks into every tier, the results do not depend on it"},
+    {"WTGPU_PASS_C_THIN", K(pass_c_thin), KNOB_U32, 8, 0, kU32, "pass C in tiers: a round whose queue holds at most this many walks per wavefront of k_interact_c_prep's grid takes one wavefront per walk there (the thin rounds are bound by their longest walk, not by lanes); 0: groups of eight always (the tests); the results do not depend on it"},
     {"WTGPU_TILED_SPLAT", K(tiled_splat), KNOB_U32, 1, 0, kU32, "0: the plain per-sample splat kernel"},
     {"WTGPU_TRACE_STAGED", K(trace_staged), KNOB_U32, 1, 0, kU32, "1: the traversal in stages (k_tr_axis / k_tr_cone / k_tr_policy / k_tr_tail) ..."},
     {"WTGPU_TRACE_STAGES", K(trace_stages), KNOB_U32, 3, 1, 16, "... with this many cone stages before the tail ..."},
diff --git a/wave_tracer_amd/csrc/wtgpu_upload.hip b/wave_tracer_amd/csrc/wtgpu_upload.hip
--- a/wave_tracer_amd/csrc/wtgpu_upload.hip
+++ b/wave_tracer_amd/csrc/wtgpu_upload.hip
@@ -170,7 +170,7 @@
     if ((rc = dmalloc(s, &st.intb_queue, W2))) return rc;
     if ((rc = dmalloc(s, &st.gather_queue, W2))) return rc;
     if ((rc = dmalloc(s, &st.intc_queue, W2))) return rc;
-    if ((rc = dmalloc(s, &st.intd_queue, W2))) return rc;
+    if ((rc = dmalloc(s, &st.intd_queue, (path_mode ? 1 : 3) * W2))) return rc;
     st.ftask_cap = path_mode ? 1u : (1u << 22);
     if ((rc = dmalloc(s, &st.ftasks, (size_t)st.ftask_cap))) return rc;
     if ((rc = dmalloc(s, &st.facc, path_mode ? 1 : W2))) return rc;
```
